# lzhangbj/deep_video_interpolation_extrapolation

Hardware: AMD Instinct MI355X
Metric: train frames/s (256x512 len-3 clips) (higher is better)
Workload: dtype bf16; 1 GPU; InterNet int_5_len_3 train step 256x512 bf16; per_gpu_batch=8, global_batch=8, parallelism=dp1, step=eager, executor side-stream lanes

## Files before the change

deep_video_interpolation_extrapolation_amd/_lib.py:

```python
import ctypes
import os
import threading

import torch

LIB_PATH = os.path.join(os.path.dirname(os.path.abspath(__file__)), "libdvie.so")

DVIE_OK = 0
DVIE_EINVAL = 1001
F32, BF16 = 0, 1
ACT_NONE, ACT_LRELU, ACT_ELU, ACT_RELU, ACT_TANH = 0, 1, 2, 3, 4
EW_FUSE, EW_UPT, EW_POOL, EW_POOLT, EW_COPY, EW_L1SIGN, EW_NCHW, EW_TONCHW, EW_MASK, EW_IM2COL, EW_LABELS = range(11)
LOSS_L1, LOSS_GDL, LOSS_SSIM, LOSS_MSE, LOSS_CE, LOSS_L1NHWC, LOSS_COSNHWC, LOSS_IOU, LOSS_ARGMAX_IOU = range(9)
OP_CONV, OP_WGRAD, OP_WREDUCE, OP_COLSUM, OP_EW, OP_LOSS, OP_PACK = 1, 2, 3, 4, 5, 6, 7
OP_BN_FWD, OP_BN_BWD, OP_HEAD_FWD, OP_HEAD_BWD, OP_ATTN, OP_HEAD3_BWD, OP_SEGENC_FWD = 8, 9, 10, 11, 12, 13, 14
OP_SEGENC_BWD = 15
OP_WREDUCE_MULTI = 16
(ATTN_L2NORM, ATTN_L2NORM_BWD, ATTN_CORR, ATTN_GATHER, ATTN_GATHER_T, ATTN_SOFTMAX, ATTN_SOFTMAX_BWD, ATTN_WNORM,
 ATTN_WNORM_BWD, ATTN_POOL, ATTN_POOL_T) = range(11)

vp = ctypes.c_void_p
i32 = ctypes.c_int
i64 = ctypes.c_longlong
f32 = ctypes.c_float


class ConvDesc(ctypes.Structure):
    _fields_ = [
        ("x", vp), ("w", vp), ("y", vp), ("bias", vp), ("res", vp), ("z", vp),
        ("x_ld", i64), ("y_ld", i64), ("res_ld", i64), ("z_ld", i64),
        ("n", i32), ("ih", i32), ("iw", i32), ("c", i32),
        ("kpad", i32), ("cout", i32),
        ("oh", i32), ("ow", i32), ("sy", i32), ("sx", i32),
        ("th", i32), ("tw", i32), ("dy0", i32), ("dx0", i32), ("ddy", i32), ("ddx", i32),
        ("yh", i32), ("yw", i32), ("osy", i32), ("osx", i32), ("ory", i32), ("orx", i32),
        ("act", i32), ("dact", i32), ("beta", i32), ("dtype", i32),
        ("out_f32", i32), ("alpha", f32), ("phc", i32), ("pad1", i32),
    ]


class WgradDesc(ctypes.Structure):
    _fields_ = [
        ("g", vp), ("x", vp), ("ws", vp),
        ("g_ld", i64), ("x_ld", i64),
        ("n", i32), ("oh", i32), ("ow", i32), ("cout", i32),
        ("ih", i32), ("iw", i32), ("c", i32), ("sy", i32),
        ("sx", i32), ("th", i32), ("tw", i32), ("dy0", i32),
        ("dx0", i32), ("ddy", i32), ("ddx", i32), ("splits", i32),
        ("dtype", i32), ("tmap", i32), ("bws", vp), ("ws_taps", i32), ("pad1", i32),
    ]


class WreduceDesc(ctypes.Structure):
    _fields_ = [
        ("ws", vp), ("dw", vp), ("cmap", vp),
        ("splits", i32), ("ws_rows", i32), ("ws_k", i32), ("co_off", i32),
        ("cout_p", i32), ("cin_p", i32), ("kh_n", i32), ("kw_n", i32),
        ("c", i32), ("beta", i32),
    ]


class ColsumDesc(ctypes.Structure):
    _fields_ = [
        ("g", vp), ("ws", vp), ("g_ld", i64), ("rows", i64),
        ("c", i32), ("splits", i32), ("dtype", i32), ("pad0", i32),
    ]


class PackDesc(ctypes.Structure):
    _fields_ = [
        ("src", vp), ("dst", vp), ("cmap", vp),
        ("rows", i32), ("kpad", i32), ("c", i32), ("mode", i32),
        ("th", i32), ("tw", i32), ("kh0", i32), ("kw0", i32),
        ("dkh", i32), ("dkw", i32), ("cout_s", i32), ("cin_s", i32),
        ("kh_s", i32), ("kw_s", i32), ("dtype", i32), ("blk0", i32),
    ]


class EwDesc(ctypes.Structure):
    _fields_ = [
        ("y", vp), ("src0", vp), ("src1", vp), ("src2", vp), ("res", vp), ("z", vp),
        ("ext", vp), ("mean", vp), ("std", vp),
        ("y_ld", i64), ("src_ld0", i64), ("src_ld1", i64), ("src_ld2", i64), ("res_ld", i64), ("z_ld", i64),
        ("sn", i64), ("sc", i64), ("sh", i64), ("sw", i64),
        ("op", i32), ("n", i32), ("h", i32), ("w", i32),
        ("c", i32), ("nsrc", i32), ("sh0", i32), ("sw0", i32),
        ("sh1", i32), ("sw1", i32), ("sh2", i32), ("sw2", i32),
        ("act", i32), ("dact", i32), ("beta", i32), ("dtype", i32),
        ("ext_c", i32), ("align", i32),
        ("alpha", f32), ("scale", f32),
    ]


class LossDesc(ctypes.Structure):
    _fields_ = [
        ("a", vp), ("b", vp), ("grad", vp), ("out", vp), ("partial", vp), ("ws", vp),
        ("a_sn", i64), ("a_sc", i64), ("a_sh", i64), ("a_sw", i64),
        ("b_sn", i64), ("b_sc", i64), ("b_sh", i64), ("b_sw", i64),
        ("kind", i32), ("bsz", i32), ("ch", i32), ("h", i32),
        ("w", i32), ("beta", i32), ("dtype", i32), ("out_acc", i32),
        ("weight", f32), ("out_scale", f32),
    ]


class WarpDesc(ctypes.Structure):
    _fields_ = [
        ("img", vp), ("flow", vp), ("out", vp), ("dout", vp), ("dimg", vp), ("dflow", vp), ("ws", vp),
        ("n", i32), ("c", i32), ("h", i32), ("w", i32),
        ("align_corners", i32), ("pad0", i32),
    ]


class ClipDesc(ctypes.Structure):
    _fields_ = [
        ("img", vp), ("seg", vp), ("idx", vp), ("params", vp), ("frames", vp), ("segs", vp), ("bad", vp),
        ("b", i32), ("t", i32), ("h0", i32), ("w0", i32), ("hc", i32), ("wc", i32),
        ("n_classes", i32), ("pad0", i32),
    ]


class SynthLoadDesc(ctypes.Structure):
    _fields_ = [("frames", vp), ("out", vp), ("npix", i64), ("out_ld", i32), ("pad0", i32)]


class SynthFinishDesc(ctypes.Structure):
    _fields_ = [
        ("rgb", vp), ("seg", vp), ("frame", vp), ("label", vp), ("npix", i64),
        ("rgb_ld", i32), ("seg_ld", i32), ("n_classes", i32), ("pad0", i32),
    ]


class SynthLoadPadDesc(ctypes.Structure):
    _fields_ = [
        ("frames", vp), ("labels", vp), ("out", vp), ("label_out", vp),
        ("n", i32), ("h", i32), ("w", i32), ("hp", i32), ("wp", i32), ("out_ld", i32),
    ]


class SynthFinishCropDesc(ctypes.Structure):
    _fields_ = [
        ("rgb", vp), ("seg", vp), ("frame", vp), ("label", vp), ("label_canvas", vp),
        ("n", i32), ("h", i32), ("w", i32), ("hp", i32), ("wp", i32),
        ("rgb_ld", i32), ("seg_ld", i32), ("n_classes", i32), ("pad0", i32),
    ]


class SynthBridgeDesc(ctypes.Structure):
    _fields_ = [
        ("rgb", vp), ("seg", vp), ("dst", vp), ("npix", i64),
        ("rgb_ld", i32), ("seg_ld", i32), ("dst_ld", i32), ("dtype", i32),
        ("n_rgb", i32), ("rgb_w", i32), ("seg_w", i32), ("pad0", i32),
    ]


class SynthScoreDesc(ctypes.Structure):
    _fields_ = [
        ("pred", vp), ("gt", vp), ("pred_label", vp), ("gt_label", vp),
        ("sse", vp), ("ssim", vp), ("agree", vp), ("valid", vp), ("inter", vp), ("uni", vp), ("ws", vp),
        ("pred_s0", i64), ("pred_s1", i64), ("gt_s0", i64), ("gt_s1", i64),
        ("pred_label_s0", i64), ("pred_label_s1", i64), ("gt_label_s0", i64), ("gt_label_s1", i64),
        ("n0", i32), ("n1", i32), ("h", i32), ("w", i32), ("n_classes", i32), ("pad0", i32),
    ]


class BnDesc(ctypes.Structure):
    _fields_ = [
        ("x", vp), ("y", vp), ("g", vp), ("dx", vp), ("gamma", vp), ("beta", vp), ("dgamma", vp), ("dbeta", vp),
        ("running_mean", vp), ("running_var", vp), ("partial", vp), ("stats", vp),
        ("x_ld", i64), ("y_ld", i64), ("g_ld", i64), ("dx_ld", i64), ("rows", i64),
        ("c", i32), ("splits", i32), ("act", i32), ("training", i32),
        ("dtype", i32), ("accumulate", i32), ("beta_dx", i32), ("x_f32", i32),
        ("alpha", f32), ("eps", f32), ("momentum", f32), ("pad1", f32),
    ]


class HeadDesc(ctypes.Structure):
    _fields_ = [
        ("x", vp), ("gx", vp), ("gout", vp), ("out", vp), ("pooled", vp),
        ("x_ld", i64), ("gx_ld", i64),
        ("n", i32), ("h", i32), ("w", i32), ("c", i32),
        ("pool", i32), ("dtype", i32), ("beta", i32), ("pad0", i32),
    ]


class SoftmaxDesc(ctypes.Structure):
    _fields_ = [
        ("x", vp), ("y", vp), ("gy", vp), ("gx", vp),
        ("sn", i64), ("sc", i64), ("sh", i64), ("sw", i64),
        ("n", i32), ("c", i32), ("h", i32), ("w", i32),
        ("beta", i32), ("pad0", i32),
    ]


class SnLayer(ctypes.Structure):
    _fields_ = [
        ("w_bar", vp), ("u", vp), ("v", vp), ("w_eff", vp), ("g_eff", vp), ("g_bar", vp), ("g_u", vp), ("g_v", vp),
        ("state_off", i64),
        ("h", i32), ("width", i32), ("power_iterations", i32), ("beta", i32),
    ]


class AttnDesc(ctypes.Structure):
    _fields_ = [
        ("a", vp), ("b0", vp), ("b1", vp), ("y", vp), ("res", vp), ("z", vp),
        ("a_ld", i64), ("b_ld", i64), ("y_ld", i64), ("res_ld", i64), ("z_ld", i64),
        ("op", i32), ("n", i32), ("h", i32), ("w", i32),
        ("c", i32), ("wh", i32), ("ww", i32), ("nhalf", i32),
        ("half0", i32), ("act", i32), ("dact", i32), ("beta", i32),
        ("dtype", i32), ("pad0", i32),
        ("alpha", f32), ("pad1", f32),
    ]


class PackList(ctypes.Structure):
    _fields_ = [("descs_dev", vp), ("n", i32), ("blocks", i32)]


class Head3BwdDesc(ctypes.Structure):
    _fields_ = [
        ("g", vp), ("h", vp), ("wd", vp), ("dh", vp), ("ws", vp),
        ("g_ld", i64), ("h_ld", i64), ("dh_ld", i64),
        ("n", i32), ("hgt", i32), ("wid", i32), ("c", i32),
        ("cout", i32), ("kpad", i32), ("dy0", i32), ("dx0", i32),
        ("splits", i32), ("dact", i32),
        ("alpha", f32), ("pad0", f32),
    ]


class SegencDesc(ctypes.Structure):
    _fields_ = [
        ("inp", vp), ("e1", vp), ("e2", vp), ("out", vp), ("w0", vp), ("w2", vp), ("w4", vp),
        ("b0", vp), ("b2", vp), ("b4", vp),
        ("in_ld", i64), ("e1_ld", i64), ("e2_ld", i64), ("out_ld", i64),
        ("n", i32), ("h", i32), ("w", i32), ("kpad0", i32), ("kpad2", i32), ("kpad4", i32),
    ]


class SegencBwdDesc(ctypes.Structure):
    _fields_ = [
        ("dout", vp), ("e2", vp), ("e1", vp), ("inp", vp), ("w4d", vp), ("w2d", vp),
        ("dw4", vp), ("dw2", vp), ("dw0", vp), ("db4", vp), ("db2", vp), ("db0", vp),
        ("dout_ld", i64), ("e2_ld", i64), ("e1_ld", i64), ("in_ld", i64),
        ("n", i32), ("h", i32), ("w", i32), ("kpad4", i32), ("kpad2", i32), ("slabs", i32),
    ]


class WreduceMultiDesc(ctypes.Structure):
    _fields_ = [("descs", vp), ("n", i32), ("pad", i32)]


class _OpUnion(ctypes.Union):
    _fields_ = [
        ("conv", ConvDesc), ("wgrad", WgradDesc), ("wreduce", WreduceDesc), ("colsum", ColsumDesc),
        ("ew", EwDesc), ("loss", LossDesc), ("pack", PackList), ("bn", BnDesc), ("head", HeadDesc),
        ("attn", AttnDesc), ("head3", Head3BwdDesc), ("segenc", SegencDesc), ("segenc_bwd", SegencBwdDesc),
        ("wreduce_multi", WreduceMultiDesc),
    ]


class Op(ctypes.Structure):
    _fields_ = [("kind", i32), ("lane", i32), ("u", _OpUnion)]


_ABI = {0: Op, OP_CONV: ConvDesc, OP_WGRAD: WgradDesc, OP_WREDUCE: WreduceDesc, OP_COLSUM: ColsumDesc,
        OP_EW: EwDesc, OP_LOSS: LossDesc, OP_PACK: PackDesc, OP_BN_FWD: BnDesc, OP_HEAD_FWD: HeadDesc,
        OP_ATTN: AttnDesc, OP_HEAD3_BWD: Head3BwdDesc, OP_SEGENC_FWD: SegencDesc, OP_SEGENC_BWD: SegencBwdDesc, OP_WREDUCE_MULTI: WreduceMultiDesc, 100: WarpDesc, 101: SoftmaxDesc, 102: SnLayer, 103: ClipDesc,
        104: SynthLoadDesc, 105: SynthFinishDesc, 106: SynthBridgeDesc, 107: SynthScoreDesc,
        108: SynthLoadPadDesc, 109: SynthFinishCropDesc}

EXPORTS = [
    "dvie_conv2d_fwd", "dvie_conv2d_wgrad", "dvie_wgrad_splits_hint", "dvie_wgrad_slabs", "dvie_wgrad_reduce", "dvie_wgrad_reduce_multi", "dvie_colsum", "dvie_pack_weights",
    "dvie_ew", "dvie_loss", "dvie_loss_partial_count", "dvie_loss_ws_floats", "dvie_warp_fwd",
    "dvie_warp_bwd", "dvie_adamax", "dvie_scale", "dvie_run_ops", "dvie_abi_sizeof", "dvie_version",
    "dvie_last_error", "dvie_bn_fwd", "dvie_bn_bwd", "dvie_bn_partial_splits", "dvie_head_fwd", "dvie_head_bwd",
    "dvie_softmax_fwd", "dvie_softmax_bwd", "dvie_adam", "dvie_sn_fwd", "dvie_sn_bwd", "dvie_reparam_fwd",
    "dvie_reparam_bwd", "dvie_warp_ws_floats", "dvie_clip_prep", "dvie_attn", "dvie_step_inc", "dvie_adamax_dev",
    "dvie_adam_dev", "dvie_mfma_probe", "dvie_launch_probe", "dvie_sum_f32", "dvie_wgrad_bias_slabs", "dvie_head3_bwd",
    "dvie_segenc_fwd", "dvie_segenc_bwd", "dvie_pack_blocks", "dvie_trace_kernels", "dvie_traced_kernels",
    "dvie_synth_load", "dvie_synth_finish", "dvie_synth_bridge", "dvie_synth_score", "dvie_synth_score_ws_bytes",
    "dvie_synth_load_pad", "dvie_synth_finish_crop",
]

_lib = None
_lock = threading.Lock()


class DvieError(RuntimeError):
    pass


def load():
    global _lib
    if _lib is not None:
        return _lib
    with _lock:
        if _lib is not None:
            return _lib
        if not os.path.exists(LIB_PATH):
            raise DvieError(
                f"{LIB_PATH} is missing: build it with `python -c 'import __graft_entry__ as g; g.build()'` "
                "(there is no non-HIP fallback)")
        lib = ctypes.CDLL(LIB_PATH)
        lib.dvie_abi_sizeof.restype = ctypes.c_size_t
        lib.dvie_abi_sizeof.argtypes = [i32]
        for which, st in _ABI.items():
            got = lib.dvie_abi_sizeof(which)
            if got != ctypes.sizeof(st):
                raise DvieError(f"ABI mismatch for {st.__name__}: C {got} vs ctypes {ctypes.sizeof(st)}")
        lib.dvie_version.restype = ctypes.c_char_p
        lib.dvie_last_error.restype = ctypes.c_char_p
        for name in ("dvie_conv2d_fwd", "dvie_conv2d_wgrad", "dvie_wgrad_reduce", "dvie_colsum", "dvie_ew",
                     "dvie_loss", "dvie_warp_fwd", "dvie_warp_bwd", "dvie_bn_fwd", "dvie_bn_bwd", "dvie_head_fwd",
                     "dvie_head_bwd", "dvie_softmax_fwd", "dvie_softmax_bwd", "dvie_clip_prep", "dvie_attn",
                     "dvie_head3_bwd", "dvie_segenc_fwd", "dvie_segenc_bwd", "dvie_synth_load", "dvie_synth_finish",
                     "dvie_synth_bridge", "dvie_synth_score", "dvie_synth_load_pad", "dvie_synth_finish_crop"):
            getattr(lib, name).argtypes = [vp, vp]
            getattr(lib, name).restype = i32
        lib.dvie_pack_weights.argtypes = [vp, i32, i32, vp]
        lib.dvie_wgrad_reduce_multi.argtypes = [vp, i32, vp]
        lib.dvie_wgrad_reduce_multi.restype = i32
        lib.dvie_trace_kernels.argtypes = [i32]
        lib.dvie_trace_kernels.restype = i32
        lib.dvie_traced_kernels.argtypes = []
        lib.dvie_traced_kernels.restype = ctypes.c_char_p
        for name in ("dvie_wgrad_splits_hint", "dvie_wgrad_slabs", "dvie_bn_partial_splits", "dvie_pack_blocks"):
            getattr(lib, name).argtypes = [vp]
            getattr(lib, name).restype = i32
        lib.dvie_run_ops.argtypes = [vp, i32, vp]
        lib.dvie_loss_partial_count.argtypes = [vp]
        lib.dvie_loss_partial_count.restype = ctypes.c_size_t
        lib.dvie_warp_ws_floats.argtypes = [vp]
        lib.dvie_warp_ws_floats.restype = ctypes.c_size_t
        lib.dvie_loss_ws_floats.argtypes = [vp]
        lib.dvie_loss_ws_floats.restype = ctypes.c_size_t
        lib.dvie_synth_score_ws_bytes.argtypes = [vp]
        lib.dvie_synth_score_ws_bytes.restype = ctypes.c_size_t
        lib.dvie_adamax.argtypes = [vp, vp, vp, vp, i64, f32, f32, f32, f32, f32, vp]
        lib.dvie_scale.argtypes = [vp, i64, f32, vp]
        lib.dvie_adam.argtypes = [vp, vp, vp, vp, i64, f32, f32, f32, f32, f32, vp]
        f64 = ctypes.c_double
        lib.dvie_adamax_dev.argtypes = [vp, vp, vp, vp, i64, f64, f64, f64, f64, f64, vp, vp]
        lib.dvie_adam_dev.argtypes = [vp, vp, vp, vp, i64, f64, f64, f64, f64, f64, vp, vp]
        lib.dvie_step_inc.argtypes = [vp, vp]
        lib.dvie_mfma_probe.argtypes = [vp, i32, i32, vp]
        lib.dvie_mfma_probe.restype = i32
        lib.dvie_launch_probe.argtypes = [i32, i32, vp]
        lib.dvie_launch_probe.restype = i32
        lib.dvie_sum_f32.argtypes = [vp, i32, vp, vp]
        lib.dvie_sum_f32.restype = i32
        lib.dvie_wgrad_bias_slabs.argtypes = [vp]
        lib.dvie_wgrad_bias_slabs.restype = i32
        for name in ("dvie_sn_fwd", "dvie_sn_bwd"):
            getattr(lib, name).argtypes = [vp, i32, vp, vp]
            getattr(lib, name).restype = i32
        lib.dvie_reparam_fwd.argtypes = [vp, vp, vp, vp, i64, vp]
        lib.dvie_reparam_bwd.argtypes = [vp, vp, vp, vp, vp, i64, i32, vp]
        lib.dvie_reparam_fwd.restype = lib.dvie_reparam_bwd.restype = i32
        _lib = lib
        return lib


def check(rc, what=""):
    if rc != DVIE_OK:
        msg = load().dvie_last_error().decode(errors="replace") if rc == DVIE_EINVAL else f"hipError {rc}"
        raise DvieError(f"{what}: {msg}")


def stream_ptr(device=None):
    return torch.cuda.current_stream(device).cuda_stream


def require_gpu(t):
    if not t.is_cuda:
        raise DvieError("dvie ops run on the MI355X only: tensor is on %s (no CPU fallback)" % t.device)
```

deep_video_interpolation_extrapolation_amd/csrc/conv1x1.hip:

```cpp
#include <stdlib.h>

#include "conv_epilogue.h"

namespace dvie {

typedef __attribute__((address_space(3))) void* lds_ptr_1x1;

#define DVIE_VMCNT1(N) __builtin_amdgcn_s_waitcnt(((N) & 15) | (((N) >> 4) << 14) | (7 << 4) | (15 << 8))

__device__ __forceinline__ void transpose8x8(i32x4 (&ob)[8], int lane) {
  const int b = lane & 7;
#pragma unroll
  for (int d = 4; d >= 1; d >>= 1) {
    const bool up = (b & d) != 0;
#pragma unroll
    for (int k = 0; k < 8; ++k) {
      if (k & d) continue;
      i32x4 t, r;
#pragma unroll
      for (int e = 0; e < 4; ++e) t[e] = up ? ob[k][e] : ob[k + d][e];
#pragma unroll
      for (int e = 0; e < 4; ++e) r[e] = __shfl_xor(t[e], d);
#pragma unroll
      for (int e = 0; e < 4; ++e) {
        ob[k][e] = up ? r[e] : ob[k][e];
        ob[k + d][e] = up ? ob[k + d][e] : r[e];
      }
    }
  }
}

template <int TMC, int NS, int KC, int NWP, int MI = 1, int NWC = 1>
struct G1Cfg {
  static constexpr int NW = NWP * NWC;
  static constexpr int BC = 32 * TMC * NWC;
  static constexpr int BP = 32 * MI * NWP;
  static constexpr int RB = KC * 2;
  static constexpr int NCH = RB / 16;
  static constexpr int RPP = 64 / NCH;
  static constexpr int NSL = KC / 16;
  static constexpr int XSZ = BP * RB;
  static constexpr int WSZ = BC * RB;
  static constexpr int STAGE = XSZ + WSZ;
  static constexpr int SMEM = NS * STAGE;
  static constexpr int XQ = BP / RPP / NW;
  static constexpr int WQ = (BC / RPP + NW - 1) / NW;
  static __device__ __forceinline__ int swz(int row) { return NCH == 8 ? (row >> 1) & 7 : (row >> 2) & 3; }
};

template <int TMC, int NS, int KC, int NWP, int MI, int NWC, bool OUTF32, int PRE = 0, bool CE = false>
__global__ __launch_bounds__(64 * NWP * NWC) void conv1x1_kernel(const dvie_conv_desc p, int n_ct, int n_tiles, int dbg) {
  dbg = DVIE_DBG(dbg);
  typedef G1Cfg<TMC, NS, KC, NWP, MI, NWC> C;
  constexpr int NW = C::NW;
  __shared__ __attribute__((aligned(1024))) char smem[C::SMEM];
  const int tid = threadIdx.x, lane = tid & 63;
  const int wave = __builtin_amdgcn_readfirstlane(tid >> 6);
  const int r32 = lane & 31, hh = lane >> 5;
  const unsigned OOB = 0xFFFFFFF0u;

  const int g = blockIdx.x & 7, i8 = blockIdx.x >> 3;
  const int q8 = n_tiles >> 3, r8 = n_tiles & 7;
  const int bid = (g < r8 ? g * (q8 + 1) : r8 * (q8 + 1) + (g - r8) * q8) + i8;
  const int c0 = (bid % n_ct) * C::BC;
  const int p0 = (bid / n_ct) * C::BP;
  const int npix = p.n * p.oh * p.ow;
  const int nk = (p.c + KC - 1) / KC;

  const int lrow = lane / C::NCH, lch = lane % C::NCH;
  unsigned xo[C::XQ];
#pragma unroll
  for (int q = 0; q < C::XQ; ++q) {
    const int row = (wave + NW * q) * C::RPP + lrow;
    const int cs = lch ^ C::swz(row);
    xo[q] = (p0 + row < npix) ? (unsigned)(p0 + row) * (unsigned)p.x_ld * 2u + cs * 16u : OOB;
    if (cs * 8 >= p.c) xo[q] = OOB;
  }
  unsigned wo[C::WQ];
#pragma unroll
  for (int q = 0; q < C::WQ; ++q) {
    const int row = (wave + NW * q) * C::RPP + lrow;
    const int cs = lch ^ C::swz(row);
    wo[q] = (row < C::BC && cs * 8 < p.c) ? (unsigned)row * (unsigned)p.kpad * 2u + cs * 16u : OOB;
  }
  const unsigned long long xbytes =
      ((unsigned long long)p.n * p.ih * p.iw - 1) * (unsigned long long)p.x_ld * 2ull + (unsigned long long)p.c * 2ull;
  const unsigned wbytes = (unsigned)p.cout * (unsigned)p.kpad * 2u;

  auto stage = [&](int k, int sb) {
    char* X = smem + sb * C::STAGE;
    char* W = X + C::XSZ;
    const int xr = (int)(xbytes - (unsigned long long)k * C::RB);
    const __amdgpu_buffer_rsrc_t rx =
        __builtin_amdgcn_make_buffer_rsrc((void*)((const char*)p.x + (size_t)k * C::RB), 0, xr, 0x00020000);
    const unsigned wb = (unsigned)(c0 * p.kpad + KC * k) * 2u;
    const __amdgpu_buffer_rsrc_t rw =
        __builtin_amdgcn_make_buffer_rsrc((void*)((const char*)p.w + wb), 0, (int)(wbytes - wb), 0x00020000);
    const int cvalid = p.c - KC * k;
#pragma unroll
    for (int q = 0; q < C::XQ; ++q) {
      const int row = (wave + NW * q) * C::RPP + lrow;
      const int cs = lch ^ C::swz(row);
      const unsigned o = cs * 8 < cvalid ? xo[q] : OOB;
      __builtin_amdgcn_raw_ptr_buffer_load_lds(rx, (lds_ptr_1x1)(X + (wave + NW * q) * 1024), 16, o, 0, 0, 0);
    }
#pragma unroll
    for (int q = 0; q < C::WQ; ++q) {
      if (wave + NW * q < C::BC / C::RPP) {
        const int row = (wave + NW * q) * C::RPP + lrow;
        const int cs = lch ^ C::swz(row);
        const unsigned o = cs * 8 < cvalid ? wo[q] : OOB;
        __builtin_amdgcn_raw_ptr_buffer_load_lds(rw, (lds_ptr_1x1)(W + (wave + NW * q) * 1024), 16, o, 0, 0, 0);
      }
    }
  };

  const int wp = wave % NWP, wc = wave / NWP;
  int xf[C::NSL], wf[C::NSL];
#pragma unroll
  for (int s = 0; s < C::NSL; ++s) {
    const int prow = wp * 32 * MI + r32;
    xf[s] = prow * C::RB + (((2 * s + hh) ^ C::swz(prow)) << 4);
    wf[s] = (wc * 32 * TMC + r32) * C::RB + (((2 * s + hh) ^ C::swz(r32)) << 4);
  }

  f32x16 acc[MI][TMC];
#pragma unroll
  for (int i = 0; i < MI; ++i)
#pragma unroll
    for (int j = 0; j < TMC; ++j)
#pragma unroll
      for (int e = 0; e < 16; ++e) acc[i][j][e] = 0.f;

#pragma unroll
  for (int k = 0; k < (NS > 1 ? NS - 1 : 1); ++k)
    if (k < nk) stage(k, k);

  static_assert(PRE == 0 || (NS == 1 && !OUTF32), "operand prefetch: single K-step, bf16 output");
  i32x4 pr_r[(PRE & 1) ? MI : 1][TMC][2], pr_b[(PRE & 2) ? MI : 1][TMC][2], pr_z[(PRE & 4) ? MI : 1][TMC][2];
  constexpr bool CEL = CE && (PRE & (PRE - 1)) != 0;
  if constexpr (CEL) {
    const int wp0 = wave % NWP, wc0 = wave / NWP;
    const int a8 = r32 >> 3, bl = lane & 7;
    const int co = c0 + wc0 * 32 * TMC + 16 * bl + 8 * hh;
#pragma unroll
    for (int k = 0; k < 8; ++k) {
      const int pix = p0 + wp0 * 32 + 8 * a8 + k;
      const bool ok = pix < npix;
      const long long q = ok ? pix : 0;
      if constexpr ((PRE & 1) != 0)
        pr_r[0][k >> 1][k & 1] = ok ? *(const i32x4*)((const bf16_t*)p.res + q * p.res_ld + co) : i32x4{0, 0, 0, 0};
      if constexpr ((PRE & 2) != 0)
        pr_b[0][k >> 1][k & 1] = ok ? *(const i32x4*)((const bf16_t*)p.y + q * p.y_ld + co) : i32x4{0, 0, 0, 0};
      if constexpr ((PRE & 4) != 0)
        pr_z[0][k >> 1][k & 1] = ok ? *(const i32x4*)((const bf16_t*)p.z + q * p.z_ld + co) : i32x4{0, 0, 0, 0};
    }
  } else if constexpr (PRE != 0) {
    const int wp0 = wave % NWP, wc0 = wave / NWP;
#pragma unroll
    for (int i = 0; i < MI; ++i)
#pragma unroll
      for (int j = 0; j < TMC; ++j)
#pragma unroll
        for (int P = 0; P < 2; ++P) {
          const int pix = p0 + wp0 * 32 * MI + 32 * i + r32;
          const int co = c0 + wc0 * 32 * TMC + 32 * j + 16 * P + 8 * hh;
          const bool ok = pix < npix && co < p.cout;
          const long long q = ok ? pix : 0;
          if constexpr ((PRE & 1) != 0)
            pr_r[i][j][P] = ok ? *(const i32x4*)((const bf16_t*)p.res + q * p.res_ld + co) : i32x4{0, 0, 0, 0};
          if constexpr ((PRE & 2) != 0)
            pr_b[i][j][P] = ok ? *(const i32x4*)((const bf16_t*)p.y + q * p.y_ld + co) : i32x4{0, 0, 0, 0};
          if constexpr ((PRE & 4) != 0)
            pr_z[i][j][P] = ok ? *(const i32x4*)((const bf16_t*)p.z + q * p.z_ld + co) : i32x4{0, 0, 0, 0};
        }
  }
  for (int k = 0; k < nk; ++k) {
    const int sb = k % NS;
    if constexpr (NS >= 3) {
      static_assert(NS <= 5, "wait table covers up to 3 stages in flight");
      constexpr int P_HI = C::XQ + C::WQ, P_LO = C::XQ + C::WQ - 1;
      static_assert(3 * P_HI < 64, "vmcnt is 6 bits");
      const bool hi = wave + NW * (C::WQ - 1) < C::BC / C::RPP;
      const int m = min(NS - 2, nk - 1 - k);
      if (m >= 3) {
        if (hi) DVIE_VMCNT1(3 * P_HI); else DVIE_VMCNT1(3 * P_LO);
      } else if (m == 2) {
        if (hi) DVIE_VMCNT1(2 * P_HI); else DVIE_VMCNT1(2 * P_LO);
      } else if (m == 1) {
        if (hi) DVIE_VMCNT1(P_HI); else DVIE_VMCNT1(P_LO);
      } else {
        __builtin_amdgcn_s_waitcnt(0);
      }
    } else {
      __builtin_amdgcn_s_waitcnt(0);
    }
    __builtin_amdgcn_s_barrier();
    if (NS > 1 && k + NS - 1 < nk) stage(k + NS - 1, (k + NS - 1) % NS);
    const char* X = smem + sb * C::STAGE;
    const char* W = X + C::XSZ;
    if (dbg & 2) continue;
#pragma unroll
    for (int s = 0; s < C::NSL; ++s) {
      i32x4 b[MI], a[TMC];
#pragma unroll
      for (int i = 0; i < MI; ++i) b[i] = *(const i32x4*)(X + xf[s] + i * 32 * C::RB);
#pragma unroll
      for (int j = 0; j < TMC; ++j) a[j] = *(const i32x4*)(W + wf[s] + j * 32 * C::RB);
#pragma unroll
      for (int i = 0; i < MI; ++i)
#pragma unroll
        for (int j = 0; j < TMC; ++j)
          acc[i][j] = __builtin_amdgcn_mfma_f32_32x32x16_bf16(__builtin_bit_cast(bf16x8, a[j]),
                                                              __builtin_bit_cast(bf16x8, b[i]), acc[i][j], 0, 0, 0);
    }
  }

  static_assert(!CE || (MI == 1 && 2 * TMC == 8 && !OUTF32), "coalesced epilogue: 8 chunks per lane");
  if constexpr (CEL) {
    auto tr = [&](i32x4 (&a)[TMC][2]) {
      i32x4 t8[8];
#pragma unroll
      for (int k = 0; k < 8; ++k) t8[k] = a[k >> 1][k & 1];
      transpose8x8(t8, lane);
#pragma unroll
      for (int k = 0; k < 8; ++k) a[k >> 1][k & 1] = t8[k];
    };
    if constexpr ((PRE & 1) != 0) tr(pr_r[0]);
    if constexpr ((PRE & 2) != 0) tr(pr_b[0]);
    if constexpr ((PRE & 4) != 0) tr(pr_z[0]);
  }
  i32x4 ob[CE ? 8 : 1];
#pragma unroll
  for (int i = 0; i < MI; ++i) {
  const int pix0 = p0 + wp * 32 * MI + 32 * i + r32;
  const int pix = CE ? min(pix0, npix - 1) : pix0;
  float v[TMC][2][8];
#pragma unroll
  for (int j = 0; j < TMC; ++j) acc_rows8(acc[i][j], v[j]);
  if (!CE && pix >= npix) continue;
  long long yp = pix;
  if (p.osy != 1 || p.osx != 1 || p.ory != 0 || p.orx != 0 || p.yh != p.oh || p.yw != p.ow) {
    const int hw = p.oh * p.ow;
    const int n = pix / hw, r = pix - n * hw;
    const int oy = r / p.ow, ox = r - oy * p.ow;
    yp = ((long long)n * p.yh + oy * p.osy + p.ory) * p.yw + ox * p.osx + p.orx;
  }
#pragma unroll
  for (int j = 0; j < TMC; ++j)
#pragma unroll
    for (int P = 0; P < 2; ++P) {
      const int co = c0 + wc * 32 * TMC + 32 * j + 16 * P + 8 * hh;
      if (!CE && co >= p.cout) continue;
      float* w = v[j][P];
      if constexpr (OUTF32) {
        epi8_mem<true>(w, p, yp, co);
      } else {
        if (p.bias) add_f32x8(w, p.bias + co);
        bf16_t* dst = (bf16_t*)p.y + yp * p.y_ld + co;
        if (p.res) {
          if constexpr ((PRE & 1) != 0)
            add_bf16x8(w, pr_r[i][j][P]);
          else
            add_bf16x8(w, *(const i32x4*)((const bf16_t*)p.res + yp * p.res_ld + co));
        }
        if (p.beta) {
          if constexpr ((PRE & 2) != 0)
            add_bf16x8(w, pr_b[i][j][P]);
          else
            add_bf16x8(w, *(const i32x4*)dst);
        }
        act8(w, p.act, p.alpha);
        if (p.dact) {
          if constexpr ((PRE & 4) != 0)
            dact_bf16x8(w, pr_z[i][j][P], p.dact, p.alpha);
          else
            dact_bf16x8(w, *(const i32x4*)((const bf16_t*)p.z + yp * p.z_ld + co), p.dact, p.alpha);
        }
        const i32x4 o = pack_bf16x8(w);
        if constexpr (CE)
          ob[2 * j + P] = o;
        else if (!(dbg & 1) || w[0] == 12345.678f)
          *(i32x4*)dst = o;
      }
    }
  }
  if constexpr (CE) {
    transpose8x8(ob, lane);
    const int b = lane & 7;
    const int a8 = r32 >> 3;
#pragma unroll
    for (int k = 0; k < 8; ++k) {
      const int px = p0 + wp * 32 + 8 * a8 + k;
      const int co = c0 + wc * 32 * TMC + 32 * (b >> 1) + 16 * (b & 1) + 8 * hh;
      if (px < npix) *(i32x4*)((bf16_t*)p.y + (long long)px * p.y_ld + co) = ob[k];
    }
  }
}

template <int TMC, int NS, int KC, int NWP, int MI, int NWC>
__global__ __launch_bounds__(64 * NWP * NWC) void conv1x1_persist_kernel(const dvie_conv_desc p, int n_ct, int n_tiles) {
  typedef G1Cfg<TMC, NS, KC, NWP, MI, NWC> C;
  constexpr int NW = C::NW;
  static_assert(NS >= 2, "stage ring");
  __shared__ __attribute__((aligned(1024))) char smem[C::SMEM];
  const int tid = threadIdx.x, lane = tid & 63;
  const int wave = __builtin_amdgcn_readfirstlane(tid >> 6);
  const int r32 = lane & 31, hh = lane >> 5;
  const unsigned OOB = 0xFFFFFFF0u;

  const int G = gridDim.x;
  const int g = blockIdx.x & 7, i8 = blockIdx.x >> 3;
  const int q8 = G >> 3, r8 = G & 7;
  const int b = (g < r8 ? g * (q8 + 1) : r8 * (q8 + 1) + (g - r8) * q8) + i8;
  const int npix = p.n * p.oh * p.ow;
  const int nk = (p.c + KC - 1) / KC;
  const int my_tiles = b < n_tiles ? (n_tiles - 1 - b) / G + 1 : 0;
  const int njobs = my_tiles * nk;
  if (njobs == 0) return;

  const int lrow = lane / C::NCH, lch = lane % C::NCH;
  const unsigned long long xbytes =
      ((unsigned long long)p.n * p.ih * p.iw - 1) * (unsigned long long)p.x_ld * 2ull + (unsigned long long)p.c * 2ull;
  const unsigned wbytes = (unsigned)p.cout * (unsigned)p.kpad * 2u;

  auto stage = [&](int jj, int sb) {
    const int i = jj / nk, k = jj - nk * (jj / nk);
    const int T = b + i * G;
    const int c0 = (T % n_ct) * C::BC, p0 = (T / n_ct) * C::BP;
    char* X = smem + sb * C::STAGE;
    char* W = X + C::XSZ;
    const int xr = (int)(xbytes - (unsigned long long)k * C::RB);
    const __amdgpu_buffer_rsrc_t rx =
        __builtin_amdgcn_make_buffer_rsrc((void*)((const char*)p.x + (size_t)k * C::RB), 0, xr, 0x00020000);
    const unsigned wb = (unsigned)(c0 * p.kpad + KC * k) * 2u;
    const __amdgpu_buffer_rsrc_t rw =
        __builtin_amdgcn_make_buffer_rsrc((void*)((const char*)p.w + wb), 0, (int)(wbytes - wb), 0x00020000);
    const int cvalid = p.c - KC * k;
#pragma unroll
    for (int q = 0; q < C::XQ; ++q) {
      const int row = (wave + NW * q) * C::RPP + lrow;
      const int cs = lch ^ C::swz(row);
      const unsigned o = (cs * 8 < cvalid && p0 + row < npix) ? (unsigned)(p0 + row) * (unsigned)p.x_ld * 2u + cs * 16u : OOB;
      __builtin_amdgcn_raw_ptr_buffer_load_lds(rx, (lds_ptr_1x1)(X + (wave + NW * q) * 1024), 16, o, 0, 0, 0);
    }
#pragma unroll
    for (int q = 0; q < C::WQ; ++q) {
      if (wave + NW * q < C::BC / C::RPP) {
        const int row = (wave + NW * q) * C::RPP + lrow;
        const int cs = lch ^ C::swz(row);
        const unsigned o = (row < C::BC && cs * 8 < cvalid) ? (unsigned)row * (unsigned)p.kpad * 2u + cs * 16u : OOB;
        __builtin_amdgcn_raw_ptr_buffer_load_lds(rw, (lds_ptr_1x1)(W + (wave + NW * q) * 1024), 16, o, 0, 0, 0);
      }
    }
  };

  const int wp = wave % NWP, wc = wave / NWP;
  int xf[C::NSL], wf[C::NSL];
#pragma unroll
  for (int sl = 0; sl < C::NSL; ++sl) {
    const int prow = wp * 32 * MI + r32;
    xf[sl] = prow * C::RB + (((2 * sl + hh) ^ C::swz(prow)) << 4);
    wf[sl] = (wc * 32 * TMC + r32) * C::RB + (((2 * sl + hh) ^ C::swz(r32)) << 4);
  }

  constexpr int P_HI = C::XQ + C::WQ, P_LO = C::XQ + C::WQ - 1;
  static_assert((NS - 2) * P_HI < 64, "vmcnt is 6 bits");
  const bool hi = wave + NW * (C::WQ - 1) < C::BC / C::RPP;
  auto wait_stages = [&](int j) {
    const int m = min(NS - 2, njobs - 1 - j);
    if (m >= 3) {
      if (hi) DVIE_VMCNT1(3 * P_HI); else DVIE_VMCNT1(3 * P_LO);
    } else if (m == 2) {
      if (hi) DVIE_VMCNT1(2 * P_HI); else DVIE_VMCNT1(2 * P_LO);
    } else if (m == 1) {
      if (hi) DVIE_VMCNT1(P_HI); else DVIE_VMCNT1(P_LO);
    } else {
      __builtin_amdgcn_s_waitcnt(0);
    }
  };

  f32x16 acc[MI][TMC];
#pragma unroll
  for (int k = 0; k < NS - 1; ++k)
    if (k < njobs) stage(k, k);
  for (int jj = 0; jj < njobs; ++jj) {
    const int k = jj - nk * (jj / nk);
    if (k == 0) {
#pragma unroll
      for (int i = 0; i < MI; ++i)
#pragma unroll
        for (int j = 0; j < TMC; ++j)
#pragma unroll
          for (int e = 0; e < 16; ++e) acc[i][j][e] = 0.f;
    }
    if (k != 0 || jj == 0) wait_stages(jj);
    __builtin_amdgcn_s_barrier();
    if (jj + NS - 1 < njobs) stage(jj + NS - 1, (jj + NS - 1) % NS);
    const char* X = smem + (jj % NS) * C::STAGE;
    const char* W = X + C::XSZ;
#pragma unroll
    for (int sl = 0; sl < C::NSL; ++sl) {
      i32x4 bq[MI], a[TMC];
#pragma unroll
      for (int i = 0; i < MI; ++i) bq[i] = *(const i32x4*)(X + xf[sl] + i * 32 * C::RB);
#pragma unroll
      for (int j = 0; j < TMC; ++j) a[j] = *(const i32x4*)(W + wf[sl] + j * 32 * C::RB);
#pragma unroll
      for (int i = 0; i < MI; ++i)
#pragma unroll
        for (int j = 0; j < TMC; ++j)
          acc[i][j] = __builtin_amdgcn_mfma_f32_32x32x16_bf16(__builtin_bit_cast(bf16x8, a[j]),
                                                              __builtin_bit_cast(bf16x8, bq[i]), acc[i][j], 0, 0, 0);
    }
    if (k + 1 < nk) continue;
    if (jj + 1 < njobs) wait_stages(jj + 1);

    const int T = b + (jj / nk) * G;
    const int c0 = (T % n_ct) * C::BC, p0 = (T / n_ct) * C::BP;
#pragma unroll
    for (int i = 0; i < MI; ++i) {
      const int pix = p0 + wp * 32 * MI + 32 * i + r32;
      float v[TMC][2][8];
#pragma unroll
      for (int j = 0; j < TMC; ++j) acc_rows8(acc[i][j], v[j]);
      if (pix >= npix) continue;
      long long yp = pix;
      if (p.osy != 1 || p.osx != 1 || p.ory != 0 || p.orx != 0 || p.yh != p.oh || p.yw != p.ow) {
        const int hw = p.oh * p.ow;
        const int n = pix / hw, r = pix - n * hw;
        const int oy = r / p.ow, ox = r - oy * p.ow;
        yp = ((long long)n * p.yh + oy * p.osy + p.ory) * p.yw + ox * p.osx + p.orx;
      }
#pragma unroll
      for (int j = 0; j < TMC; ++j)
#pragma unroll
        for (int P = 0; P < 2; ++P) {
          const int co = c0 + wc * 32 * TMC + 32 * j + 16 * P + 8 * hh;
          if (co >= p.cout) continue;
          epi8_mem<false>(v[j][P], p, yp, co);
        }
    }
  }
  __builtin_amdgcn_s_waitcnt(0);
}

template <int TMC, int NWP, int MI, int NWC, int ACT, int AB = 0>
__global__ __launch_bounds__(64 * NWP * NWC) void conv1x1_ring_kernel(const dvie_conv_desc p, int n_ct, int n_tiles) {
  constexpr int dbg = AB;
  typedef G1Cfg<TMC, 2, 64, NWP, MI, NWC> C;
  constexpr int NW = C::NW, SL = 32768, NSLOT = 5, PPH = 4;
  static_assert(C::XSZ == SL && C::WSZ == SL && C::XQ == PPH && C::WQ == PPH && C::BC / C::RPP == NW * PPH,
                "ring slot = one operand of one K-step, 4 pieces per wave");
  __shared__ __attribute__((aligned(1024))) char smem[NSLOT * SL];
  const int tid = threadIdx.x, lane = tid & 63;
  const int wave = __builtin_amdgcn_readfirstlane(tid >> 6);
  const int r32 = lane & 31, hh = lane >> 5;
  const unsigned OOB = 0xFFFFFFF0u;

  const int G = gridDim.x;
  const int g = blockIdx.x & 7, i8 = blockIdx.x >> 3;
  const int q8 = G >> 3, r8 = G & 7;
  const int b = (g < r8 ? g * (q8 + 1) : r8 * (q8 + 1) + (g - r8) * q8) + i8;
  const int npix = p.n * p.oh * p.ow;
  const int nk = (p.c + 63) / 64;
  const int my_tiles = b < n_tiles ? (n_tiles - 1 - b) / G + 1 : 0;
  const int njobs = my_tiles * nk;
  if (njobs == 0) return;

  const int lrow = lane / C::NCH, lch = lane % C::NCH;
  const unsigned long long xbytes =
      ((unsigned long long)p.n * p.ih * p.iw - 1) * (unsigned long long)p.x_ld * 2ull + (unsigned long long)p.c * 2ull;
  const unsigned wbytes = (unsigned)p.cout * (unsigned)p.kpad * 2u;
  const __amdgpu_buffer_rsrc_t rx = __builtin_amdgcn_make_buffer_rsrc((void*)p.x, 0, (int)xbytes, 0x00020000);
  const __amdgpu_buffer_rsrc_t rw = __builtin_amdgcn_make_buffer_rsrc((void*)p.w, 0, (int)wbytes, 0x00020000);
  const unsigned long long ybytes =
      ((unsigned long long)p.n * p.yh * p.yw - 1) * (unsigned long long)p.y_ld * 2ull + (unsigned long long)p.cout * 2ull;
  const __amdgpu_buffer_rsrc_t ry = __builtin_amdgcn_make_buffer_rsrc(p.y, 0, (int)ybytes, 0x00020000);
  const __amdgpu_buffer_rsrc_t rb = __builtin_amdgcn_make_buffer_rsrc((void*)p.bias, 0, p.bias ? p.cout * 4 : 0, 0x00020000);

  int prow[PPH];
  unsigned xoff[PPH], woff[PPH], chk[PPH];
#pragma unroll
  for (int q = 0; q < PPH; ++q) {
    const int row = (wave + NW * q) * C::RPP + lrow;
    const int cs = lch ^ C::swz(row);
    prow[q] = row;
    chk[q] = (unsigned)cs * 8u;
    xoff[q] = (unsigned)row * (unsigned)p.x_ld * 2u + (unsigned)cs * 16u;
    woff[q] = (unsigned)row * (unsigned)p.kpad * 2u + (unsigned)cs * 16u;
  }
  struct Cur {
    int i, k, c0, p0;
  };
  auto cur_at = [&](int jj) {
    Cur c;
    c.i = jj / nk;
    c.k = jj - c.i * nk;
    const int T = b + c.i * G;
    c.c0 = (T % n_ct) * C::BC;
    c.p0 = (T / n_ct) * C::BP;
    return c;
  };
  auto cur_next = [&](Cur c) {
    if (++c.k == nk) {
      c.k = 0;
      ++c.i;
      const int T = b + c.i * G;
      c.c0 = (T % n_ct) * C::BC;
      c.p0 = (T / n_ct) * C::BP;
    }
    return c;
  };
  auto issue = [&](const Cur& c, bool live, int wop, int sl) {
    char* dst = smem + sl * SL + wave * 1024;
    const int cvalid = live ? p.c - 64 * c.k : 0;
    const int lim = live ? (wop ? p.cout - c.c0 : npix - c.p0) : 0;
    const unsigned base = wop ? (unsigned)c.c0 * (unsigned)p.kpad * 2u + 128u * (unsigned)c.k
                              : (unsigned)c.p0 * (unsigned)p.x_ld * 2u + 128u * (unsigned)c.k;
#pragma unroll
    for (int q = 0; q < PPH; ++q) {
      const bool ok = prow[q] < lim && (cvalid >= 64 || (int)chk[q] < cvalid);
      const unsigned o = ok ? base + (wop ? woff[q] : xoff[q]) : OOB;
      __builtin_amdgcn_raw_ptr_buffer_load_lds(wop ? rw : rx, (lds_ptr_1x1)(dst + q * NW * 1024), 16, o, 0, 0, 0);
    }
  };

  const int wp = wave % NWP, wc = wave / NWP;
  int xf[C::NSL], wf[C::NSL];
#pragma unroll
  for (int sl = 0; sl < C::NSL; ++sl) {
    const int pr = wp * 32 * MI + r32;
    xf[sl] = pr * C::RB + (((2 * sl + hh) ^ C::swz(pr)) << 4);
    wf[sl] = (wc * 32 * TMC + r32) * C::RB + (((2 * sl + hh) ^ C::swz(r32)) << 4);
  }
  const int bco = wc * 32 * TMC + 4 * hh;

  f32x16 acc[MI][TMC];
  Cur cj = cur_at(0);
  Cur cw = cur_next(cj);
  Cur cx = cur_next(cw);
  issue(cj, true, 0, 0);
  issue(cj, true, 1, 1);
  issue(cw, 1 < njobs, 0, 2);
  int s0 = 0;
  int jj = 0;
  auto job = [&](bool first, bool after_epi) {
    if (after_epi)
      DVIE_VMCNT1(PPH + 2 * MI * TMC);
    else
      DVIE_VMCNT1(PPH);
    __builtin_amdgcn_s_waitcnt(0xC07F);
    __builtin_amdgcn_s_barrier();
    f32x4 bi[TMC][4];
    if (first) {
#pragma unroll
      for (int j = 0; j < TMC; ++j)
#pragma unroll
        for (int u = 0; u < 4; ++u) {
          const int co = cj.c0 + bco + 32 * j + 8 * u;
          bi[j][u] = __builtin_bit_cast(f32x4, __builtin_amdgcn_raw_buffer_load_b128(rb, co < p.cout ? (unsigned)co * 4u : OOB, 0, 0));
        }
    }
    if (!(dbg & 4)) {
      const int sw = s0 + 3 >= NSLOT ? s0 + 3 - NSLOT : s0 + 3, sx = s0 + 4 >= NSLOT ? s0 + 4 - NSLOT : s0 + 4;
      issue(cw, jj + 1 < njobs, 1, sw);
      issue(cx, jj + 2 < njobs, 0, sx);
    }
    if (first) {
#pragma unroll
      for (int ii = 0; ii < MI; ++ii)
#pragma unroll
        for (int j = 0; j < TMC; ++j)
#pragma unroll
          for (int e = 0; e < 16; ++e) acc[ii][j][e] = bi[j][e >> 2][e & 3];
    }
    const char* X = smem + s0 * SL;
    const char* W = smem + (s0 + 1 >= NSLOT ? s0 + 1 - NSLOT : s0 + 1) * SL;
#pragma unroll
    for (int sl = 0; sl < C::NSL; ++sl) {
      if (dbg & 2) break;
      i32x4 bq[MI], a[TMC];
#pragma unroll
      for (int ii = 0; ii < MI; ++ii) bq[ii] = *(const i32x4*)(X + xf[sl] + ii * 32 * C::RB);
#pragma unroll
      for (int j = 0; j < TMC; ++j) a[j] = *(const i32x4*)(W + wf[sl] + j * 32 * C::RB);
#pragma unroll
      for (int ii = 0; ii < MI; ++ii)
#pragma unroll
        for (int j = 0; j < TMC; ++j)
          acc[ii][j] = __builtin_amdgcn_mfma_f32_32x32x16_bf16(__builtin_bit_cast(bf16x8, a[j]),
                                                               __builtin_bit_cast(bf16x8, bq[ii]), acc[ii][j], 0, 0, 0);
    }
    s0 = s0 + 2 >= NSLOT ? s0 + 2 - NSLOT : s0 + 2;
    cj = cw;
    cw = cx;
    cx = cur_next(cx);
    ++jj;
  };
  for (int it = 0; it < my_tiles; ++it) {
    const int c0 = cj.c0, p0 = cj.p0;
    job(true, it > 0);
    for (int k = 1; k < nk; ++k) job(false, false);

#pragma unroll
    for (int ii = 0; ii < MI; ++ii) {
      const int pix0 = p0 + wp * 32 * MI + 32 * ii + r32;
      const bool pix_ok = pix0 < npix;
      const int pix = pix_ok ? pix0 : npix - 1;
      long long yp = pix;
      if (p.osy != 1 || p.osx != 1 || p.ory != 0 || p.orx != 0 || p.yh != p.oh || p.yw != p.ow) {
        const int hw = p.oh * p.ow;
        const int n = pix / hw, r = pix - n * hw;
        const int oy = r / p.ow, ox = r - oy * p.ow;
        yp = ((long long)n * p.yh + oy * p.osy + p.ory) * p.yw + ox * p.osx + p.orx;
      }
#pragma unroll
      for (int j = 0; j < TMC; ++j)
#pragma unroll
        for (int P = 0; P < 2; ++P) {
          float w[8];
#pragma unroll
          for (int e = 0; e < 4; ++e) {
            const auto sw = __builtin_amdgcn_permlane32_swap(__float_as_uint(acc[ii][j][8 * P + e]),
                                                             __float_as_uint(acc[ii][j][8 * P + 4 + e]), false, false);
            w[e] = __uint_as_float(sw[0]);
            w[4 + e] = __uint_as_float(sw[1]);
          }
          if (ACT == DVIE_ACT_LRELU) {
#pragma unroll
            for (int e = 0; e < 8; ++e) w[e] = fmaxf(w[e], w[e] * p.alpha);
          }
          const i32x4 o = pack_bf16x8(w);
          const int co = c0 + wc * 32 * TMC + 32 * j + 16 * P + 8 * hh;
          const unsigned yo = (pix_ok && co < p.cout && !(dbg & 1)) ? (unsigned)((yp * p.y_ld + co) * 2) : OOB;
          __builtin_amdgcn_raw_buffer_store_b128(__builtin_bit_cast(i32x4, o), ry, yo, 0, 0);
        }
    }
  }
  __builtin_amdgcn_s_waitcnt(0);
}

template <int V, int NS, int MT>
struct PreOk {
  static constexpr int v = NS != 1 || MT > 4 ? 0 : V;
};

static int dbg_env() {
#ifdef DVIE_TIMING_DBG
  const char* e = getenv("DVIE_1X1_DBG");
  return e && *e ? atoi(e) : 0;
#else
  return 0;
#endif
}

static bool ce_env_on() {
  const char* e = getenv("DVIE_1X1_CE");
  return !(e && *e == '0');
}

template <int TMC, int NS, int KC = 64, int NWP = 8, int MI = 1, int NWC = 1>
static void launch_1x1(const dvie_conv_desc& p, hipStream_t s) {
  typedef G1Cfg<TMC, NS, KC, NWP, MI, NWC> C;
  constexpr int NW = C::NW;
  const int npix = p.n * p.oh * p.ow;
  const int n_ct = (p.cout + C::BC - 1) / C::BC;
  const int n_tiles = n_ct * ((npix + C::BP - 1) / C::BP);
  if (p.out_f32) {
    DVIE_LAUNCH((conv1x1_kernel<TMC, NS, KC, NWP, MI, NWC, true>), dim3(n_tiles), dim3(64 * NW), 0, s, p, n_ct, n_tiles, dbg_env());
    return;
  }
  if constexpr (NS == 2 && KC == 64 && TMC == 4 && NWP == 4 && MI == 2 && NWC == 2) {
    const unsigned long long span = ((unsigned long long)p.n * p.yh * p.yw - 1) * (unsigned long long)p.y_ld * 2ull +
                                    (unsigned long long)p.cout * 2ull;
    const unsigned long long xspan = ((unsigned long long)npix - 1) * (unsigned long long)p.x_ld * 2ull + (unsigned long long)p.c * 2ull;
    if (p.c > KC && n_tiles > 256 && !p.res && !p.beta && !p.dact && span < 0xFFFFFF00ull &&
        xspan < 0xFFFFFF00ull && p.ih == p.oh && p.iw == p.ow &&
        (p.act == DVIE_ACT_NONE || (p.act == DVIE_ACT_LRELU && p.alpha >= 0.f && p.alpha <= 1.f))) {
#ifdef DVIE_TIMING_DBG
      if (p.act == DVIE_ACT_LRELU) switch (dbg_env() & 7) {
#define DVIE_RING_AB(V)                                                                                                \
  case V:                                                                                                              \
    DVIE_LAUNCH((conv1x1_ring_kernel<TMC, NWP, MI, NWC, DVIE_ACT_LRELU, V>), dim3(256), dim3(64 * NW), 0, s, p, n_ct, \
                n_tiles);                                                                                              \
    return;
          DVIE_RING_AB(1) DVIE_RING_AB(2) DVIE_RING_AB(3) DVIE_RING_AB(4) DVIE_RING_AB(5) DVIE_RING_AB(6) DVIE_RING_AB(7)
#undef DVIE_RING_AB
          default: break;
        }
#endif
      if (p.act == DVIE_ACT_LRELU)
        DVIE_LAUNCH((conv1x1_ring_kernel<TMC, NWP, MI, NWC, DVIE_ACT_LRELU>), dim3(256), dim3(64 * NW), 0, s, p, n_ct, n_tiles);
      else
        DVIE_LAUNCH((conv1x1_ring_kernel<TMC, NWP, MI, NWC, DVIE_ACT_NONE>), dim3(256), dim3(64 * NW), 0, s, p, n_ct, n_tiles);
      return;
    }
  }
  if constexpr (NS >= 2 && NS <= 5 && MI * TMC <= 4) {
    const int per_cu = 163840 / C::SMEM;
    const int G = 256 * (per_cu > 2 ? 2 : per_cu);
    if (p.c > KC && n_tiles > G) {
      DVIE_LAUNCH((conv1x1_persist_kernel<TMC, NS, KC, NWP, MI, NWC>), dim3(G), dim3(64 * NW), 0, s, p, n_ct,
                         n_tiles);
      return;
    }
  }
  const bool ident = p.osy == 1 && p.osx == 1 && p.ory == 0 && p.orx == 0 && p.yh == p.oh && p.yw == p.ow;
  int pre = 0;
  if constexpr (NS == 1) {
    if (ident && p.c <= KC) {
      pre = MI * TMC > 4 ? 0 : (p.res ? 1 : 0) | (p.beta ? 2 : 0) | (p.dact ? 4 : 0);
    }
  }
  if constexpr (NS == 1 && MI == 1 && 2 * TMC == 8) {
    if (ident && ce_env_on() && p.cout % C::BC == 0) {
      switch (pre) {
#define DVIE_CE_CASE(V)                                                                                              \
  case V:                                                                                                            \
    DVIE_LAUNCH((conv1x1_kernel<TMC, NS, KC, NWP, MI, NWC, false, PreOk<V, NS, MI * TMC>::v, true>), dim3(n_tiles), \
                       dim3(64 * NW), 0, s, p, n_ct, n_tiles, 0);                                                     \
    return;
        DVIE_CE_CASE(0) DVIE_CE_CASE(1) DVIE_CE_CASE(2) DVIE_CE_CASE(3) DVIE_CE_CASE(4)
        DVIE_CE_CASE(5) DVIE_CE_CASE(6) DVIE_CE_CASE(7)
#undef DVIE_CE_CASE
      }
    }
  }
  switch (pre) {
#define DVIE_PRE_CASE(V)                                                                                          \
  case V:                                                                                                        \
    DVIE_LAUNCH((conv1x1_kernel<TMC, NS, KC, NWP, MI, NWC, false, PreOk<V, NS, MI * TMC>::v>), dim3(n_tiles), \
                       dim3(64 * NW), 0, s, p, n_ct, n_tiles, dbg_env());                                                   \
    break;
    DVIE_PRE_CASE(1) DVIE_PRE_CASE(2) DVIE_PRE_CASE(3) DVIE_PRE_CASE(4) DVIE_PRE_CASE(5)
    DVIE_PRE_CASE(6) DVIE_PRE_CASE(7)
#undef DVIE_PRE_CASE
    default:
      DVIE_LAUNCH((conv1x1_kernel<TMC, NS, KC, NWP, MI, NWC, false>), dim3(n_tiles), dim3(64 * NW), 0, s, p, n_ct, n_tiles, dbg_env());
  }
}

bool conv1x1_launch(const dvie_conv_desc& p, hipStream_t s) {
  if (p.dtype != DVIE_BF16 || p.th != 1 || p.tw != 1) return false;
  if (p.sy != 1 || p.sx != 1 || p.dy0 != 0 || p.dx0 != 0 || p.ih != p.oh || p.iw != p.ow) return false;
  if (p.osy < 1 || p.osx < 1 || p.ory < 0 || p.orx < 0) return false;
  if (p.c % 64 != 0 && p.c > 64) return false;
  if ((long long)p.n * p.oh * p.ow >= (1LL << 31)) return false;
  const int cout = p.cout;
  const bool one = p.c <= 64;
  if (cout <= 64 || (cout <= 128 && one))
    one ? launch_1x1<2, 1>(p, s) : launch_1x1<2, 3>(p, s);
  else if (cout <= 128)
    launch_1x1<4, 3>(p, s);
  else if (one)
    launch_1x1<4, 1>(p, s);
  else
    launch_1x1<4, 2, 64, 4, 2, 2>(p, s);
  return true;
}

}
```

deep_video_interpolation_extrapolation_amd/csrc/conv_epilogue.h:

```cpp
#pragma once
#include "common.h"

namespace dvie {

template <bool F32OUT = false>
__device__ __forceinline__ void act8(float* v, int act, float alpha) {
  if (act == DVIE_ACT_LRELU) {
    for (int k = 0; k < 8; ++k) v[k] = v[k] > 0.f ? v[k] : v[k] * alpha;
  } else if (act == DVIE_ACT_RELU) {
    for (int k = 0; k < 8; ++k) v[k] = v[k] > 0.f ? v[k] : 0.f;
  } else if (act == DVIE_ACT_ELU) {
    for (int k = 0; k < 8; ++k) v[k] = F32OUT ? (v[k] > 0.f ? v[k] : expm1f(v[k])) : elu_bf(v[k]);
  } else if (act == DVIE_ACT_TANH) {
    for (int k = 0; k < 8; ++k) v[k] = F32OUT ? tanhf(v[k]) : tanh_bf(v[k]);
  }
}

__device__ __forceinline__ void dact8(float* v, const float* z, int dact, float alpha) {
  if (dact == DVIE_ACT_LRELU) {
    for (int k = 0; k < 8; ++k) v[k] *= z[k] > 0.f ? 1.f : alpha;
  } else if (dact == DVIE_ACT_RELU) {
    for (int k = 0; k < 8; ++k) v[k] = z[k] > 0.f ? v[k] : 0.f;
  } else if (dact == DVIE_ACT_ELU) {
    for (int k = 0; k < 8; ++k) v[k] *= z[k] > 0.f ? 1.f : z[k] + 1.f;
  } else if (dact == DVIE_ACT_TANH) {
    for (int k = 0; k < 8; ++k) v[k] *= 1.f - z[k] * z[k];
  }
}

__device__ __forceinline__ void unpack_bf16x8(const i32x4 t, float* v) {
#pragma unroll
  for (int e = 0; e < 4; ++e) {
    v[2 * e] = __uint_as_float(((uint32_t)t[e]) << 16);
    v[2 * e + 1] = __uint_as_float(((uint32_t)t[e]) & 0xffff0000u);
  }
}

__device__ __forceinline__ void add_bf16x8(float* w, const i32x4 t) {
  float v[8];
  unpack_bf16x8(t, v);
#pragma unroll
  for (int e = 0; e < 8; ++e) w[e] += v[e];
}

__device__ __forceinline__ void add_f32x8(float* w, const float* s) {
  const f32x4 r0 = *(const f32x4*)s, r1 = *(const f32x4*)(s + 4);
#pragma unroll
  for (int e = 0; e < 4; ++e) {
    w[e] += r0[e];
    w[4 + e] += r1[e];
  }
}

__device__ __forceinline__ i32x4 pack_bf16x8(const float* w) {
  i32x4 o;
#pragma unroll
  for (int e = 0; e < 4; ++e) o[e] = (int)pack_bf16x2(w[2 * e], w[2 * e + 1]);
  return o;
}

__device__ __forceinline__ void dact_bf16x8(float* w, const i32x4 tz, int dact, float alpha) {
  float z[8];
  unpack_bf16x8(tz, z);
  dact8(w, z, dact, alpha);
}

template <bool R, bool B, bool Z>
__device__ __forceinline__ i32x4 epi8_regs(float* w, const dvie_conv_desc& p, const i32x4* r, const i32x4* b,
                                           const i32x4* z) {
  if constexpr (R) add_bf16x8(w, *r);
  if constexpr (B) add_bf16x8(w, *b);
  act8(w, p.act, p.alpha);
  if constexpr (Z) dact_bf16x8(w, *z, p.dact, p.alpha);
  return pack_bf16x8(w);
}

template <bool OUTF32>
__device__ __forceinline__ void epi8_mem(float* w, const dvie_conv_desc& p, long long pix, int co) {
  if (p.bias) add_f32x8(w, p.bias + co);
  if constexpr (OUTF32) {
    float* dst = (float*)p.y + pix * p.y_ld + co;
    if (p.res) add_f32x8(w, (const float*)p.res + pix * p.res_ld + co);
    if (p.beta) add_f32x8(w, dst);
    act8<true>(w, p.act, p.alpha);
    if (p.dact) dact_bf16x8(w, *(const i32x4*)((const bf16_t*)p.z + pix * p.z_ld + co), p.dact, p.alpha);
    *(f32x4*)dst = f32x4{w[0], w[1], w[2], w[3]};
    *(f32x4*)(dst + 4) = f32x4{w[4], w[5], w[6], w[7]};
  } else {
    bf16_t* dst = (bf16_t*)p.y + pix * p.y_ld + co;
    if (p.res) add_bf16x8(w, *(const i32x4*)((const bf16_t*)p.res + pix * p.res_ld + co));
    if (p.beta) add_bf16x8(w, *(const i32x4*)dst);
    act8(w, p.act, p.alpha);
    if (p.dact) dact_bf16x8(w, *(const i32x4*)((const bf16_t*)p.z + pix * p.z_ld + co), p.dact, p.alpha);
    *(i32x4*)dst = pack_bf16x8(w);
  }
}

}
```

deep_video_interpolation_extrapolation_amd/csrc/conv_fwd.hip:

```cpp
#include "common.h"

namespace dvie {

template <typename T>
__device__ __forceinline__ void mfma_chunk(f32x4& acc, const i32x4& a, const i32x4& b);

template <>
__device__ __forceinline__ void mfma_chunk<float>(f32x4& acc, const i32x4& a, const i32x4& b) {
  acc = __builtin_amdgcn_mfma_f32_16x16x4f32(__int_as_float(a[0]), __int_as_float(b[0]), acc, 0, 0, 0);
  acc = __builtin_amdgcn_mfma_f32_16x16x4f32(__int_as_float(a[1]), __int_as_float(b[1]), acc, 0, 0, 0);
  acc = __builtin_amdgcn_mfma_f32_16x16x4f32(__int_as_float(a[2]), __int_as_float(b[2]), acc, 0, 0, 0);
  acc = __builtin_amdgcn_mfma_f32_16x16x4f32(__int_as_float(a[3]), __int_as_float(b[3]), acc, 0, 0, 0);
}

template <>
__device__ __forceinline__ void mfma_chunk<bf16_t>(f32x4& acc, const i32x4& a, const i32x4& b) {
  acc = __builtin_amdgcn_mfma_f32_16x16x32_bf16(__builtin_bit_cast(bf16x8, a), __builtin_bit_cast(bf16x8, b),
                                                acc, 0, 0, 0);
}

__device__ __forceinline__ int swz128(int row, int ch) { return row * 128 + ((ch ^ ((row >> 1) & 7)) << 4); }

typedef __attribute__((address_space(3))) void* lds_ptr_t;

// ... 154 lines not shown
      } else {
        const int kv = kv0 + b_ch[i];
        tap = kv / CV;
        cv = kv - tap * CV;
        const int ti = tap / p.tw;
        dy = p.dy0 + ti * p.ddy;
        dx = p.dx0 + (tap - ti * p.tw) * p.ddx;
      }
      const int iy = by[i] + dy, ix = bx[i] + dx;
      unsigned off = OOB;
      if (tap < ntap && (unsigned)iy < (unsigned)p.ih && (unsigned)ix < (unsigned)p.iw)
        off = (unsigned)(((((unsigned long long)bn[i] * p.ih + iy) * p.iw + ix) * p.x_ld + (unsigned)cv * VEC) * ES);
      __builtin_amdgcn_raw_ptr_buffer_load_lds(rx, (lds_ptr_t)(Bs + (wave + 4 * i) * 1024), 16, off, 0, 0, 0);
    }
  };

  f32x4 acc[TM][TN];
#pragma unroll
  for (int i = 0; i < TM; ++i)
#pragma unroll
    for (int j = 0; j < TN; ++j) acc[i][j] = f32x4{0.f, 0.f, 0.f, 0.f};

  stage(0, 0);
  __builtin_amdgcn_s_waitcnt(0);
  __syncthreads();

  const int r16 = lane & 15;
  for (int kt = 0; kt < nk; ++kt) {
    const int cur = kt & 1;
    if (kt + 1 < nk) stage(kt + 1, cur ^ 1);
    const char* As = smem + cur * STAGE;
    const char* Bs = As + BC * 128;
#pragma unroll
    for (int s = 0; s < 2; ++s) {
      const int ch = 4 * s + (lane >> 4);
      i32x4 af[TM], bfr[TN];
#pragma unroll
      for (int i = 0; i < TM; ++i) af[i] = *(const i32x4*)(As + swz128(wc * (BC / WC) + 16 * i + r16, ch));
#pragma unroll
      for (int j = 0; j < TN; ++j) bfr[j] = *(const i32x4*)(Bs + swz128(wp * (BP / WP) + 16 * j + r16, ch));
#pragma unroll
      for (int i = 0; i < TM; ++i)
#pragma unroll
        for (int j = 0; j < TN; ++j) mfma_chunk<T>(acc[i][j], af[i], bfr[j]);
    }
    __builtin_amdgcn_s_waitcnt(0);
    __syncthreads();
  }

  float* E = (float*)smem;
#pragma unroll
  for (int i = 0; i < TM; ++i)
#pragma unroll
    for (int j = 0; j < TN; ++j) {
      const int co_l = wc * (BC / WC) + 16 * i + 4 * (lane >> 4);
      const int px_l = wp * (BP / WP) + 16 * j + r16;
      *(f32x4*)((char*)E + px_l * EROW + co_l * 4) = acc[i][j];
    }
  __syncthreads();
  constexpr int OV = Out16<OutT>::N;
  constexpr int CPR = BC / OV;
  OutT* __restrict__ yg = (OutT*)p.y;
  const OutT* __restrict__ rg = (const OutT*)p.res;
  const T* __restrict__ zg = (const T*)p.z;
  for (int idx = tid; idx < BP * CPR; idx += 256) {
    const int px_l = idx / CPR;
    const int ck = idx - px_l * CPR;
    const int co = c0 + ck * OV;
    const long long pix = p0 + px_l;
    if (pix >= npix || co >= p.cout) continue;
    float v[OV];
    const char* er = (const char*)E + px_l * EROW + ck * OV * 4;
#pragma unroll
    for (int k = 0; k < OV; k += 4) {
      const f32x4 t = *(const f32x4*)(er + k * 4);
      v[k] = t[0];
      v[k + 1] = t[1];
      v[k + 2] = t[2];
      v[k + 3] = t[3];
    }
    const int n = (int)(pix / hw);
    const int r = (int)(pix - (long long)n * hw);
    const int oy = r / p.ow;
    const int ox = r - oy * p.ow;
    const long long yrow = ((long long)n * p.yh + oy * p.osy + p.ory) * p.yw + ox * p.osx + p.orx;
    if (p.bias) {
#pragma unroll
      for (int k = 0; k < OV; k += 4) {
        const f32x4 b = *(const f32x4*)(p.bias + co + k);
        v[k] += b[0];
        v[k + 1] += b[1];
        v[k + 2] += b[2];
        v[k + 3] += b[3];
      }
    }
    if (rg) {
      float t[OV];
      Out16<OutT>::load(rg + yrow * p.res_ld + co, t);
#pragma unroll
      for (int k = 0; k < OV; ++k) v[k] += t[k];
    }
    if (p.beta) {
      float t[OV];
      Out16<OutT>::load(yg + yrow * p.y_ld + co, t);
#pragma unroll
      for (int k = 0; k < OV; ++k) v[k] += t[k];
    }
    if (p.act) {
#pragma unroll
      for (int k = 0; k < OV; ++k) v[k] = act_fwd(v[k], p.act, p.alpha);
    }
    if (p.dact) {
      float z[OV];
      load_n<T, OV>(zg + yrow * p.z_ld + co, z);
#pragma unroll
      for (int k = 0; k < OV; ++k) v[k] *= act_dz(z[k], p.dact, p.alpha);
    }
    Out16<OutT>::store(yg + yrow * p.y_ld + co, v);
  }
}

template <typename T, int BC, int BP, int WC, int WP>
static void launch_conv(const dvie_conv_desc& p, hipStream_t s) {
  const long long npix = (long long)p.n * p.oh * p.ow;
  const int n_ct = (p.cout + BC - 1) / BC;
  const int n_tiles = (int)((npix + BP - 1) / BP) * n_ct;
  if (p.out_f32)
    DVIE_LAUNCH((conv_igemm_kernel<T, BC, BP, WC, WP, true>), dim3(n_tiles), dim3(256), 0, s, p, n_ct, n_tiles);
  else
    DVIE_LAUNCH((conv_igemm_kernel<T, BC, BP, WC, WP, false>), dim3(n_tiles), dim3(256), 0, s, p, n_ct,
                       n_tiles);
}

template <typename T>
static void dispatch_conv(const dvie_conv_desc& p, hipStream_t s) {
  const long long npix = (long long)p.n * p.oh * p.ow;
  const bool small = npix < 64LL * 512;
  if (p.cout <= 32) {
    if (small) launch_conv<T, 32, 64, 2, 2>(p, s);
    else launch_conv<T, 32, 128, 2, 2>(p, s);
  } else if (p.cout <= 64) {
    if (small) launch_conv<T, 64, 64, 2, 2>(p, s);
    else launch_conv<T, 64, 128, 2, 2>(p, s);
  } else {
    if (small) launch_conv<T, 128, 64, 2, 2>(p, s);
    else launch_conv<T, 128, 128, 2, 2>(p, s);
  }
}

bool conv_halo_launch(const dvie_conv_desc& p, hipStream_t s);
bool conv_halo_ph4_launch(const dvie_conv_desc& p, hipStream_t s);
bool conv1x1_launch(const dvie_conv_desc& p, hipStream_t s);
bool conv_s2_launch(const dvie_conv_desc& p, hipStream_t s);

}

using namespace dvie;

extern "C" int dvie_conv2d_fwd(const dvie_conv_desc* d, void* stream) {
  DVIE_CHECK_ARG(d && d->x && d->w && d->y, "conv: null pointer");
  const int vec = d->dtype == DVIE_BF16 ? 8 : 4;
  const int es = d->dtype == DVIE_BF16 ? 2 : 4;
  const int ovec = (d->out_f32 || d->dtype == DVIE_F32) ? 4 : 8;
  DVIE_CHECK_ARG(d->c > 0 && d->c % vec == 0, "conv: c=%d must be a multiple of %d", d->c, vec);
  DVIE_CHECK_ARG(d->cout > 0 && d->cout % ovec == 0, "conv: cout=%d must be a multiple of %d", d->cout, ovec);
  DVIE_CHECK_ARG(d->kpad % 64 == 0 && d->kpad >= d->th * d->tw * d->c, "conv: kpad=%d", d->kpad);
  DVIE_CHECK_ARG(d->x_ld % vec == 0 && d->y_ld % ovec == 0 && (!d->res || d->res_ld % ovec == 0) &&
                     (!d->z || d->z_ld % ovec == 0),
                 "conv: ld alignment x_ld=%lld y_ld=%lld", d->x_ld, d->y_ld);
  DVIE_CHECK_ARG(d->th >= 1 && d->tw >= 1 && d->th * d->tw <= 64, "conv: taps");
  DVIE_CHECK_ARG(d->n > 0 && d->oh > 0 && d->ow > 0 && d->ih > 0 && d->iw > 0, "conv: empty shape");
  DVIE_CHECK_ARG(((uintptr_t)d->x & 15) == 0 && ((uintptr_t)d->w & 15) == 0 && ((uintptr_t)d->y & 15) == 0,
                 "conv: x/w/y not 16B aligned");
  DVIE_CHECK_ARG(!d->bias || ((uintptr_t)d->bias & 15) == 0, "conv: bias not 16B aligned");
  DVIE_CHECK_ARG(d->dtype == DVIE_BF16 || d->out_f32 || d->dtype == DVIE_F32, "conv: dtype");
  const unsigned long long img_x = (unsigned long long)d->ih * d->iw * d->x_ld * es;
  const unsigned long long wb = (unsigned long long)d->cout * d->kpad * es;
  DVIE_CHECK_ARG(wb < 0xFFFFFF00ull, "conv: weights exceed the 4 GiB buffer range");
  DVIE_CHECK_ARG(img_x < 0xFFFFFF00ull, "conv: one input image exceeds the 4 GiB buffer range");
  hipStream_t s = (hipStream_t)stream;
  const long long chunk = (long long)(0xFFFFFF00ull / img_x) < d->n ? (long long)(0xFFFFFF00ull / img_x) : d->n;
  const int oes = (d->out_f32 || d->dtype == DVIE_F32) ? 4 : 2;
  const unsigned long long img_y = (unsigned long long)d->yh * d->yw;
  for (long long n0 = 0; n0 < d->n; n0 += chunk) {
    dvie_conv_desc c = *d;
    c.n = (int)(d->n - n0 < chunk ? d->n - n0 : chunk);
    c.x = (const char*)d->x + n0 * img_x;
    c.y = (char*)d->y + n0 * img_y * d->y_ld * oes;
    if (d->res) c.res = (const char*)d->res + n0 * img_y * d->res_ld * oes;
    if (d->z) c.z = (const char*)d->z + n0 * img_y * d->z_ld * es;
    if (c.phc) {
      DVIE_CHECK_ARG(conv_halo_ph4_launch(c, s), "conv: phase-split output (phc=%d) needs bf16, 2x2 taps at "
                     "(0,0), osy=osx=2, cout=4*phc, phc %% 32 == 0, no bias", c.phc);
      continue;
    }
    if (conv1x1_launch(c, s)) continue;
    if (conv_halo_launch(c, s)) continue;
    if (conv_s2_launch(c, s)) continue;
    if (c.dtype == DVIE_BF16)
      dispatch_conv<bf16_t>(c, s);
    else
      dispatch_conv<float>(c, s);
  }
  DVIE_RETURN_LAUNCH();
}
```

deep_video_interpolation_extrapolation_amd/csrc/conv_halo.hip:

```cpp
#include <stdlib.h>
#include <string.h>

#include "conv_epilogue.h"

namespace dvie {

typedef __attribute__((address_space(3))) void* lds_ptr_t;

__device__ __forceinline__ int xcd_remap3(int b, int nb) {
  const int g = b & 7, i = b >> 3;
  const int q = nb >> 3, r = nb & 7;
  const int start = g < r ? g * (q + 1) : r * (q + 1) + (g - r) * q;
  return start + i;
}

template <int TM, int WC, int WP, int TH, int TW>
struct HaloCfg {
  static constexpr int NW = WC * WP;
  static constexpr int NTH = NW * 64;
  static constexpr int BC = 32 * TM * WC;
  static constexpr int PR = WP;
  static constexpr int NT = TH * TW;
  static constexpr int HR = PR + TH - 1;
  static constexpr int HWD = 64 + TW - 1;
// ... 661 lines not shown
  auto group_issue = [&](int g) {
    const __amdgpu_buffer_rsrc_t r = g < niter ? rx : rnone;
#pragma unroll
    for (int q = 0; q < C::NPL; ++q) {
      const int pc = wave + NW * q;
      const int j = pc / C::RP, pr = pc - C::RP * (pc / C::RP);
      const int R = g * WR + 2 + j;
      char* dst = smem + (R % C::RR) * C::RB + pr * 1024;
      const unsigned o = lane_off(pr, yb + R);
      __builtin_amdgcn_raw_ptr_buffer_load_lds(r, (lds_ptr_t)dst, 16, o, 0, 0, 0);
    }
  };
  {
#pragma unroll
    for (int q = 0; q < C::NP0; ++q) {
      const int pc = wave + NW * q;
      const int j = pc / C::RP, pr = pc - C::RP * (pc / C::RP);
      char* dst = pc < 2 * C::RP ? smem + j * C::RB + pr * 1024 : smem + C::RR * C::RB + (pc - 2 * C::RP) * 1024;
      const unsigned o = pc < 2 * C::RP ? lane_off(pr, yb + j) : OOB;
      __builtin_amdgcn_raw_ptr_buffer_load_lds(rx, (lds_ptr_t)dst, 16, o, 0, 0, 0);
    }
#pragma unroll
    for (int g = 0; g < D; ++g) group_issue(g);
  }

  constexpr int NE = OUTF32 ? 0 : 4 * (((EPI & 1) ? 1 : 0) + ((EPI & 2) ? 1 : 0) + ((EPI & 4) ? 1 : 0));
  i32x4 er[2][2], eb[2][2], ez[2][2];
  auto epi_issue = [&](int i) {
    const int oy = ys + i * WR + wr;
#pragma unroll
    for (int b = 0; b < 2; ++b)
#pragma unroll
      for (int P = 0; P < 2; ++P) {
        const int ox = x0 + 32 * b + r32, co = 32 * wc + 8 * hh + 16 * P;
        const bool ok = oy < p.oh && ox < p.ow && co < p.cout;
        const long long pix = ((long long)n * p.yh + (long long)oy * p.osy + p.ory) * p.yw + (long long)ox * p.osx + p.orx;
        if constexpr ((EPI & 1) != 0) {
          const __amdgpu_buffer_rsrc_t r = __builtin_amdgcn_make_buffer_rsrc((void*)p.res, 0, 0x7FFFFFF0, 0x00020000);
          er[b][P] = __builtin_amdgcn_raw_buffer_load_b128(r, ok ? (unsigned)((pix * p.res_ld + co) * 2) : OOB, 0, 0);
        }
        if constexpr ((EPI & 2) != 0) {
          const __amdgpu_buffer_rsrc_t r = __builtin_amdgcn_make_buffer_rsrc((void*)p.y, 0, 0x7FFFFFF0, 0x00020000);
          eb[b][P] = __builtin_amdgcn_raw_buffer_load_b128(r, ok ? (unsigned)((pix * p.y_ld + co) * 2) : OOB, 0, 0);
        }
        if constexpr ((EPI & 4) != 0) {
          const __amdgpu_buffer_rsrc_t r = __builtin_amdgcn_make_buffer_rsrc((void*)p.z, 0, 0x7FFFFFF0, 0x00020000);
          ez[b][P] = __builtin_amdgcn_raw_buffer_load_b128(r, ok ? (unsigned)((pix * p.z_ld + co) * 2) : OOB, 0, 0);
        }
      }
  };

  constexpr int NST = OUTF32 ? 8 : 4;
  const int b_lane = r32 * C::PITCH + hh * 16;
  for (int i = 0; i < niter; ++i) {
    wait_vmcnt((D - 1) * C::NPL + min(i, D) * NST + min(i, D - 1) * NE);
    __builtin_amdgcn_s_barrier();
    if constexpr (NE > 0) epi_issue(i);
    group_issue(i + D);

    f32x16 acc[2];
#pragma unroll
    for (int b = 0; b < 2; ++b)
#pragma unroll
      for (int e = 0; e < 16; ++e) acc[b][e] = 0.f;
#pragma unroll
    for (int ti = 0; ti < 3; ++ti) {
      const char* H = smem + ((i * WR + wr + ti) % C::RR) * C::RB + b_lane;
#pragma unroll
      for (int tj = 0; tj < 3; ++tj)
#pragma unroll
        for (int sl = 0; sl < KS; ++sl) {
          i32x4 bf[2];
#pragma unroll
          for (int b = 0; b < 2; ++b) bf[b] = *(const i32x4*)(H + (32 * b + tj) * C::PITCH + sl * 32);
#pragma unroll
          for (int b = 0; b < 2; ++b)
            acc[b] = __builtin_amdgcn_mfma_f32_32x32x16_bf16(__builtin_bit_cast(bf16x8, wa[3 * ti + tj][sl]),
                                                             __builtin_bit_cast(bf16x8, bf[b]), acc[b], 0, 0, 0);
        }
    }
#pragma unroll
    for (int b = 0; b < 2; ++b) {
      if constexpr (OUTF32)
        ws_epilogue<true>(p, acc[b], n, ys + i * WR + wr, x0 + 32 * b + r32, 32 * wc + 8 * hh);
      else
        strip_epilogue<(EPI < 0 ? 0 : EPI)>(p, acc[b], n, ys + i * WR + wr, x0 + 32 * b + r32, 32 * wc + 8 * hh, er[b], eb[b],
                                          ez[b]);
    }
  }
  __builtin_amdgcn_s_waitcnt(0);
}

template <int KS, int WR, int D, int EPI>
static void launch_strip_k(const dvie_conv_desc& p, hipStream_t s) {
  const int tiles_x = (p.ow + 63) / 64;
  const int cap = 256 * (4 / WR);
  const int cols = p.n * tiles_x;
  int nseg = cap / cols;
  if (nseg < 1) nseg = 1;
  if (nseg > (p.oh + WR - 1) / WR) nseg = (p.oh + WR - 1) / WR;
  int seg = (p.oh + nseg - 1) / nseg;
  seg = (seg + WR - 1) / WR * WR;
  nseg = (p.oh + seg - 1) / seg;
  const int n_wg = cols * nseg;
  DVIE_LAUNCH((conv_strip_kernel<KS, EPI, WR, D>), dim3(n_wg), dim3(2 * WR * 64), 0, s, p, tiles_x, nseg, seg,
                     n_wg);
}

template <int KS, int WR, int D>
static bool launch_strip_cfg(const dvie_conv_desc& p, hipStream_t s) {
  if (p.out_f32) {
    launch_strip_k<KS, WR, D, -1>(p, s);
    return true;
  }
  switch ((p.res ? 1 : 0) | (p.beta ? 2 : 0) | (p.dact ? 4 : 0)) {
    case 0: launch_strip_k<KS, WR, D, 0>(p, s); return true;
    case 1: launch_strip_k<KS, WR, D, 1>(p, s); return true;
    case 2: launch_strip_k<KS, WR, D, 2>(p, s); return true;
    case 3: launch_strip_k<KS, WR, D, 3>(p, s); return true;
    case 4: launch_strip_k<KS, WR, D, 4>(p, s); return true;
    case 5: launch_strip_k<KS, WR, D, 5>(p, s); return true;
    case 6: launch_strip_k<KS, WR, D, 6>(p, s); return true;
  }
  return false;
}

static int strip_mode() {
  const char* e = getenv("DVIE_CONV_STRIP");
  return e && *e ? atoi(e) : 2;
}

template <int KS>
static bool launch_strip(const dvie_conv_desc& p, hipStream_t s) {
  switch (strip_mode()) {
    case 1: return launch_strip_cfg<KS, 4, 2>(p, s);
    case 2: return launch_strip_cfg<KS, 2, 2>(p, s);
    case 3: return launch_strip_cfg<KS, 2, 1>(p, s);
  }
  return false;
}

template <int CP8>
struct NkCfg {
  static constexpr int WP = 4, NW = 8;
  static constexpr int HR = WP + 2, HWD = 66;
  static constexpr int PS = CP8 == 1 ? 1 : 3;
  static constexpr int SLOTS = HR * HWD * PS;
  static constexpr int NPC = ((SLOTS + 63) / 64 + NW - 1) / NW;
  static constexpr int HSZ = NPC * NW * 1024;
  static constexpr int NG = 9 * CP8;
  static constexpr int NS = (NG + 1) / 2;
};

template <int CP8, bool OUTF32, bool PRE = false>
__global__ __launch_bounds__(512, 2) void conv_nk_kernel(const dvie_conv_desc p, int n_cb, int n_tiles, int tiles_x,
                                                        int tiles_y) {
  typedef NkCfg<CP8> C;
  __shared__ __attribute__((aligned(1024))) char smem[2 * C::HSZ];
  const int tid = threadIdx.x, lane = tid & 63;
  const int wave = __builtin_amdgcn_readfirstlane(tid >> 6);
  const int wc = wave / C::WP, wp = wave % C::WP;
  const int r32 = lane & 31, hh = lane >> 5;
  const unsigned OOB = 0xFFFFFFF0u;

  const int lid = xcd_remap3(blockIdx.x, gridDim.x);
  const int cb = lid % n_cb;
  const int per_cb = gridDim.x / n_cb;
  const int tile0 = lid / n_cb;
  if (tile0 >= n_tiles) return;

  i32x4 wa[C::NS];
  {
    const int co = cb * 64 + 32 * wc + r32;
#pragma unroll
    for (int sl = 0; sl < C::NS; ++sl) {
      const int k = 16 * sl + 8 * hh;
      i32x4 v = {0, 0, 0, 0};
      if (co < p.cout && k < 9 * p.c) v = *(const i32x4*)((const bf16_t*)p.w + (long long)co * p.kpad + k);
      wa[sl] = v;
    }
  }
  int boff[C::NS];
#pragma unroll
  for (int sl = 0; sl < C::NS; ++sl) {
    const int g = 2 * sl + hh;
    const int t = g < C::NG ? g / CP8 : 0, j = g < C::NG ? g % CP8 : 0;
    boff[sl] = (((t / 3) * C::HWD + (t % 3)) * C::PS + j) * 16;
  }
  int hgeo[C::NPC];
#pragma unroll
  for (int q = 0; q < C::NPC; ++q) {
    const int slot = (wave + C::NW * q) * 64 + lane;
    const int px = slot / C::PS, cs = slot - C::PS * (slot / C::PS);
    const int hy = px / C::HWD, hx = px - (px / C::HWD) * C::HWD;
    hgeo[q] = (cs < CP8 && cs * 8 < p.c && px < C::HR * C::HWD) ? (hy << 16) | (hx << 4) | cs : -1;
  }
  const unsigned xrow = (unsigned)p.x_ld * 2u;
  const unsigned long long xbytes =
      ((unsigned long long)p.n * p.ih * p.iw - 1) * (unsigned long long)p.x_ld * 2ull + (unsigned long long)p.c * 2ull;
  const __amdgpu_buffer_rsrc_t rx = __builtin_amdgcn_make_buffer_rsrc((void*)p.x, 0, (int)xbytes, 0x00020000);
  struct TP {
    int n, y0, x0;
  };
  auto decode = [&](int t) {
    TP q;
    q.x0 = (t % tiles_x) * 64;
    const int r = t / tiles_x;
    q.y0 = (r % tiles_y) * C::WP;
    q.n = r / tiles_y;
    return q;
  };
  auto halo_issue = [&](const TP& T, int hb) {
    char* dst = smem + hb * C::HSZ + wave * 1024;
    const int ybase = T.y0 + p.dy0, xbase = T.x0 + p.dx0;
#pragma unroll
    for (int q = 0; q < C::NPC; ++q) {
      const int gq = hgeo[q];
      const int iy = ybase + (gq >> 16), ix = xbase + ((gq >> 4) & 0xFFF);
      const bool ok = gq >= 0 && (unsigned)iy < (unsigned)p.ih && (unsigned)ix < (unsigned)p.iw;
      const unsigned o = ok ? (unsigned)((T.n * p.ih + iy) * p.iw + ix) * xrow + (unsigned)(gq & 15) * 16u : OOB;
      __builtin_amdgcn_raw_ptr_buffer_load_lds(rx, (lds_ptr_t)(dst + q * C::NW * 1024), 16, o, 0, 0, 0);
    }
  };

  const int b_base = ((wp * C::HWD + r32) * C::PS) * 16;
  TP cur = decode(tile0);
  halo_issue(cur, 0);
  if constexpr (PRE) {
    const int co0 = cb * 64 + 32 * wc + 8 * hh;
    const unsigned long long yspan =
        ((unsigned long long)p.n * p.yh * p.yw - 1) * (unsigned long long)p.y_ld * 2ull + (unsigned long long)p.cout * 2ull;
    const __amdgpu_buffer_rsrc_t ry = __builtin_amdgcn_make_buffer_rsrc(p.y, 0, (int)yspan, 0x00020000);
    const __amdgpu_buffer_rsrc_t rr = __builtin_amdgcn_make_buffer_rsrc(
        (void*)p.res, 0,
        p.res ? (int)(((unsigned long long)p.n * p.yh * p.yw - 1) * (unsigned long long)p.res_ld * 2ull + p.cout * 2ull) : 0,
        0x00020000);
    const __amdgpu_buffer_rsrc_t rz = __builtin_amdgcn_make_buffer_rsrc(
        (void*)p.z, 0,
        p.dact ? (int)(((unsigned long long)p.n * p.yh * p.yw - 1) * (unsigned long long)p.z_ld * 2ull + p.cout * 2ull) : 0,
        0x00020000);
    const int nops = (p.res ? 1 : 0) + (p.beta ? 1 : 0) + (p.dact ? 1 : 0);
    auto offs = [&](const TP& T, int b, int P, unsigned& oy_, unsigned& or_, unsigned& oz_) {
      const int oy = T.y0 + wp, ox = T.x0 + 32 * b + r32, co = co0 + 16 * P;
      const bool ok = oy < p.oh && ox < p.ow && co < p.cout;
      const long long pix = ((long long)T.n * p.yh + oy * p.osy + p.ory) * p.yw + ox * p.osx + p.orx;
      oy_ = ok ? (unsigned)((pix * p.y_ld + co) * 2) : OOB;
      or_ = ok ? (unsigned)((pix * p.res_ld + co) * 2) : OOB;
      oz_ = ok ? (unsigned)((pix * p.z_ld + co) * 2) : OOB;
    };
    i32x4 er[2][2], eb[2][2], ez[2][2];
    auto prefetch = [&](const TP& T) {
#pragma unroll
      for (int b = 0; b < 2; ++b)
#pragma unroll
        for (int P = 0; P < 2; ++P) {
          unsigned o_y, o_r, o_z;
          offs(T, b, P, o_y, o_r, o_z);
          if (p.res) er[b][P] = __builtin_bit_cast(i32x4, __builtin_amdgcn_raw_buffer_load_b128(rr, o_r, 0, 0));
          if (p.beta) eb[b][P] = __builtin_bit_cast(i32x4, __builtin_amdgcn_raw_buffer_load_b128(ry, o_y, 0, 0));
          if (p.dact) ez[b][P] = __builtin_bit_cast(i32x4, __builtin_amdgcn_raw_buffer_load_b128(rz, o_z, 0, 0));
        }
    };
    f32x4 bia[2][2];
#pragma unroll
    for (int P = 0; P < 2; ++P) {
      const int co = co0 + 16 * P;
      bia[P][0] = p.bias && co < p.cout ? *(const f32x4*)(p.bias + co) : f32x4{0.f, 0.f, 0.f, 0.f};
      bia[P][1] = p.bias && co < p.cout ? *(const f32x4*)(p.bias + co + 4) : f32x4{0.f, 0.f, 0.f, 0.f};
    }
    prefetch(cur);
    __builtin_amdgcn_s_waitcnt(0);
    __syncthreads();
    int hb = 0;
    for (int tile = tile0; tile < n_tiles; tile += per_cb, hb ^= 1) {
      const bool has_next = tile + per_cb < n_tiles;
      const TP nxt = decode(has_next ? tile + per_cb : tile);
      halo_issue(nxt, hb ^ 1);
      f32x16 acc[2];
#pragma unroll
      for (int b = 0; b < 2; ++b)
#pragma unroll
        for (int e = 0; e < 16; ++e) acc[b][e] = 0.f;
      const char* H = smem + hb * C::HSZ + b_base;
#pragma unroll
      for (int sl = 0; sl < C::NS; ++sl) {
        i32x4 bf[2];
#pragma unroll
        for (int b = 0; b < 2; ++b) bf[b] = *(const i32x4*)(H + boff[sl] + 32 * b * C::PS * 16);
#pragma unroll
        for (int b = 0; b < 2; ++b)
          acc[b] = __builtin_amdgcn_mfma_f32_32x32x16_bf16(__builtin_bit_cast(bf16x8, wa[sl]), __builtin_bit_cast(bf16x8, bf[b]),
                                                           acc[b], 0, 0, 0);
      }
#pragma unroll
      for (int b = 0; b < 2; ++b) {
        float v[2][8];
#pragma unroll
        for (int P = 0; P < 2; ++P)
#pragma unroll
          for (int e = 0; e < 4; ++e) {
            const auto sw = __builtin_amdgcn_permlane32_swap(__float_as_uint(acc[b][8 * P + e]),
                                                             __float_as_uint(acc[b][8 * P + 4 + e]), false, false);
            v[P][e] = __uint_as_float(sw[0]) + bia[P][0][e];
            v[P][4 + e] = __uint_as_float(sw[1]) + bia[P][1][e];
          }
#pragma unroll
        for (int P = 0; P < 2; ++P) {
          float* w = v[P];
          if (p.res) add_bf16x8(w, er[b][P]);
          if (p.beta) add_bf16x8(w, eb[b][P]);
          act8(w, p.act, p.alpha);
          if (p.dact) dact_bf16x8(w, ez[b][P], p.dact, p.alpha);
          const i32x4 o = pack_bf16x8(w);
          unsigned o_y, o_r, o_z;
          offs(cur, b, P, o_y, o_r, o_z);
          __builtin_amdgcn_raw_buffer_store_b128(__builtin_bit_cast(i32x4, o), ry, o_y, 0, 0);
        }
      }
      prefetch(nxt);
      wait_vmcnt(4 + 4 * nops);
      __builtin_amdgcn_s_barrier();
      cur = nxt;
    }
    __builtin_amdgcn_s_waitcnt(0);
    return;
  }
  __builtin_amdgcn_s_waitcnt(0);
  __syncthreads();
  int hb = 0;
  for (int tile = tile0; tile < n_tiles; tile += per_cb, hb ^= 1) {
    const bool has_next = tile + per_cb < n_tiles;
    const TP nxt = decode(has_next ? tile + per_cb : tile);
    if (has_next) halo_issue(nxt, hb ^ 1);
    f32x16 acc[2];
#pragma unroll
    for (int b = 0; b < 2; ++b)
#pragma unroll
      for (int e = 0; e < 16; ++e) acc[b][e] = 0.f;
    const char* H = smem + hb * C::HSZ + b_base;
#pragma unroll
    for (int sl = 0; sl < C::NS; ++sl) {
      i32x4 bf[2];
#pragma unroll
      for (int b = 0; b < 2; ++b) bf[b] = *(const i32x4*)(H + boff[sl] + 32 * b * C::PS * 16);
#pragma unroll
      for (int b = 0; b < 2; ++b)
        acc[b] = __builtin_amdgcn_mfma_f32_32x32x16_bf16(__builtin_bit_cast(bf16x8, wa[sl]), __builtin_bit_cast(bf16x8, bf[b]),
                                                         acc[b], 0, 0, 0);
    }
    __builtin_amdgcn_s_waitcnt(0);
    __builtin_amdgcn_s_barrier();
#pragma unroll
    for (int b = 0; b < 2; ++b)
      ws_epilogue<OUTF32>(p, acc[b], cur.n, cur.y0 + wp, cur.x0 + 32 * b + r32, cb * 64 + 32 * wc + 8 * hh);
    cur = nxt;
  }
}

static bool nk_pre_on() {
  const char* e = getenv("DVIE_NK_PRE");
  return !(e && *e == '0');
}

template <int CP8>
static void launch_nk(const dvie_conv_desc& p, hipStream_t s) {
  typedef NkCfg<CP8> C;
  const int tiles_x = (p.ow + 63) / 64, tiles_y = (p.oh + C::WP - 1) / C::WP;
  const int n_tiles = tiles_x * tiles_y * p.n;
  const int n_cb = (p.cout + 63) / 64;
  int per_cb = 512 / n_cb;
  if (per_cb < 1) per_cb = 1;
  if (per_cb > n_tiles) per_cb = n_tiles;
  const int grid = per_cb * n_cb;
  const unsigned long long opix = (unsigned long long)p.n * p.yh * p.yw - 1;
  const bool spans_ok = (opix * p.y_ld + p.cout) * 2ull < 0xFFFFFF00ull &&
                        (!p.res || (opix * p.res_ld + p.cout) * 2ull < 0xFFFFFF00ull) &&
                        (!p.dact || (opix * p.z_ld + p.cout) * 2ull < 0xFFFFFF00ull);
  if (p.out_f32)
    DVIE_LAUNCH((conv_nk_kernel<CP8, true>), dim3(grid), dim3(512), 0, s, p, n_cb, n_tiles, tiles_x, tiles_y);
  else if (nk_pre_on() && spans_ok && (p.res || p.beta || p.dact))
    DVIE_LAUNCH((conv_nk_kernel<CP8, false, true>), dim3(grid), dim3(512), 0, s, p, n_cb, n_tiles, tiles_x, tiles_y);
  else
    DVIE_LAUNCH((conv_nk_kernel<CP8, false>), dim3(grid), dim3(512), 0, s, p, n_cb, n_tiles, tiles_x, tiles_y);
}

struct H8 {
  static constexpr int NW = 8, NTH = 512;
  static constexpr int BC = 128, PR = 8, KC = 32;
  static constexpr int HR = PR + 2, HWD = 66, PITCH = 80;
  static constexpr int HSLOTS = HR * HWD * 5;
  static constexpr int NHI = ((HSLOTS + 63) / 64 + NW - 1) / NW * NW;
  static constexpr int NHQ = NHI / NW;
  static constexpr int HSZ = NHI * 1024;
  static constexpr int ASZ = BC * KC * 2;
  static constexpr int WSZ = 3 * ASZ;
  static constexpr int SMEM = 2 * HSZ + 2 * WSZ;
  static constexpr int H0 = 4;
};
static_assert(H8::SMEM <= 163840, "conv_h8 LDS budget");
static_assert(H8::NHQ == 7 && H8::H0 < H8::NHQ, "halo shares");

template <int EPI>
__global__ __launch_bounds__(512) void conv_h8_kernel(const dvie_conv_desc p, int n_ct, int n_tiles, int tiles_x,
                                                      int tiles_y) {
  typedef H8 C;
  __shared__ __attribute__((aligned(1024))) char smem[C::SMEM];
  const int tid = threadIdx.x, lane = tid & 63;
  const int wave = __builtin_amdgcn_readfirstlane(tid >> 6);
  const int wc = wave >> 2, wp = wave & 3;
  const int r32 = lane & 31, hh = lane >> 5;
  const int nchunks = p.c >> 5;
  const unsigned OOB = 0xFFFFFFF0u;

  const int G = gridDim.x, g = blockIdx.x & 7, jb = blockIdx.x >> 3;
  const int nbg = G / 8 + (g < G % 8 ? 1 : 0);
  const int q8 = n_tiles / 8, r8 = n_tiles % 8;
  const int ts = g < r8 ? g * (q8 + 1) : r8 * (q8 + 1) + (g - r8) * q8;
  const int tile0 = ts + jb, tile_end = ts + q8 + (g < r8 ? 1 : 0);
  if (tile0 >= tile_end) return;

  auto tile_job = [&](int t) {
    JobInfo J;
    J.t = t;
    J.k = 0;
    J.valid = t < tile_end;
    J.c0 = (t % n_ct) * C::BC;
    int pt = t / n_ct;
    J.x0 = (pt % tiles_x) * 64;
    pt /= tiles_x;
    J.y0 = (pt % tiles_y) * C::PR;
    J.n = pt / tiles_y;
    return J;
  };
  auto next_job = [&](const JobInfo& J) {
    if (J.k + 1 < nchunks) {
      JobInfo N = J;
      N.k = J.k + 1;
      return N;
    }
    return tile_job(J.t + nbg);
  };

  int hgeo[C::NHQ];
#pragma unroll
  for (int q = 0; q < C::NHQ; ++q) {
    const int slot = (wave + C::NW * q) * 64 + lane;
    const int hr = slot / 5, cs = slot - 5 * (slot / 5);
    const int hy = hr / C::HWD, hx = hr - (hr / C::HWD) * C::HWD;
    hgeo[q] = (cs < 4 && hr < C::HR * C::HWD) ? (hy << 16) | (hx << 4) | cs : -1;
  }
  const int arow = wave * 16 + (lane >> 2);
  const unsigned aoff = (unsigned)arow * (unsigned)p.kpad * 2u + (unsigned)((((lane & 3) ^ ((arow >> 2) & 3))) * 16);
  const unsigned xrow = (unsigned)p.x_ld * 2u;
  const unsigned long long xbytes =
      ((unsigned long long)p.n * p.ih * p.iw - 1) * (unsigned long long)p.x_ld * 2ull + (unsigned long long)p.c * 2ull;
  const unsigned wbytes = (unsigned)p.cout * (unsigned)p.kpad * 2u;

  char* const Hs = smem;
  char* const As = smem + 2 * C::HSZ;

  auto halo_issue = [&](const JobInfo& J, int hb, int qa, int qb) {
    const int nrec = J.valid ? (int)(xbytes - (unsigned long long)J.k * 64) : 0;
    const __amdgpu_buffer_rsrc_t r =
        __builtin_amdgcn_make_buffer_rsrc((void*)((const char*)p.x + (size_t)J.k * 64), 0, nrec, 0x00020000);
    char* dst = Hs + hb * C::HSZ + wave * 1024;
    const int ybase = J.y0 + p.dy0, xbase = J.x0 + p.dx0;
#pragma unroll
    for (int q = qa; q < qb; ++q) {
      const int gq = hgeo[q];
      const int iy = ybase + (gq >> 16), ix = xbase + ((gq >> 4) & 0xFFF);
      const bool ok = gq >= 0 && (unsigned)iy < (unsigned)p.ih && (unsigned)ix < (unsigned)p.iw;
      const unsigned o = ok ? (unsigned)((J.n * p.ih + iy) * p.iw + ix) * xrow + (unsigned)(gq & 15) * 16u : OOB;
      __builtin_amdgcn_raw_ptr_buffer_load_lds(r, (lds_ptr_t)(dst + q * C::NW * 1024), 16, o, 0, 0, 0);
    }
  };
  auto a_issue = [&](const JobInfo& J, int v, int ab, int ti) {
    const __amdgpu_buffer_rsrc_t r = __builtin_amdgcn_make_buffer_rsrc((void*)p.w, 0, J.valid ? (int)wbytes : 0, 0x00020000);
    const unsigned so = (unsigned)(J.c0 * p.kpad + (ti * 3 + v) * p.c + 32 * J.k) * 2u;
    __builtin_amdgcn_raw_ptr_buffer_load_lds(r, (lds_ptr_t)(As + ab * C::WSZ + ti * C::ASZ + wave * 1024), 16, aoff, so, 0,
                                             0);
  };

  const int arw = wc * 64 + r32;
  const int a_s0 = arw * 64 + (((0 + hh) ^ ((arw >> 2) & 3)) << 4);
  const int a_s1 = arw * 64 + (((2 + hh) ^ ((arw >> 2) & 3)) << 4);
  const int b_base = (2 * wp * C::HWD + r32) * C::PITCH + hh * 16;

  f32x16 acc[2][2][2];

  {
    const JobInfo J0 = tile_job(tile0);
    halo_issue(J0, 0, 0, C::NHQ);
#pragma unroll
    for (int ti = 0; ti < 3; ++ti) a_issue(J0, 0, 0, ti);
    __builtin_amdgcn_s_waitcnt(0);
    __syncthreads();
  }

  int hb = 0, ab = 0;
  JobInfo J = tile_job(tile0);
  JobInfo J1 = next_job(J);
  i32x4 pa[2], pb[2][2];
  auto load_p0 = [&](const char* A0, const char* H0, int v0) {
#pragma unroll
    for (int i = 0; i < 2; ++i) pa[i] = *(const i32x4*)(A0 + a_s0 + i * 2048);
#pragma unroll
    for (int r = 0; r < 2; ++r)
#pragma unroll
      for (int b = 0; b < 2; ++b) pb[r][b] = *(const i32x4*)(H0 + (r * C::HWD + 32 * b + v0) * C::PITCH);
  };
  load_p0(As, Hs + b_base, 0);
  while (J.valid) {
    if (J.k == 0) {
#pragma unroll
      for (int i = 0; i < 2; ++i)
#pragma unroll
        for (int r = 0; r < 2; ++r)
#pragma unroll
          for (int b = 0; b < 2; ++b)
#pragma unroll
            for (int e = 0; e < 16; ++e) acc[i][r][b][e] = 0.f;
    }
    const char* H = Hs + hb * C::HSZ + b_base;
    const bool tile_end_job = J.k + 1 == nchunks;
#pragma unroll
    for (int v = 0; v < 3; ++v) {
      const char* A = As + ab * C::WSZ;
      const JobInfo& JW = v < 2 ? J : J1;
      const int vw = v < 2 ? v + 1 : 0;
      i32x4 af[2][3][2], bf[2][4][2];
      auto load_a = [&](int s, int ti) {
#pragma unroll
        for (int i = 0; i < 2; ++i) af[s][ti][i] = *(const i32x4*)(A + (s ? a_s1 : a_s0) + ti * C::ASZ + i * 2048);
      };
      auto load_b = [&](int s, int row) {
#pragma unroll
        for (int b = 0; b < 2; ++b) bf[s][row][b] = *(const i32x4*)(H + (row * C::HWD + 32 * b + v) * C::PITCH + s * 32);
      };
#pragma unroll
      for (int i = 0; i < 2; ++i) af[0][0][i] = pa[i];
#pragma unroll
      for (int r = 0; r < 2; ++r)
#pragma unroll
        for (int b = 0; b < 2; ++b) bf[0][r][b] = pb[r][b];
#pragma unroll
      for (int ph = 0; ph < 6; ++ph) {
        const int s = ph / 3, ti = ph % 3;
        if (ph < 5) {
          const int s2 = (ph + 1) / 3, t2 = (ph + 1) % 3;
          load_a(s2, t2);
          if (t2 == 0) {
            load_b(s2, 0);
            load_b(s2, 1);
          } else {
            load_b(s2, t2 + 1);
          }
        }
        if (ph < 3) a_issue(JW, vw, ab ^ 1, ph);
        if (v == 0 && ph == 3) halo_issue(J1, hb ^ 1, 0, 2);
        if (v == 0 && ph == 4) halo_issue(J1, hb ^ 1, 2, 3);
        if (v == 0 && ph == 5) halo_issue(J1, hb ^ 1, 3, C::H0);
        if (v == 1 && ph == 3) halo_issue(J1, hb ^ 1, C::H0, C::H0 + 1);
        if (v == 1 && ph == 4) halo_issue(J1, hb ^ 1, C::H0 + 1, C::H0 + 2);
        if (v == 1 && ph == 5) halo_issue(J1, hb ^ 1, C::H0 + 2, C::NHQ);
        if (ph == 5) {
          if (v == 0)
            DVIE_VMCNT_LGKM0(C::H0);
          else if (v == 1)
            DVIE_VMCNT_LGKM0(C::NHQ - C::H0);
          else
            DVIE_VMCNT_LGKM0(0);
          __builtin_amdgcn_s_barrier();
          if (v < 2)
            load_p0(As + (ab ^ 1) * C::WSZ, H, v + 1);
          else if (!tile_end_job)
            load_p0(As + (ab ^ 1) * C::WSZ, Hs + (hb ^ 1) * C::HSZ + b_base, 0);
        }
        __builtin_amdgcn_sched_barrier(0);
#pragma unroll
        for (int i = 0; i < 2; ++i)
#pragma unroll
          for (int r = 0; r < 2; ++r)
#pragma unroll
            for (int b = 0; b < 2; ++b)
              acc[i][r][b] = __builtin_amdgcn_mfma_f32_32x32x16_bf16(__builtin_bit_cast(bf16x8, af[s][ti][i]),
                                                                     __builtin_bit_cast(bf16x8, bf[s][ti + r][b]),
                                                                     acc[i][r][b], 0, 0, 0);
        __builtin_amdgcn_sched_barrier(0);
      }
      ab ^= 1;
    }
    hb ^= 1;

    if (J.k + 1 == nchunks) {
      const long long pix0 = ((long long)J.n * p.yh + (long long)J.y0 * p.osy + p.ory) * p.yw + (long long)J.x0 * p.osx + p.orx;
      const __amdgpu_buffer_rsrc_t rr = __builtin_amdgcn_make_buffer_rsrc(
          (void*)((const bf16_t*)p.res + ((EPI & 1) ? pix0 * p.res_ld : 0)), 0, 0x7FFFFFF0, 0x00020000);
      const __amdgpu_buffer_rsrc_t rb =
          __builtin_amdgcn_make_buffer_rsrc((void*)((const bf16_t*)p.y + pix0 * p.y_ld), 0, 0x7FFFFFF0, 0x00020000);
      const __amdgpu_buffer_rsrc_t rz = __builtin_amdgcn_make_buffer_rsrc(
          (void*)((const bf16_t*)p.z + ((EPI & 4) ? pix0 * p.z_ld : 0)), 0, 0x7FFFFFF0, 0x00020000);
      i32x4 o_r[2][2], o_b[2][2], o_z[2][2];
      auto epi_load = [&](int gi) {
        const int i = gi & 1, r = gi >> 2, b = (gi >> 1) & 1, u = gi & 1;
#pragma unroll
          for (int P = 0; P < 2; ++P) {
            const int oy = J.y0 + 2 * wp + r, ox = J.x0 + 32 * b + r32;
            const int co = J.c0 + wc * 64 + 32 * i + 16 * P + 8 * hh;
            const bool ok = oy < p.oh && ox < p.ow;
            const long long dp = (long long)(2 * wp + r) * p.osy * p.yw + (long long)(32 * b + r32) * p.osx;
            if (EPI & 1) o_r[u][P] = __builtin_amdgcn_raw_buffer_load_b128(rr, ok ? (unsigned)((dp * p.res_ld + co) * 2) : OOB, 0, 0);
            if (EPI & 2) o_b[u][P] = __builtin_amdgcn_raw_buffer_load_b128(rb, ok ? (unsigned)((dp * p.y_ld + co) * 2) : OOB, 0, 0);
            if (EPI & 4) o_z[u][P] = __builtin_amdgcn_raw_buffer_load_b128(rz, ok ? (unsigned)((dp * p.z_ld + co) * 2) : OOB, 0, 0);
          }
      };
      if (EPI) epi_load(0);
#pragma unroll
      for (int gi = 0; gi < 8; ++gi) {
        const int i = gi & 1, r = gi >> 2, b = (gi >> 1) & 1, u = gi & 1;
        if (EPI && gi < 7) epi_load(gi + 1);
        __builtin_amdgcn_sched_barrier(0);
        {
          float v8[2][8];
#pragma unroll
          for (int P = 0; P < 2; ++P)
#pragma unroll
            for (int e = 0; e < 4; ++e) {
              const auto sw = __builtin_amdgcn_permlane32_swap(__float_as_uint(acc[i][r][b][8 * P + e]),
                                                               __float_as_uint(acc[i][r][b][8 * P + 4 + e]), false, false);
              v8[P][e] = __uint_as_float(sw[0]);
              v8[P][4 + e] = __uint_as_float(sw[1]);
            }
          const int oy = J.y0 + 2 * wp + r, ox = J.x0 + 32 * b + r32;
          const bool ok = oy < p.oh && ox < p.ow;
          const long long dp = (long long)(2 * wp + r) * p.osy * p.yw + (long long)(32 * b + r32) * p.osx;
#pragma unroll
          for (int P = 0; P < 2; ++P) {
            const int co = J.c0 + wc * 64 + 32 * i + 16 * P + 8 * hh;
            float* w = v8[P];
            if (p.bias) add_f32x8(w, p.bias + co);
            const i32x4 o = epi8_regs<(EPI & 1) != 0, (EPI & 2) != 0, (EPI & 4) != 0>(w, p, &o_r[u][P], &o_b[u][P], &o_z[u][P]);
            if (ok) __builtin_amdgcn_raw_buffer_store_b128(o, rb, (unsigned)((dp * p.y_ld + co) * 2), 0, 0);
          }
        }
        __builtin_amdgcn_sched_barrier(0);
      }
      load_p0(As + ab * C::WSZ, Hs + hb * C::HSZ + b_base, 0);
    }
    J = J1;
    J1 = next_job(J1);
  }
}

static bool h8_on() {
  const char* e = getenv("DVIE_CONV_H8");
  return !(e && *e == '0');
}

template <int EPI>
static void launch_h8(const dvie_conv_desc& p, hipStream_t s, int n_ct, int n_tiles, int tiles_x, int tiles_y) {
  const int grid = n_tiles > 256 ? 256 : n_tiles;
  DVIE_LAUNCH((conv_h8_kernel<EPI>), dim3(grid), dim3(H8::NTH), 0, s, p, n_ct, n_tiles, tiles_x, tiles_y);
}

static bool conv_h8_launch(const dvie_conv_desc& p, hipStream_t s) {
  if (!h8_on() || p.out_f32 || p.c % 32 != 0 || p.c < 64 || p.cout % 128 != 0) return false;
  const int n_ct = p.cout / H8::BC, tiles_x = (p.ow + 63) / 64, tiles_y = (p.oh + H8::PR - 1) / H8::PR;
  const long long nt = (long long)n_ct * tiles_x * tiles_y * p.n;
  if (nt < 224 || nt >= (1LL << 30)) return false;
  const int n_tiles = (int)nt;
  switch ((p.res ? 1 : 0) | (p.beta ? 2 : 0) | (p.dact ? 4 : 0)) {
#define DVIE_H8(EPI) \
  case EPI: launch_h8<EPI>(p, s, n_ct, n_tiles, tiles_x, tiles_y); break;
    DVIE_H8(0) DVIE_H8(1) DVIE_H8(2) DVIE_H8(3) DVIE_H8(4) DVIE_H8(5) DVIE_H8(6) DVIE_H8(7)
#undef DVIE_H8
  }
  return true;
}

bool conv_narrow_launch(const dvie_conv_desc& p, hipStream_t s);

bool conv_halo_ph4_launch(const dvie_conv_desc& p, hipStream_t s) {
  if (p.dtype != DVIE_BF16 || p.out_f32 || p.bias || p.phc <= 0 || p.phc % 32 != 0 || p.cout != 4 * p.phc) return false;
  if (p.th != 2 || p.tw != 2 || p.dy0 != 0 || p.dx0 != 0 || p.ddy != 1 || p.ddx != 1 || p.sy != 1 || p.sx != 1)
    return false;
  if (p.osy != 2 || p.osx != 2 || p.ory != 0 || p.orx != 0) return false;
  if (p.c % 64 != 0 && p.c > 64) return false;
  const unsigned long long pix = (unsigned long long)p.n * p.ih * p.iw;
  if (pix >= (1ull << 31) || ((pix - 1) * (unsigned long long)p.x_ld + (unsigned long long)p.c) * 2ull >= 0xFFFFFF00ull)
    return false;
  return p.cout % 128 != 0 ? try_halo<1, 2, 4, 2, 2, true>(p, s) : try_halo<2, 2, 4, 2, 2, true>(p, s);
}

bool conv_halo_launch(const dvie_conv_desc& p, hipStream_t s) {
  if (p.dtype != DVIE_BF16) return false;
  if (p.sy != 1 || p.sx != 1 || p.ddy != 1 || p.ddx != 1) return false;
  if (p.osy < 1 || p.osx < 1 || p.ory < 0 || p.orx < 0) return false;
  if (p.c % 64 != 0 && p.c > 64) return false;
  const bool t1 = p.th == 1 && p.tw == 1, t3 = p.th == 3 && p.tw == 3;
  const bool t22 = p.th == 2 && p.tw == 2, t12 = p.th == 1 && p.tw == 2, t21 = p.th == 2 && p.tw == 1;
  if (!t1 && !t3 && !t22 && !t12 && !t21) return false;
  const unsigned long long pix = (unsigned long long)p.n * p.ih * p.iw;
  if (pix >= (1ull << 31)) return false;
  if (((pix - 1) * (unsigned long long)p.x_ld + (unsigned long long)p.c) * 2ull >= 0xFFFFFF00ull) return false;
  if (t3 && p.c % 8 == 0 && p.c <= 24 && p.kpad >= 9 * p.c) {
    switch (p.c / 8) {
      case 1: launch_nk<1>(p, s); break;
      case 2: launch_nk<2>(p, s); break;
      default: launch_nk<3>(p, s); break;
    }
    return true;
  }
  if (t3 && p.c <= 64 && p.cout <= 64 && (long long)p.n * p.oh * p.ow >= 65536) {
    switch ((p.c + 15) / 16) {
      case 1: if (!launch_strip<1>(p, s)) launch_ws<1>(p, s); break;
      case 2: if (!launch_strip<2>(p, s)) launch_ws<2>(p, s); break;
      case 3: if (!launch_strip<3>(p, s)) launch_ws<3>(p, s); break;
      default: if (!launch_strip<4>(p, s)) launch_ws<4>(p, s); break;
    }
    return true;
  }
  if (t3 && conv_narrow_launch(p, s)) return true;
  if (t3 && conv_h8_launch(p, s)) return true;
  int cfg;
  if (p.cout <= 32)
    cfg = 2;
  else if (t1)
    cfg = p.cout <= 64 ? 3 : (p.c <= 64 ? 5 : 4);
  else
    cfg = (p.cout <= 64 || p.cout % 128 != 0) ? 3 : 4;
  if (t3 && cfg == 4 && (long long)(p.cout / 128) * ((p.ow + 63) / 64) * ((p.oh + 3) / 4) * p.n < 256) cfg = 5;
  if (t3) return launch_cfg<3, 3>(cfg, p, s);
  if (t1) return launch_cfg<1, 1>(cfg, p, s);
  const int c2 = p.cout <= 64 || p.cout % 128 != 0 ? 3 : 4;
  if (t22) return launch_cfg2<2, 2>(c2, p, s);
  if (t12) return launch_cfg2<1, 2>(c2, p, s);
  return launch_cfg2<2, 1>(c2, p, s);
}

}
```

deep_video_interpolation_extrapolation_amd/engine.py:

```python
import ctypes
import os
from typing import NamedTuple, Optional

import torch

from . import _lib as L

PADC = 8
PROFILE = None
DEBUG_NAN = bool(os.environ.get("DVIE_DEBUG_NAN"))
def _wgrad_lane():
    return os.environ.get("DVIE_WGRAD_LANE", "1") != "0"


OP_HOOK = None


def pack_blocks(d):
    n = L.load().dvie_pack_blocks(ctypes.byref(d))
    assert n > 0, "dvie_pack_blocks: empty pack descriptor"
    return n


def _reduce_meta(name, r):
# ... 468 lines not shown
        self.n_l1 += 1
        self._add(op)
        return op.idx

    def output(self, key, region, channels):
        self.outputs[key] = (region, channels)

    def segenc_chain(self, ops):
        self.segenc.append(tuple(ops))

    def _add(self, op):
        self.ops.append(op)
        if op.out is not None:
            op.out.buf.producers.append(op)
        for r in op.inputs():
            r.buf.consumers.append((op, r))

    def compile(self, n_fwd, device, n_bwd=None, backward=True, alias=False):
        return Plan(self, n_fwd, n_fwd if n_bwd is None else n_bwd, device, backward, alias)


ARENA_ALIGN = 512


def segenc_fusable(dtype, nf, ops):
    if dtype != torch.bfloat16 or os.environ.get("DVIE_SEGENC_FUSED", "1") == "0":
        return False
    o0, o1, o2 = ops
    acts = (L.ACT_ELU, L.ACT_ELU, L.ACT_NONE)
    chans = ((24, 32), (32, 32), (32, 8))
    for op, act, (ci, co) in zip(ops, acts, chans):
        lay = op.layer
        if not (isinstance(op, ConvOp) and op.act == act and op.res is None and lay.kh == 3 and lay.kw == 3
                and lay.stride == 1 and lay.pad == 1 and lay.dil == 1 and lay.has_bias and op.x.c == ci
                and op.out.c == co and lay.cout_p == co):
            return False
    if not (o1.x.buf is o0.out.buf and o2.x.buf is o1.out.buf and o0.out.c0 == 0 and o1.out.c0 == 0):
        return False
    if o0.out.buf.C != 32 or o1.out.buf.C != 32 or o2.out.buf.external:
        return False
    x = o0.x
    return nf * x.H * x.W * x.buf.C * 2 < 0xFFFFFF00


def forward_launches(g, nf):
    fused_first, skip = {}, set()
    if os.environ.get("DVIE_SEGENC_FWD", "1") == "1":
        for chain in g.segenc:
            if segenc_fusable(g.dtype, nf, chain):
                fused_first[id(chain[0])] = chain
                skip.update(id(op) for op in chain[1:])
    return [list(fused_first.get(id(op), (op,))) for op in g.ops if id(op) not in skip]


def _op_regions(op):
    rs = list(op.inputs())
    for r in (op.out, getattr(op, "region", None)):
        if r is not None:
            rs.append(r)
    return rs


def forward_lifetimes(g, nf):
    life = {}
    for i, ops in enumerate(forward_launches(g, nf)):
        for op in ops:
            for r in _op_regions(op):
                a, b = life.get(id(r.buf), (i, i))
                life[id(r.buf)] = (min(a, i), max(b, i))
    for r in g.caller_written.values():
        life[id(r.buf)] = (0, life.get(id(r.buf), (0, 0))[1])
    return life


def assign_offsets(items):
    size = [rup(max(int(b), 1), ARENA_ALIGN) for b, _, _ in items]
    order = sorted(range(len(items)), key=lambda i: (-size[i], items[i][1], i))
    offsets = [0] * len(items)
    placed = []
    arena = 0
    for i in order:
        _, f, l = items[i]
        busy = sorted((offsets[j], offsets[j] + size[j]) for j in placed if items[j][1] <= l and f <= items[j][2])
        off = 0
        for lo, hi in busy:
            if off + size[i] <= lo:
                break
            off = max(off, hi)
        offsets[i] = off
        placed.append(i)
        arena = max(arena, off + size[i])
    if arena > sum(size):
        offsets, arena = [], 0
        for sz in size:
            offsets.append(arena)
            arena += sz
    return offsets, arena


def arena_layout(g, nf):
    life = forward_lifetimes(g, nf)
    n_sites = max([b for _, b in life.values()] + [0])
    bufs = [b for b in g.buffers if not b.external]
    items = []
    for b in bufs:
        nbytes = nf * b.H * b.W * b.C * elem_size(b.dtype or g.dtype)
        items.append((nbytes,) + life.get(id(b), (0, n_sites)))
    offsets, arena = assign_offsets(items)
    return {id(b): o for b, o in zip(bufs, offsets)}, arena, sum(it[0] for it in items)


class Plan:

    def __init__(self, g, nf, nb, device, backward, alias=False):
        assert not (alias and backward), "alias=True is for forward-only plans (a backward reads every activation)"
        self.g, self.nf, self.nb, self.device, self.alias = g, nf, nb, device, alias
        self.dtype = g.dtype
        self.dt = dv_dtype(g.dtype)
        self.es = elem_size(g.dtype)
        self.vec = 16 // self.es
        self.backward_enabled = backward
        self.keep = []
        self.busy = False
        self.generation = 0
        self.static_weights = False
        self._pack_srcs, self._pack_sig, self._pack_descs = [], None, []
        self.arena, self.arena_bytes, self.unaliased_bytes = None, None, 0
        self.l1_out = self.bn_partial = None
        self.bn_splits = 1
        self._seg_bwd, self._seg_inner = {}, set()
        self.fwd = []
        self.bwd = []
        self.fwd_arr = self.bwd_arr = None
        self.fwd_off = self.n_bwd = 0
        self._l1_fwd = []
        self._l1_bwd = []
        self.ext_in = {}
        self.ext_out = {}
        self.ext_mask = {}
        self.ext_nchw_out = {}
        self.ext_head = {}
        self.ext_head_grad = {}
        self.keep_grad = None
        self.ext_grad = {}
        self._grad_slots = []
        self.ext_ograd = {}
        self.wg_first = {}
        self._uses_left = {}
        self.completions = []
        self._multi = []
        self._i2c = None
        self.ws = None
        self.ws_floats = 1
        self._alloc()
        self._build_pack()
        self._build_forward()
        if backward:
            self._build_backward()
        assert all(o.lane == 0 for o in self.fwd), "forward ops run on the caller's stream"
        self._finalize()

    def _alloc(self):
        g = self.g
        offsets, self.arena_bytes, self.unaliased_bytes = arena_layout(g, self.nf) if self.alias else ({}, None, 0)
        if self.alias:
            self.arena = torch.empty(max(self.arena_bytes, ARENA_ALIGN), dtype=torch.uint8, device=self.device)
            self.keep.append(self.arena)
        for b in g.buffers:
            dt = b.dtype or self.dtype
            b.dt = dt
            if b.external:
                b.t = None
            elif self.alias:
                nbytes = self.nf * b.H * b.W * b.C * elem_size(dt)
                o = offsets[id(b)]
                b.t = self.arena[o:o + nbytes].view(dt).view(self.nf, b.H, b.W, b.C)
            else:
                b.t = torch.empty((self.nf, b.H, b.W, b.C), dtype=dt, device=self.device)
                self.unaliased_bytes += b.t.numel() * b.t.element_size()
        if self.backward_enabled:
            for op in g.ops:
                if op.out is None:
                    continue
                need = False
                if isinstance(op, InputOp):
                    need = op.requires_grad
                elif isinstance(op, (ConvOp, ConvTOp)):
                    need = op.layer.trainable or any(r.buf.needs_grad for r in op.inputs())
                elif isinstance(op, BNOp):
                    need = op.trainable or op.x.buf.needs_grad
                elif isinstance(op, FuseOp) and op.detach:
                    need = False
                else:
                    need = any(r.buf.needs_grad for r in op.inputs())
                op.out.buf.needs_grad = op.out.buf.needs_grad or need
            self._seg_bwd = self._segenc_bwd_chains()
            self._seg_inner = {id(op.out.buf) for ch in self._seg_bwd.values() for op in ch[:2]}
            for b in g.buffers:
                if b.needs_grad and id(b) not in self._seg_inner:
                    b.g = torch.zeros((self.nb, b.H, b.W, b.C), dtype=self.dtype, device=self.device)
            for b in g.buffers:
                b.expected, b.pending = {}, {}
                b.n_flushed = 0
                b.done = b.dact_done = False
            for op in g.ops:
                if isinstance(op, FuseOp) and op.detach:
                    continue
                for r in op.inputs():
                    if r.buf.needs_grad:
                        r.buf.expected[r.key()] = r.buf.expected.get(r.key(), 0) + 1
            for b in g.buffers:
                keys = sorted(b.expected)
                for (a0, ac), (b0, _) in zip(keys, keys[1:]):
                    assert a0 + ac <= b0, f"{b}: consumers read overlapping regions {keys}"
        self.l1_out = torch.zeros(max(1, g.n_l1), dtype=torch.float32, device=self.device)
        self.keep.append(self.l1_out)
        for op in g.ops:
            if isinstance(op, BNOp):
                d = L.BnDesc()
                d.rows = self.nf * op.x.H * op.x.W
                self.bn_splits = max(self.bn_splits, L.load().dvie_bn_partial_splits(ctypes.byref(d)))
                d.rows = self.nb * op.x.H * op.x.W
                self.bn_splits = max(self.bn_splits, L.load().dvie_bn_partial_splits(ctypes.byref(d)))
                op.stats = torch.zeros((8, op.x.c), dtype=torch.float32, device=self.device)
                self.keep.append(op.stats)
        maxc = max([op.x.c for op in g.ops if isinstance(op, BNOp)] + [4])
        self.bn_partial = torch.zeros(self.bn_splits * 2 * maxc, dtype=torch.float64, device=self.device)
        self.keep.append(self.bn_partial)

    def ptr(self, region, n0=0, grad=False):
        b = region.buf
        t = b.g if grad else b.t
        es = elem_size(t.dtype)
        return t.data_ptr() + (n0 * b.H * b.W * b.C + region.c0) * es

    def _build_pack(self):
        descs = []
        self._pack_srcs = [t for lay in self.g.layers if lay.cin_p is not None
                           for t in (lay.m.weight, lay.m.bias if lay.has_bias else None) if t is not None]
        self._pack_sig = None
        for lay in self.g.layers:
            if lay.cin_p is None:
                continue
            K = lay.kh * lay.kw * lay.cin_p
            kpad = rup(K, 64)
            lay.kpad = kpad
            lay.wf = torch.zeros((lay.cout_p, kpad), dtype=self.dtype, device=self.device)
            cmap_t = torch.tensor(lay.cmap, dtype=torch.int32, device=self.device)
            lay.cmap_t = cmap_t
            self.keep += [lay.wf, cmap_t]
            ft = lay.fwd_taps()
            descs.append(self._pack_desc(lay, lay.wf, lay.cout_p, kpad, lay.cin_p, 0, ft, cmap_t))
            if lay.has_bias:
                nbias, rows = (lay.cin, lay.cin_p) if lay.transposed else (lay.cout, lay.cout_p)
                lay.bias_p = torch.zeros(rows, dtype=torch.float32, device=self.device)
                self.keep.append(lay.bias_p)
                d = L.PackDesc()
                d.src, d.dst, d.cmap = lay.m.bias.data_ptr(), lay.bias_p.data_ptr(), None
                d.rows, d.kpad, d.c, d.mode = rows, 1, 1, 0
                d.th, d.tw, d.kh0, d.kw0, d.dkh, d.dkw = 1, 1, 0, 0, 1, 1
                d.cout_s, d.cin_s, d.kh_s, d.kw_s, d.dtype = nbias, 1, 1, 1, L.F32
                descs.append(d)
            lay.wd = []
            lay.wd4 = None
        self._pack_descs = descs

    def _pack_desc(self, lay, dst, rows, kpad, c, mode, taps, cmap_t):
        if isinstance(lay.m, StackedConv):
            assert lay.m.contiguous(), f"{lay.name}: stacked parts are not consecutive in memory"
        d = L.PackDesc()
        d.src, d.dst, d.cmap = lay.m.weight.data_ptr(), dst.data_ptr(), cmap_t.data_ptr()
        d.rows, d.kpad, d.c, d.mode = rows, kpad, c, mode
        d.th, d.tw, d.kh0, d.kw0, d.dkh, d.dkw = taps["th"], taps["tw"], taps["kh0"], taps["kw0"], taps["dkh"], taps["dkw"]
        d.cout_s, d.cin_s, d.kh_s, d.kw_s, d.dtype = lay.cout, lay.cin, lay.kh, lay.kw, self.dt
        return d

    def _dgrad_weights(self, lay, H, W):
        key = (H, W)
        for k, v in lay.wd:
            if k == key:
                return v
        out = []
        for ph in lay.dgrad_phases(H, W):
            kpad = rup(ph["th"] * ph["tw"] * lay.cout_p, 64)
            t = torch.zeros((lay.cin_p, kpad), dtype=self.dtype, device=self.device)
            self.keep.append(t)
            self._pack_descs.append(self._pack_desc(lay, t, lay.cin_p, kpad, lay.cout_p, 1, ph, lay.cmap_t))
            out.append((ph, t, kpad))
        lay.wd.append((key, out))
        return out

    PH4_ORDER = ((0, 0), (1, 1), (0, 1), (1, 0))

    def _ph4_eligible(self, lay, x):
        return (self.dtype == torch.bfloat16 and os.environ.get("DVIE_PH4", "1") != "0" and lay.stride == 2
                and lay.kh == 3 and lay.kw == 3 and lay.pad == 1 and lay.dil == 1 and not lay.transposed
                and x.c == lay.cin_p and lay.cin_p % 32 == 0 and lay.cin_p <= 128
                and (lay.cout_p % 64 == 0 or lay.cout_p < 64))

    def _dgrad_weights_ph4(self, lay):
        if lay.wd4 is not None:
            return lay.wd4
        kpad = rup(4 * lay.cout_p, 64)
        t = torch.zeros((4 * lay.cin_p, kpad), dtype=self.dtype, device=self.device)
        self.keep.append(t)
        for q, (a, b) in enumerate(self.PH4_ORDER):
            taps = dict(th=2, tw=2, kh0=a + 1, kw0=b + 1, dkh=-2, dkw=-2)
            self._pack_descs.append(self._pack_desc(lay, t[q * lay.cin_p:(q + 1) * lay.cin_p], lay.cin_p, kpad,
                                                    lay.cout_p, 1, taps, lay.cmap_t))
        lay.wd4 = (t, kpad)
        return lay.wd4

    def _op(self, kind):
        o = L.Op()
        o.kind = kind
        o.ws_base, o.ws_off, o.bws_off, o.ws_ptr = 0, 0, None, None
        o.l1_seed = None
        return o

    def conv_desc(self, x_ptr, x_ld, n, ih, iw, c, w_ptr, kpad, cout, oh, ow, sy, sx, taps, y_ptr, y_ld, yh, yw,
                  osy=1, osx=1, ory=0, orx=0, bias=None, res=None, res_ld=0, z=None, z_ld=0, act=0, dact=0, beta=0,
                  out_f32=False):
        o = self._op(L.OP_CONV)
        d = o.u.conv
        d.x, d.w, d.y, d.bias, d.res, d.z = x_ptr, w_ptr, y_ptr, bias, res, z
        d.x_ld, d.y_ld, d.res_ld, d.z_ld = x_ld, y_ld, res_ld, z_ld
        d.n, d.ih, d.iw, d.c, d.kpad, d.cout = n, ih, iw, c, kpad, cout
        d.oh, d.ow, d.sy, d.sx = oh, ow, sy, sx
        d.th, d.tw, d.dy0, d.dx0, d.ddy, d.ddx = taps["th"], taps["tw"], taps["dy0"], taps["dx0"], taps["ddy"], taps["ddx"]
        d.yh, d.yw, d.osy, d.osx, d.ory, d.orx = yh, yw, osy, osx, ory, orx
        d.act, d.dact, d.beta, d.dtype, d.out_f32 = act, dact, beta, self.dt, int(out_f32)
        d.alpha = 0.2
        return o

    def ew_desc(self, op, n, h, w, c, y_ptr, y_ld, srcs=(), res=None, res_ld=0, z=None, z_ld=0, act=0, dact=0,
                beta=0, scale=1.0):
        o = self._op(L.OP_EW)
        d = o.u.ew
        d.op, d.n, d.h, d.w, d.c = op, n, h, w, c
        d.y, d.y_ld = y_ptr, y_ld
        d.nsrc = len(srcs)
        for i, (p, ld, sh, sw) in enumerate(srcs):
            setattr(d, f"src{i}", p)
            setattr(d, f"src_ld{i}", ld)
            setattr(d, f"sh{i}", sh)
            setattr(d, f"sw{i}", sw)
        d.res, d.res_ld, d.z, d.z_ld = res, res_ld, z, z_ld
        d.act, d.dact, d.beta, d.dtype = act, dact, beta, self.dt
        d.alpha, d.scale = 0.2, scale
        npx = n * h * w
        nbytes = self.es * c * (npx * (1 + int(bool(beta)) + int(res is not None) + int(z is not None))
                                + sum(n * sh * sw for (_, _, sh, sw) in srcs))
        o.meta = dict(cls="pointwise", name=f"ew{op} {n}x{h}x{w}x{c} src{len(srcs)}"
                      + ("+res" if res is not None else "") + ("+acc" if beta else "") + ("+z" if z is not None else ""),
                      flops=0.0, bytes=float(nbytes))
        return o

    def _part(self, part):
        if part is None:
            return 0, self.nf
        return (0 if part == 0 else self.nf // 2), self.nf // 2

    def _segenc_fwd(self, ops):
        o0, o1, o2 = ops
        x, nf = o0.x, self.nf
        o = self._op(L.OP_SEGENC_FWD)
        d = o.u.segenc
        d.inp, d.e1, d.e2, d.out = self.ptr(x), self.ptr(o0.out), self.ptr(o1.out), self.ptr(o2.out)
        d.in_ld, d.e1_ld, d.e2_ld, d.out_ld = x.buf.C, o0.out.buf.C, o1.out.buf.C, o2.out.buf.C
        d.w0, d.w2, d.w4 = o0.layer.wf.data_ptr(), o1.layer.wf.data_ptr(), o2.layer.wf.data_ptr()
        d.b0, d.b2, d.b4 = o0.layer.bias_p.data_ptr(), o1.layer.bias_p.data_ptr(), o2.layer.bias_p.data_ptr()
        d.n, d.h, d.w = nf, x.H, x.W
        d.kpad0, d.kpad2, d.kpad4 = o0.layer.kpad, o1.layer.kpad, o2.layer.kpad
        npx = nf * x.H * x.W
        o.meta = dict(cls="conv_fwd", name="seg_encoder (fused)",
                      flops=2.0 * npx * 9 * sum(op.layer.cout * op.layer.cin for op in ops),
                      bytes=float(self.es * npx * (x.c + 32 + 32 + 8)))
        return o

    def _build_forward(self):
        for site in forward_launches(self.g, self.nf):
            if len(site) > 1:
                self.fwd.append(self._segenc_fwd(tuple(site)))
                continue
            lower = self._FWD.get(type(site[0]))
            if lower is None:
                raise TypeError(site[0])
            lower(self, site[0])

    def _label_input_fwd(self, op):
        o = self.ew_desc(L.EW_LABELS, self.nf, op.out.H, op.out.W, op.out.c, self.ptr(op.out), op.out.buf.C)
        o.u.ew.ext_c = op.ext_c
        self.ext_in.setdefault(op.key, []).append((len(self.fwd), op))
        self.fwd.append(o)

    def _input_fwd(self, op):
        n0, cnt = self._part(op.part)
        o = self.ew_desc(L.EW_NCHW, cnt, op.out.H, op.out.W, op.out.c, self.ptr(op.out, n0), op.out.buf.C)
        o.u.ew.ext_c = op.ext_c
        if op.normalize:
            m = torch.tensor(_IMAGENET_MEAN + [0.0] * 5, dtype=torch.float32, device=self.device)
            s = torch.tensor(_IMAGENET_STD + [1.0] * 5, dtype=torch.float32, device=self.device)
            self.keep += [m, s]
            o.u.ew.mean, o.u.ew.std = m.data_ptr(), s.data_ptr()
            op.std_t = s
        self.ext_in.setdefault(op.key, []).append((len(self.fwd), op))
        self.fwd.append(o)

    def _conv_fwd(self, op):
        lay, x, out, nf = op.layer, op.x, op.out, self.nf
        ext = out.buf.external
        o = self.conv_desc(
            self.ptr(x), x.buf.C, nf, x.H, x.W, x.c, lay.wf.data_ptr(), lay.kpad, lay.cout_p, out.H, out.W,
            lay.stride, lay.stride, lay.fwd_taps(), 0 if ext else self.ptr(out), out.buf.C, out.H, out.W,
            bias=lay.bias_p.data_ptr() if lay.has_bias else None,
            res=self.ptr(op.res) if op.res is not None else None,
            res_ld=op.res.buf.C if op.res is not None else 0, act=op.act,
            out_f32=(out.buf.dt == torch.float32 and self.dtype != torch.float32))
        npx = nf * out.H * out.W
        o.meta = dict(cls="conv_fwd", name=lay.name,
                      flops=2.0 * npx * lay.cout * lay.cin * lay.kh * lay.kw,
                      bytes=float(self.es * (nf * x.H * x.W * lay.cin + npx * lay.cout * (2 if op.res is not None else 1)
                                             + lay.cout * lay.cin * lay.kh * lay.kw)))
        if ext:
            self.ext_out.setdefault(out.buf.name, []).append((len(self.fwd), out))
        self.fwd.append(o)

    def _convT_fwd(self, op):
        lay, x, out, nf = op.layer, op.x, op.out, self.nf
        assert not out.buf.external
        for ph, wt, kpad in self._dgrad_weights(lay, out.H, out.W):
            o = self.conv_desc(
                self.ptr(x), x.buf.C, nf, x.H, x.W, lay.cout_p, wt.data_ptr(), kpad, out.c, ph["oh"], ph["ow"],
                1, 1, ph, self.ptr(out), out.buf.C, out.H, out.W, osy=lay.stride, osx=lay.stride,
                ory=ph["ry"], orx=ph["rx"], bias=lay.bias_p.data_ptr() if lay.has_bias else None, act=op.act,
                out_f32=(out.buf.dt == torch.float32 and self.dtype != torch.float32))
            npx = nf * ph["oh"] * ph["ow"]
            o.meta = dict(cls="conv_fwd", name=lay.name, flops=2.0 * npx * lay.cout * lay.cin * ph["th"] * ph["tw"],
                          bytes=float(self.es * (nf * x.H * x.W * lay.cout + npx * lay.cin)))
            self.fwd.append(o)

    def _fuse_fwd(self, op):
        out = op.out
        srcs = [(self.ptr(s), s.buf.C, s.H, s.W) for s in op.srcs]
        o = self.ew_desc(L.EW_FUSE, self.nf, out.H, out.W, out.c, self.ptr(out), out.buf.C, srcs, act=op.act)
        o.u.ew.align = int(op.align)
        self.fwd.append(o)

    def _mask_fwd(self, op):
        out, src = op.out, op.src
        o = self.ew_desc(L.EW_MASK, self.nf, out.H, out.W, out.c, self.ptr(out), out.buf.C,
                         [(self.ptr(src), src.buf.C, src.H, src.W)])
        o.u.ew.ext_c = int(op.inverse)
        self.ext_mask.setdefault(op.key, []).append(("fwd", len(self.fwd), op))
        self.fwd.append(o)

    def _out_nchw_fwd(self, op):
        r = op.region
        o = self.ew_desc(L.EW_TONCHW, self.nf, r.H, r.W, r.c, 0, 0, [(self.ptr(r), r.buf.C, r.H, r.W)])
        o.u.ew.ext_c = op.channels
        if op.clamp:
            o.u.ew.align, o.u.ew.scale = 1, float(op.clamp)
        self.ext_nchw_out[op.key] = len(self.fwd)
        self.fwd.append(o)

    def _pool_fwd(self, op):
        x, out = op.x, op.out
        self.fwd.append(self.ew_desc(L.EW_POOL, self.nf, out.H, out.W, out.c, self.ptr(out), out.buf.C,
                                     [(self.ptr(x), x.buf.C, x.H, x.W)]))

    def _bn_fwd(self, op):
        o = self._op(L.OP_BN_FWD)
        self._bn_common(o.u.bn, op, self.nf)
        o.u.bn.y, o.u.bn.y_ld = self.ptr(op.out), op.out.buf.C
        self.fwd.append(o)

    def _head_fwd(self, op):
        x = op.x
        o = self._op(L.OP_HEAD_FWD)
        d = o.u.head
        d.x, d.x_ld = self.ptr(x), x.buf.C
        d.n, d.h, d.w, d.c, d.pool, d.dtype = self.nf, x.H, x.W, x.c, op.pool, self.dt
        rows = self.nf * (x.H // op.pool) * (x.W // op.pool)
        op.pooled = torch.zeros(rows * x.c, dtype=torch.float32, device=self.device)
        self.keep.append(op.pooled)
        d.pooled = op.pooled.data_ptr()
        self.ext_head[op.key] = (len(self.fwd), rows)
        self.fwd.append(o)

    def _l1feat_fwd(self, op):
        a = op.a
        half = self.nf // 2
        o = self._op(L.OP_LOSS)
        d = o.u.loss
        d.a, d.b = self.ptr(a, 0), self.ptr(a, half)
        sn, sh, sw = a.H * a.W * a.buf.C, a.W * a.buf.C, a.buf.C
        d.a_sn, d.a_sc, d.a_sh, d.a_sw = sn, 1, sh, sw
        d.b_sn, d.b_sc, d.b_sh, d.b_sw = sn, 1, sh, sw
        d.kind, d.bsz, d.ch, d.h, d.w, d.dtype = L.LOSS_L1NHWC, half, a.c, a.H, a.W, self.dt
        d.weight, d.out_scale = 1.0, 1.0
        npart = L.load().dvie_loss_partial_count(ctypes.byref(d))
        part = torch.zeros(max(1, npart), dtype=torch.float64, device=self.device)
        self.keep.append(part)
        d.partial = part.data_ptr()
        d.out = self.l1_out.data_ptr() + 4 * op.idx
        self._l1_fwd.append((len(self.fwd), op.idx))
        self.fwd.append(o)

    _ATTN_FWD = {"l2norm": L.ATTN_L2NORM, "corr": L.ATTN_CORR, "softmax": L.ATTN_SOFTMAX, "wnorm": L.ATTN_WNORM,
                 "gather": L.ATTN_GATHER, "pool": L.ATTN_POOL}

    def attn_desc(self, kind, n, region_hw, c, a, a_ld, y, y_ld, b0=None, b1=None, b_ld=0, wh=1, ww=1, nhalf=1,
                  half0=0, res=None, res_ld=0, z=None, z_ld=0, dact=0, beta=0):
        o = self._op(L.OP_ATTN)
        d = o.u.attn
        d.op, d.n, d.h, d.w, d.c = kind, n, region_hw[0], region_hw[1], c
        d.a, d.a_ld, d.y, d.y_ld, d.b0, d.b1, d.b_ld = a, a_ld, y, y_ld, b0, b1, b_ld
        d.wh, d.ww, d.nhalf, d.half0 = wh, ww, nhalf, half0
        d.res, d.res_ld, d.z, d.z_ld, d.dact, d.beta = res, res_ld, z, z_ld, dact, beta
        d.dtype, d.alpha = self.dt, 0.2
        return o

    def _attn_fwd(self, op):
        a, out = op.a, op.out
        bs = [self.ptr(b) for b in op.bs] + [None, None]
        b_ld = op.bs[0].buf.C if op.bs else 0
        if len(op.bs) == 2:
            assert op.bs[1].buf.C == b_ld, "attn: target maps need one pixel stride"
        o = self.attn_desc(self._ATTN_FWD[op.kind], self.nf, (out.H, out.W), op.c, self.ptr(a), a.buf.C,
                           self.ptr(out), out.buf.C, bs[0], bs[1], b_ld, op.wh, op.ww, op.nhalf, op.half0)
        npx = self.nf * out.H * out.W
        o.meta = dict(cls="attn", name=f"{op.kind}:{out.buf.name}", flops=0.0,
                      bytes=float(self.es * npx * (a.c + sum(b.c for b in op.bs) + out.c)))
        self.fwd.append(o)

    def _attn_backward(self, op, gout, gld):
        nb = self.nb
        a, out = op.a, op.out
        hw = (out.H, out.W)
        K = op.wh * op.ww
        ld_a = a.buf.C

        npx = nb * out.H * out.W
        J = op.nhalf * K
        cb = sum(b.c for b in op.bs)
        moved = {"l2norm": 4 * op.c, "softmax": 3 * J, "wnorm": 4 * J, "pool": 2 * op.c,
                 "corr": op.c + J + cb, "gather": out.c + J + cb}[op.kind]

        def contrib(region, build):
            if region.buf.needs_grad:
                def emit(epi):
                    o = build(epi._asdict())
                    o.meta = dict(cls="attn_bwd", name=f"{op.kind}:{region.buf.name}", flops=0.0,
                                  bytes=float(self.es * npx * moved))
                    return [o]
                self._contrib(region, emit)

        if op.kind == "l2norm":
            contrib(a, lambda e: self.attn_desc(L.ATTN_L2NORM_BWD, nb, hw, op.c, gout, gld, self.ptr(a, grad=True),
                                                ld_a, self.ptr(out), self.ptr(a), self._same_ld(out, a), **e))
        elif op.kind == "softmax":
            contrib(a, lambda e: self.attn_desc(L.ATTN_SOFTMAX_BWD, nb, hw, op.c, gout, gld, self.ptr(a, grad=True),
                                                ld_a, self.ptr(out), None, out.buf.C, op.wh, op.ww, op.nhalf, **e))
        elif op.kind == "wnorm":
            contrib(a, lambda e: self.attn_desc(L.ATTN_WNORM_BWD, nb, hw, op.c, gout, gld, self.ptr(a, grad=True),
                                                ld_a, self.ptr(out), self.ptr(a), self._same_ld(out, a), op.wh,
                                                op.ww, op.nhalf, **e))
        elif op.kind == "pool":
            contrib(a, lambda e: self.attn_desc(L.ATTN_POOL_T, nb, hw, op.c, gout, gld, self.ptr(a, grad=True), ld_a,
                                                wh=op.wh, ww=op.ww, **e))
        elif op.kind == "corr":
            bs = op.bs
            bp = [self.ptr(b) for b in bs] + [None]
            contrib(a, lambda e: self.attn_desc(L.ATTN_GATHER, nb, hw, op.c, gout, gld, self.ptr(a, grad=True), ld_a,
                                                bp[0], bp[1], bs[0].buf.C, op.wh, op.ww, op.nhalf, 0, **e))
            for m, b in enumerate(bs):
                contrib(b, lambda e, m=m, b=b: self.attn_desc(
                    L.ATTN_GATHER_T, nb, hw, op.c, gout, gld, self.ptr(b, grad=True), b.buf.C, self.ptr(a), None,
                    ld_a, op.wh, op.ww, op.nhalf, m, **e))
        elif op.kind == "gather":
            fs = op.bs
            maps = [None] * op.nhalf
            for m, f in enumerate(fs):
                maps[op.half0 + m] = self.ptr(f)
            assert op.nhalf <= 2
            maps += [None]
            contrib(a, lambda e: self.attn_desc(L.ATTN_CORR, nb, hw, out.c, gout, gld, self.ptr(a, grad=True), ld_a,
                                                maps[0], maps[1], fs[0].buf.C, op.wh, op.ww, op.nhalf, **e))
            for m, f in enumerate(fs):
                contrib(f, lambda e, m=m, f=f: self.attn_desc(
                    L.ATTN_GATHER_T, nb, hw, out.c, self.ptr(a), ld_a, self.ptr(f, grad=True), f.buf.C, gout, None,
                    gld, op.wh, op.ww, op.nhalf, op.half0 + m, **e))
        else:
            raise TypeError(op.kind)

    @staticmethod
    def _same_ld(r0, r1):
        assert r0.buf.C == r1.buf.C, f"attn backward: {r0.buf} and {r1.buf} need one pixel stride"
        return r0.buf.C

    def _bn_common(self, d, op, n):
        x, m = op.x, op.m
        d.x, d.x_ld = self.ptr(x), x.buf.C
        d.rows, d.c = n * x.H * x.W, x.c
        d.splits = L.load().dvie_bn_partial_splits(ctypes.byref(d))
        d.partial, d.stats = self.bn_partial.data_ptr(), op.stats.data_ptr()
        d.gamma = m.weight.data_ptr() if m.weight is not None else None
        d.beta = m.bias.data_ptr() if m.bias is not None else None
        d.running_mean = m.running_mean.data_ptr() if m.running_mean is not None else None
        d.running_var = m.running_var.data_ptr() if m.running_var is not None else None
        assert m.num_features == x.c or rup(m.num_features, PADC) == x.c
        assert m.num_features == x.c, "BatchNorm channel count must be a multiple of 8"
        d.training = int(self.g.bn_training)
        d.act, d.alpha, d.eps = op.act, 0.2, m.eps
        d.x_f32 = int(x.buf.dt == torch.float32 and self.dtype != torch.float32)
        d.momentum = m.momentum if m.momentum is not None else 0.0
        d.dtype = self.dt

    def _contrib(self, region, emitter, ident=None):
        b = region.buf
        key = region.key()
        assert key in b.expected, (b, key)
        pend = b.pending.setdefault(key, [])
        pend.append((emitter, ident))
        if len(pend) == b.expected[key]:
            self._flush(b, key)

    def _flush(self, b, key):
        c0, c = key
        region = Region(b, c0, c)
        pending = b.pending.pop(key)
        kernels = [e for e, i in pending if e is not None]
        idents = [i for e, i in pending if e is None]
        prod = b.producers
        fuse_dact = False
        if len(prod) == 1 and prod[0].act != L.ACT_NONE and prod[0].out.buf is b:
            o0, oc = prod[0].out.c0, prod[0].out.c
            fuse_dact = (all(o0 <= k0 and k0 + kc <= o0 + oc for k0, kc in b.expected) and
                         sum(kc for _, kc in b.expected) == oc)
        b.dact_done = fuse_dact
        dact = prod[0].act if fuse_dact else 0
        z = self.ptr(region) if fuse_dact else None
        if fuse_dact:
            assert b.dt == self.dtype
        seq = []
        k = 0
        for em in kernels:
            r = idents[k] if k < len(idents) else None
            k += 1 if r is not None else 0
            seq.append((em, r))
        rest = idents[k:]
        gptr, gld = self.ptr(region, grad=True), b.C

        def copy_em(a):
            return lambda epi: [self.ew_desc(L.EW_COPY, self.nb, b.H, b.W, c, gptr, gld, [(a[0], a[1], b.H, b.W)],
                                             **epi._asdict())]

        while rest:
            a = rest.pop(0)
            seq.append((copy_em(a), rest.pop(0) if rest else None))
        for i, (em, r) in enumerate(seq):
            epi = Epilogue(beta=0 if i == 0 else 1, res=r[0] if r else None, res_ld=r[1] if r else 0)
            if i == len(seq) - 1:
                epi = epi._replace(dact=dact, z=z, z_ld=b.C)
            self.bwd.extend(em(epi))
        b.n_flushed += 1
        b.done = b.n_flushed == len(b.expected)

    def _ensure_dact(self, op):
        b = op.out.buf
        if op.act == L.ACT_NONE or b.dact_done:
            return
        out = op.out
        gp = self.ptr(out, grad=True)
        self.bwd.append(self.ew_desc(L.EW_COPY, self.nb, out.H, out.W, out.c, gp, b.C, [(gp, b.C, out.H, out.W)],
                                     z=self.ptr(out), z_ld=b.C, dact=op.act))

    def _segenc_bwd_chains(self):
        out = {}
        if os.environ.get("DVIE_SEGENC_FUSED", "1") == "0":
            return out
        for chain in self.g.segenc:
            o0, o1, o2 = chain
            if not segenc_fusable(self.dtype, self.nf, chain) or o0.x.buf.needs_grad:
                continue
            if not all(op.layer.trainable for op in chain):
                continue
            if len(o0.out.buf.consumers) != 1 or len(o1.out.buf.consumers) != 1:
                continue
            if self.nb * o0.x.H * o0.x.W * max(o2.out.buf.C, 32) * 2 >= 0xFFFFFF00:
                continue
            out[id(o2)] = chain
        return out

    def _segenc_backward(self, chain, gout, gld):
        o0, o1, o2 = chain
        x, nb = o0.x, self.nb
        slabs = 256
        bufs = {k: torch.empty(slabs * n, dtype=torch.float32, device=self.device) for k, n in
                (("dw4", 8 * 288), ("dw2", 32 * 288), ("dw0", 32 * 216), ("db4", 8), ("db2", 32), ("db0", 32))}
        self.keep += list(bufs.values())
        (_, w4d, kpad4), = self._dgrad_weights(o2.layer, x.H, x.W)
        (_, w2d, kpad2), = self._dgrad_weights(o1.layer, x.H, x.W)
        o = self._op(L.OP_SEGENC_BWD)
        d = o.u.segenc_bwd
        d.dout, d.e2, d.e1, d.inp = gout, self.ptr(o1.out), self.ptr(o0.out), self.ptr(x)
        d.dout_ld, d.e2_ld, d.e1_ld, d.in_ld = gld, o1.out.buf.C, o0.out.buf.C, x.buf.C
        d.w4d, d.w2d, d.kpad4, d.kpad2 = w4d.data_ptr(), w2d.data_ptr(), kpad4, kpad2
        for k in ("dw4", "dw2", "dw0", "db4", "db2", "db0"):
            setattr(d, k, bufs[k].data_ptr())
        d.n, d.h, d.w, d.slabs = nb, x.H, x.W, slabs
        npx = nb * x.H * x.W
        o.meta = dict(cls="conv_wgrad", name="seg_encoder (fused backward)",
                      flops=2.0 * npx * 9 * (2 * o2.layer.cout * o2.layer.cin + 2 * o1.layer.cout * o1.layer.cin
                                             + o0.layer.cout * o0.layer.cin),
                      bytes=float(self.es * npx * (8 + 32 + 32 + x.c)))
        self.bwd.append(o)
        for op, wk, bk in ((o2, "dw4", "db4"), (o1, "dw2", "db2"), (o0, "dw0", "db0")):
            self._reduce_op(op.layer, "weight", slabs, 9 * op.x.c, op.x.c, own=bufs[wk])
            self._reduce_op(op.layer, "bias", slabs, own=bufs[bk])
            self._close_layer(op.layer)
        for op in (o0, o1):
            op.out.buf.done = True
            op.out.buf.dact_done = True
            op.out.buf.pending = {}

    def _build_backward(self):
        g = self.g
        seg_bwd = self._seg_bwd
        seg_skip = {id(op) for ch in seg_bwd.values() for op in ch[:2]}
        for op in g.ops:
            if isinstance(op, (ConvOp, ConvTOp)) and op.layer.trainable:
                self._uses_left[op.layer] = self._uses_left.get(op.layer, 0) + 1
        for key, (region, ch) in g.outputs.items():
            b = region.buf
            assert b.needs_grad and not b.expected
            assert b.t is not None or all(p.act == L.ACT_NONE for p in b.producers), "external output with activation"
            o = self.ew_desc(L.EW_NCHW, self.nb, region.H, region.W, region.c, self.ptr(region, grad=True), b.C)
            o.u.ew.ext_c = ch
            self.ext_ograd[key] = len(self.bwd)
            self.bwd.append(o)
            b.done = True
            b.dact_done = all(p.act == L.ACT_NONE for p in b.producers)
        for op in reversed(g.ops):
            lower = self._BWD.get(type(op))
            if lower is None:
                raise TypeError(op)
            out = op.out
            if out is None:
                lower(self, op, None, 0)
                continue
            b = out.buf
            if not b.needs_grad or not b.done:
                continue
            if id(op) in seg_skip:
                continue
            self._ensure_dact(op)
            gout, gld = self.ptr(out, grad=True), b.C
            if id(op) in seg_bwd:
                self._segenc_backward(seg_bwd[id(op)], gout, gld)
            else:
                lower(self, op, gout, gld)
        for bf in g.buffers:
            if bf.needs_grad and bf.expected and not bf.done:
                raise RuntimeError(f"incomplete gradient for {bf}: pending {({k: len(v) for k, v in bf.pending.items()})}"
                                   f" of {bf.expected}")

    def _out_nchw_backward(self, op, gout, gld):
        pass

    def _head_backward(self, op, gout, gld):
        x = op.x
        if not x.buf.needs_grad:
            return
        xg = self.ptr(x, grad=True)

        def em(epi):
            assert epi.res is None and epi.dact == 0, "head backward has no fused epilogue"
            o = self._op(L.OP_HEAD_BWD)
            d = o.u.head
            d.gx, d.gx_ld = xg, x.buf.C
            d.n, d.h, d.w, d.c, d.pool, d.dtype, d.beta = self.nb, x.H, x.W, x.c, op.pool, self.dt, epi.beta
            self.ext_head_grad[op.key] = len(self.bwd)
            return [o]

        self._contrib(x, em)

    def _l1feat_backward(self, op, gout, gld):
        a = op.a
        if not a.buf.needs_grad:
            return
        numel = (self.nf // 2) * a.H * a.W * a.c
        ap, bp, ld = self.ptr(a, 0), self.ptr(a, self.nf // 2), a.buf.C
        gp = self.ptr(a, grad=True)
        scale = op.weight / numel

        def em(epi):
            o = self.ew_desc(L.EW_L1SIGN, self.nb, a.H, a.W, a.c, gp, ld, [(ap, ld, a.H, a.W), (bp, ld, a.H, a.W)],
                             scale=scale, **epi._asdict())
            o.l1_seed = scale
            return [o]

        self._contrib(a, em)

    def _input_backward(self, op, gout, gld):
        if not op.requires_grad:
            return
        out = op.out
        o = self.ew_desc(L.EW_TONCHW, self.nb, out.H, out.W, out.c, 0, 0, [(gout, gld, out.H, out.W)])
        o.u.ew.ext_c = op.ext_c
        if op.normalize:
            o.u.ew.std = op.std_t.data_ptr()
        self.ext_grad.setdefault(op.key, []).append((len(self.bwd), op))
        self.bwd.append(o)

    def _bn_backward(self, op, gout, gld):
        x = op.x
        assert len(x.buf.consumers) == 1, "BatchNorm input must have no other reader"
        if not x.buf.needs_grad:
            return
        xg = self.ptr(x, grad=True)

        def em(epi):
            assert epi.res is None and epi.dact == 0, "BatchNorm backward has no fused epilogue"
            o = self._op(L.OP_BN_BWD)
            d = o.u.bn
            self._bn_common(d, op, self.nb)
            d.g, d.g_ld = gout, gld
            d.dx, d.dx_ld, d.beta_dx = xg, x.buf.C, epi.beta
            if op.trainable:
                self._grad_slots.append((len(self.bwd), op.m, "bn", op.m not in self.wg_first))
                self.wg_first[op.m] = True
            return [o]

        self._contrib(x, em)

    def _fuse_backward(self, op, gout, gld):
        if op.detach:
            return
        out = op.out

        def resize_t(s):
            sp = self.ptr(s, grad=True)

            def em(epi):
                o = self.ew_desc(L.EW_UPT, self.nb, s.H, s.W, s.c, sp, s.buf.C, [(gout, gld, out.H, out.W)],
                                 **epi._asdict())
                o.u.ew.align = int(op.align)
                return [o]
            return em

        for s in op.srcs:
            if not s.buf.needs_grad:
                continue
            if (s.H, s.W) == (out.H, out.W):
                self._contrib(s, None, ident=(gout, gld))
            else:
                self._contrib(s, resize_t(s))

    def _mask_backward(self, op, gout, gld):
        src, out = op.src, op.out
        if not src.buf.needs_grad:
            return
        sp = self.ptr(src, grad=True)

        def em(epi):
            o = self.ew_desc(L.EW_MASK, self.nb, src.H, src.W, src.c, sp, src.buf.C, [(gout, gld, out.H, out.W)],
                             **epi._asdict())
            o.u.ew.ext_c = int(op.inverse)
            self.ext_mask.setdefault(op.key, []).append(("bwd", len(self.bwd), op))
            return [o]

        self._contrib(src, em)

    def _pool_backward(self, op, gout, gld):
        x, out = op.x, op.out
        if not x.buf.needs_grad:
            return
        xp = self.ptr(x, grad=True)
        self._contrib(x, lambda epi: [self.ew_desc(L.EW_POOLT, self.nb, x.H, x.W, x.c, xp, x.buf.C,
                                                   [(gout, gld, out.H, out.W)], **epi._asdict())])

    def _head3_fusable(self, op, gld):
        lay, x, out = op.layer, op.x, op.out
        mode = os.environ.get("DVIE_HEAD3_FUSED", "1")
        if self.dtype != torch.bfloat16 or mode == "0" or (mode == "1" and lay.cout_p != 8):
            return False
        if os.environ.get("DVIE_IM2COL_DGRAD", "0") == "1":
            return False
        if not (lay.trainable and x.buf.needs_grad and op.res is None and lay.kh == 3 and lay.kw == 3
                and lay.stride == 1 and lay.pad == 1 and lay.dil == 1 and lay.cout_p in (8, 24)
                and x.c % 64 == 0 and (out.H, out.W) == (x.H, x.W)):
            return False
        if x.buf.expected.get(x.key(), 0) != 1 or lay.cmap_t is not None and lay.cin != x.c:
            return False
        npx = self.nb * x.H * x.W
        return npx * max(x.buf.C, gld) * 2 < 0xFFFFFF00

    def _emit_head3(self, op, gout, gld, phase, xg, dact):
        lay, x = op.layer, op.x
        ph, wt, kpad = phase
        splits = max(1, 256 // (x.c // 64))
        slabs = torch.empty(splits * lay.cout_p * 9 * x.c, dtype=torch.float32, device=self.device)
        self.keep.append(slabs)
        o = self._op(L.OP_HEAD3_BWD)
        d = o.u.head3
        d.g, d.h, d.wd, d.dh, d.ws = gout, self.ptr(x), wt.data_ptr(), xg, slabs.data_ptr()
        d.g_ld, d.h_ld, d.dh_ld = gld, x.buf.C, x.buf.C
        d.n, d.hgt, d.wid, d.c = self.nb, x.H, x.W, x.c
        d.cout, d.kpad, d.dy0, d.dx0 = lay.cout_p, kpad, ph["dy0"], ph["dx0"]
        d.splits, d.dact, d.alpha = splits, dact, 0.2
        npix = self.nb * x.H * x.W
        o.meta = dict(cls="conv_dgrad", name=lay.name + "+wgrad",
                      flops=2.0 * npix * lay.cout * lay.cin * 9 * 2,
                      bytes=float(self.es * (2 * npix * x.c + npix * lay.cout) + 4 * slabs.numel()))
        self.bwd.append(o)
        csplits = self._colsum_op(gout, gld, npix, lay.cout_p) if lay.has_bias else 0
        self._reduce_op(lay, "weight", splits, 9 * x.c, x.c, own=slabs)
        if lay.has_bias:
# ... 596 lines not shown
```

include/dvie.h:

```cpp
#ifndef DVIE_H
#define DVIE_H

#include <stddef.h>
#include <stdint.h>

#ifdef __cplusplus
extern "C" {
#endif

#define DVIE_OK 0
#define DVIE_EINVAL 1001

#define DVIE_F32 0
#define DVIE_BF16 1

#define DVIE_ACT_NONE 0
#define DVIE_ACT_LRELU 1
#define DVIE_ACT_ELU 2
#define DVIE_ACT_RELU 3
#define DVIE_ACT_TANH 4

typedef struct dvie_conv_desc {
  const void* x;
  const void* w;
  void* y;
  const float* bias;
  const void* res;
  const void* z;
  long long x_ld, y_ld, res_ld, z_ld;
  int n, ih, iw, c;
  int kpad, cout;
  int oh, ow, sy, sx;
  int th, tw, dy0, dx0, ddy, ddx;
  int yh, yw, osy, osx, ory, orx;
  int act, dact, beta, dtype;
  int out_f32;
  float alpha;
  int phc;
  int pad1;
} dvie_conv_desc;

int dvie_conv2d_fwd(const dvie_conv_desc* d, void* stream);

typedef struct dvie_wgrad_desc {
  const void* g;
  const void* x;
  float* ws;
  long long g_ld, x_ld;
  int n, oh, ow, cout;
  int ih, iw, c, sy;
  int sx, th, tw, dy0;
  int dx0, ddy, ddx, splits;
  int dtype;
  int tmap;
  float* bws;
  int ws_taps;
  int pad1;
} dvie_wgrad_desc;

int dvie_conv2d_wgrad(const dvie_wgrad_desc* d, void* stream);

int dvie_wgrad_bias_slabs(const dvie_wgrad_desc* d);

int dvie_wgrad_splits_hint(const dvie_wgrad_desc* d);

int dvie_wgrad_slabs(const dvie_wgrad_desc* d);

typedef struct dvie_wreduce_desc {
  const float* ws;
  float* dw;
  const int* cmap;
  int splits, ws_rows, ws_k, co_off;
  int cout_p, cin_p, kh_n, kw_n;
  int c, beta;
} dvie_wreduce_desc;

int dvie_wgrad_reduce(const dvie_wreduce_desc* d, void* stream);

int dvie_wgrad_reduce_multi(const dvie_wreduce_desc* descs, int n, void* stream);
typedef struct dvie_wreduce_multi_desc {
  const dvie_wreduce_desc* descs;
  int n, pad;
} dvie_wreduce_multi_desc;

typedef struct dvie_colsum_desc {
  const void* g;
  float* ws;
  long long g_ld;
  long long rows;
  int c, splits, dtype, pad0;
} dvie_colsum_desc;

int dvie_colsum(const dvie_colsum_desc* d, void* stream);

typedef struct dvie_pack_desc {
  const float* src;
  void* dst;
  const int* cmap;
  int rows, kpad, c, mode;
  int th, tw, kh0, kw0;
  int dkh, dkw, cout_s, cin_s;
  int kh_s, kw_s, dtype, blk0;
} dvie_pack_desc;

int dvie_pack_weights(const dvie_pack_desc* descs_dev, int n, int blocks, void* stream);

int dvie_pack_blocks(const dvie_pack_desc* d);

#define DVIE_EW_FUSE 0
#define DVIE_EW_UPT 1
#define DVIE_EW_POOL 2
#define DVIE_EW_POOLT 3
#define DVIE_EW_COPY 4
#define DVIE_EW_L1SIGN 5
#define DVIE_EW_NCHW 6
#define DVIE_EW_TONCHW 7
#define DVIE_EW_MASK 8
#define DVIE_EW_IM2COL 9
#define DVIE_EW_LABELS 10

typedef struct dvie_ew_desc {
  void* y;
  const void* src0;
  const void* src1;
  const void* src2;
  const void* res;
  const void* z;
  float* ext;
  const float* mean;
  const float* std;
  long long y_ld, src_ld0, src_ld1, src_ld2, res_ld, z_ld;
  long long sn, sc, sh, sw;
  int op, n, h, w;
  int c, nsrc, sh0, sw0;
  int sh1, sw1, sh2, sw2;
  int act, dact, beta, dtype;
  int ext_c, align;
  float alpha, scale;
} dvie_ew_desc;

int dvie_ew(const dvie_ew_desc* d, void* stream);

#define DVIE_LOSS_L1 0
#define DVIE_LOSS_GDL 1
#define DVIE_LOSS_SSIM 2
#define DVIE_LOSS_MSE 3
#define DVIE_LOSS_CE 4
#define DVIE_LOSS_L1NHWC 5
#define DVIE_LOSS_COSNHWC 6
#define DVIE_LOSS_IOU 7
#define DVIE_LOSS_ARGMAX_IOU 8

typedef struct dvie_loss_desc {
  const void* a;
  const void* b;
  float* grad;
  float* out;
  double* partial;
  float* ws;
  long long a_sn, a_sc, a_sh, a_sw;
  long long b_sn, b_sc, b_sh, b_sw;
  int kind, bsz, ch, h;
  int w, beta, dtype, out_acc;
  float weight, out_scale;
} dvie_loss_desc;

int dvie_loss(const dvie_loss_desc* d, void* stream);

int dvie_sum_f32(const float* x, int n, float* out, void* stream);
size_t dvie_loss_partial_count(const dvie_loss_desc* d);
size_t dvie_loss_ws_floats(const dvie_loss_desc* d);

typedef struct dvie_warp_desc {
  const float* img;
  const float* flow;
  float* out;
  const float* dout;
  float* dimg;
  float* dflow;
  float* ws;
  int n, c, h, w;
  int align_corners, pad0;
} dvie_warp_desc;

int dvie_warp_fwd(const dvie_warp_desc* d, void* stream);
int dvie_warp_bwd(const dvie_warp_desc* d, void* stream);
size_t dvie_warp_ws_floats(const dvie_warp_desc* d);

int dvie_adamax(float* p, const float* g, float* m, float* u, long long n, float clr,
                float b1, float b2, float eps, float wd, void* stream);

int dvie_step_inc(float* step, void* stream);
int dvie_adamax_dev(float* p, const float* g, float* m, float* u, long long n, double lr, double b1, double b2,
                    double eps, double wd, const float* step, void* stream);

// ... 307 lines not shown
```

Baseline: 256.5 frames/s.

## Store activation sign bitmaps in forward convs for backward dact epilogues

```diff
diff --git a/deep_video_interpolation_extrapolation_amd/_lib.py b/deep_video_interpolation_extrapolation_amd/_lib.py
--- a/deep_video_interpolation_extrapolation_amd/_lib.py
+++ b/deep_video_interpolation_extrapolation_amd/_lib.py
@@ -36,6 +36,7 @@
         ("yh", i32), ("yw", i32), ("osy", i32), ("osx", i32), ("ory", i32), ("orx", i32),
         ("act", i32), ("dact", i32), ("beta", i32), ("dtype", i32),
         ("out_f32", i32), ("alpha", f32), ("phc", i32), ("pad1", i32),
+        ("zbits", vp), ("zbits_ld", i64),
     ]
 
 
@@ -278,7 +279,7 @@
     "dvie_adam_dev", "dvie_mfma_probe", "dvie_launch_probe", "dvie_sum_f32", "dvie_wgrad_bias_slabs", "dvie_head3_bwd",
     "dvie_segenc_fwd", "dvie_segenc_bwd", "dvie_pack_blocks", "dvie_trace_kernels", "dvie_traced_kernels",
     "dvie_synth_load", "dvie_synth_finish", "dvie_synth_bridge", "dvie_synth_score", "dvie_synth_score_ws_bytes",
-    "dvie_synth_load_pad", "dvie_synth_finish_crop",
+    "dvie_synth_load_pad", "dvie_synth_finish_crop", "dvie_conv_zbits",
 ]
 
 _lib = None
@@ -323,7 +324,8 @@
         lib.dvie_trace_kernels.restype = i32
         lib.dvie_traced_kernels.argtypes = []
         lib.dvie_traced_kernels.restype = ctypes.c_char_p
-        for name in ("dvie_wgrad_splits_hint", "dvie_wgrad_slabs", "dvie_bn_partial_splits", "dvie_pack_blocks"):
+        for name in ("dvie_wgrad_splits_hint", "dvie_wgrad_slabs", "dvie_bn_partial_splits", "dvie_pack_blocks",
+                     "dvie_conv_zbits"):
             getattr(lib, name).argtypes = [vp]
             getattr(lib, name).restype = i32
         lib.dvie_run_ops.argtypes = [vp, i32, vp]
diff --git a/deep_video_interpolation_extrapolation_amd/csrc/conv1x1.hip b/deep_video_interpolation_extrapolation_amd/csrc/conv1x1.hip
--- a/deep_video_interpolation_extrapolation_amd/csrc/conv1x1.hip
+++ b/deep_video_interpolation_extrapolation_amd/csrc/conv1x1.hip
@@ -137,8 +137,22 @@
     if (k < nk) stage(k, k);
 
   static_assert(PRE == 0 || (NS == 1 && !OUTF32), "operand prefetch: single K-step, bf16 output");
-  i32x4 pr_r[(PRE & 1) ? MI : 1][TMC][2], pr_b[(PRE & 2) ? MI : 1][TMC][2], pr_z[(PRE & 4) ? MI : 1][TMC][2];
-  constexpr bool CEL = CE && (PRE & (PRE - 1)) != 0;
+  constexpr bool ZPROD = (PRE & 16) != 0;
+  static_assert(!ZPROD || ((TMC == 4 || TMC == 2) && MI == 1 && (PRE & 14) == 0), "bitmap writer: a forward");
+  constexpr bool ZB = (PRE & 8) != 0;
+  static_assert(!ZB || ((PRE & 4) != 0 && TMC == 4), "bitmap operand: 16 bytes per 128-channel wave tile");
+  i32x4 pr_r[(PRE & 1) ? MI : 1][TMC][2], pr_b[(PRE & 2) ? MI : 1][TMC][2], pr_z[((PRE & 4) && !ZB) ? MI : 1][TMC][2];
+  i32x4 pr_zb[ZB ? MI : 1];
+  if constexpr (ZB) {
+#pragma unroll
+    for (int i = 0; i < MI; ++i) {
+      const int pix = p0 + (wave % NWP) * 32 * MI + 32 * i + r32;
+      const long long q = pix < npix ? pix : 0;
+      pr_zb[i] = *(const i32x4*)((const char*)p.zbits + q * p.zbits_ld + ((c0 + (wave / NWP) * 32 * TMC) >> 3));
+    }
+  }
+  constexpr int STREAMS = (PRE & 3) | (ZB ? 0 : (PRE & 4));
+  constexpr bool CEL = CE && (STREAMS & (STREAMS - 1)) != 0;
   if constexpr (CEL) {
     const int wp0 = wave % NWP, wc0 = wave / NWP;
     const int a8 = r32 >> 3, bl = lane & 7;
@@ -152,10 +166,10 @@
         pr_r[0][k >> 1][k & 1] = ok ? *(const i32x4*)((const bf16_t*)p.res + q * p.res_ld + co) : i32x4{0, 0, 0, 0};
       if constexpr ((PRE & 2) != 0)
         pr_b[0][k >> 1][k & 1] = ok ? *(const i32x4*)((const bf16_t*)p.y + q * p.y_ld + co) : i32x4{0, 0, 0, 0};
-      if constexpr ((PRE & 4) != 0)
+      if constexpr ((PRE & 4) != 0 && !ZB)
         pr_z[0][k >> 1][k & 1] = ok ? *(const i32x4*)((const bf16_t*)p.z + q * p.z_ld + co) : i32x4{0, 0, 0, 0};
     }
-  } else if constexpr (PRE != 0) {
+  } else if constexpr ((PRE & 7) != 0) {
     const int wp0 = wave % NWP, wc0 = wave / NWP;
 #pragma unroll
     for (int i = 0; i < MI; ++i)
@@ -171,7 +185,7 @@
             pr_r[i][j][P] = ok ? *(const i32x4*)((const bf16_t*)p.res + q * p.res_ld + co) : i32x4{0, 0, 0, 0};
           if constexpr ((PRE & 2) != 0)
             pr_b[i][j][P] = ok ? *(const i32x4*)((const bf16_t*)p.y + q * p.y_ld + co) : i32x4{0, 0, 0, 0};
-          if constexpr ((PRE & 4) != 0)
+          if constexpr ((PRE & 4) != 0 && !ZB)
             pr_z[i][j][P] = ok ? *(const i32x4*)((const bf16_t*)p.z + q * p.z_ld + co) : i32x4{0, 0, 0, 0};
         }
   }
@@ -228,11 +242,12 @@
     };
     if constexpr ((PRE & 1) != 0) tr(pr_r[0]);
     if constexpr ((PRE & 2) != 0) tr(pr_b[0]);
-    if constexpr ((PRE & 4) != 0) tr(pr_z[0]);
+    if constexpr ((PRE & 4) != 0 && !ZB) tr(pr_z[0]);
   }
   i32x4 ob[CE ? 8 : 1];
 #pragma unroll
   for (int i = 0; i < MI; ++i) {
+  unsigned zq[2] = {0u, 0u};
   const int pix0 = p0 + wp * 32 * MI + 32 * i + r32;
   const int pix = CE ? min(pix0, npix - 1) : pix0;
   float v[TMC][2][8];
@@ -272,18 +287,44 @@
         }
         act8(w, p.act, p.alpha);
         if (p.dact) {
-          if constexpr ((PRE & 4) != 0)
+          if constexpr (ZB)
+            dact_bits8(w, ((unsigned)pr_zb[i][j] >> (8 * (2 * P + hh))) & 0xffu, p.dact, p.alpha);
+          else if constexpr ((PRE & 4) != 0)
             dact_bf16x8(w, pr_z[i][j][P], p.dact, p.alpha);
           else
             dact_bf16x8(w, *(const i32x4*)((const bf16_t*)p.z + yp * p.z_ld + co), p.dact, p.alpha);
         }
         const i32x4 o = pack_bf16x8(w);
+        if constexpr (ZPROD && !CE) zq[(2 * j + P) / TMC] |= sign_bits8(o) << (8 * ((2 * j + P) % TMC));
         if constexpr (CE)
           ob[2 * j + P] = o;
         else if (!(dbg & 1) || w[0] == 12345.678f)
           *(i32x4*)dst = o;
       }
     }
+  if constexpr (ZPROD) {
+    if constexpr (CE) {
+#pragma unroll
+      for (int k = 0; k < 2 * TMC; ++k) zq[k / TMC] |= sign_bits8(ob[k]) << (8 * (k % TMC));
+    }
+    {
+      const auto sw = __builtin_amdgcn_permlane32_swap(zq[0], zq[1], false, false);
+      const unsigned ev = sw[0], od = sw[1];
+      const unsigned z0 = (ev & 0xffu) | ((od & 0xffu) << 8) | ((ev & 0xff00u) << 8) | ((od & 0xff00u) << 16);
+      const int cz = c0 + wc * 32 * TMC + 16 * TMC * hh;
+      char* zdst = (char*)p.zbits + yp * p.zbits_ld + (cz >> 3);
+      if (pix0 < npix && cz < p.cout) {
+        if constexpr (TMC == 4) {
+          i32x2 zo;
+          zo[0] = (int)z0;
+          zo[1] = (int)(((ev >> 16) & 0xffu) | ((od >> 8) & 0xff00u) | ((ev >> 8) & 0xff0000u) | (od & 0xff000000u));
+          *(i32x2*)zdst = zo;
+        } else {
+          *(unsigned*)zdst = z0;
+        }
+      }
+    }
+  }
   }
   if constexpr (CE) {
     transpose8x8(ob, lane);
@@ -445,7 +486,7 @@
   __builtin_amdgcn_s_waitcnt(0);
 }
 
-template <int TMC, int NWP, int MI, int NWC, int ACT, int AB = 0>
+template <int TMC, int NWP, int MI, int NWC, int ACT, int AB = 0, bool ZW = false>
 __global__ __launch_bounds__(64 * NWP * NWC) void conv1x1_ring_kernel(const dvie_conv_desc p, int n_ct, int n_tiles) {
   constexpr int dbg = AB;
   typedef G1Cfg<TMC, 2, 64, NWP, MI, NWC> C;
@@ -478,6 +519,10 @@
       ((unsigned long long)p.n * p.yh * p.yw - 1) * (unsigned long long)p.y_ld * 2ull + (unsigned long long)p.cout * 2ull;
   const __amdgpu_buffer_rsrc_t ry = __builtin_amdgcn_make_buffer_rsrc(p.y, 0, (int)ybytes, 0x00020000);
   const __amdgpu_buffer_rsrc_t rb = __builtin_amdgcn_make_buffer_rsrc((void*)p.bias, 0, p.bias ? p.cout * 4 : 0, 0x00020000);
+  static_assert(!ZW || (TMC == 4 && ACT == DVIE_ACT_LRELU), "bitmap writer: 16 bytes per 128-channel wave tile");
+  const __amdgpu_buffer_rsrc_t rzb = __builtin_amdgcn_make_buffer_rsrc(
+      ZW ? p.zbits : nullptr, 0,
+      ZW ? (int)(((unsigned long long)p.n * p.yh * p.yw - 1) * (unsigned long long)p.zbits_ld + p.cout / 8) : 0, 0x00020000);
 
   int prow[PPH];
   unsigned xoff[PPH], woff[PPH], chk[PPH];
@@ -547,7 +592,7 @@
   int jj = 0;
   auto job = [&](bool first, bool after_epi) {
     if (after_epi)
-      DVIE_VMCNT1(PPH + 2 * MI * TMC);
+      DVIE_VMCNT1(PPH + 2 * MI * TMC + (ZW ? MI : 0));
     else
       DVIE_VMCNT1(PPH);
     __builtin_amdgcn_s_waitcnt(0xC07F);
@@ -615,6 +660,7 @@
         const int oy = r / p.ow, ox = r - oy * p.ow;
         yp = ((long long)n * p.yh + oy * p.osy + p.ory) * p.yw + ox * p.osx + p.orx;
       }
+      unsigned zq[2] = {0u, 0u};
 #pragma unroll
       for (int j = 0; j < TMC; ++j)
 #pragma unroll
@@ -632,19 +678,69 @@
             for (int e = 0; e < 8; ++e) w[e] = fmaxf(w[e], w[e] * p.alpha);
           }
           const i32x4 o = pack_bf16x8(w);
+          if constexpr (ZW) zq[j >> 1] |= sign_bits8(o) << (8 * (2 * (j & 1) + P));
           const int co = c0 + wc * 32 * TMC + 32 * j + 16 * P + 8 * hh;
           const unsigned yo = (pix_ok && co < p.cout && !(dbg & 1)) ? (unsigned)((yp * p.y_ld + co) * 2) : OOB;
           __builtin_amdgcn_raw_buffer_store_b128(__builtin_bit_cast(i32x4, o), ry, yo, 0, 0);
         }
+      if constexpr (ZW) {
+        const auto sw = __builtin_amdgcn_permlane32_swap(zq[0], zq[1], false, false);
+        const unsigned ev = sw[0], od = sw[1];
+        i32x2 zo;
+        zo[0] = (int)((ev & 0xffu) | ((od & 0xffu) << 8) | ((ev & 0xff00u) << 8) | ((od & 0xff00u) << 16));
+        zo[1] = (int)(((ev >> 16) & 0xffu) | ((od >> 8) & 0xff00u) | ((ev >> 8) & 0xff0000u) | (od & 0xff000000u));
+        const int cz = c0 + wc * 32 * TMC + 64 * hh;
+        const unsigned zo_off = (pix_ok && cz < p.cout) ? (unsigned)(yp * p.zbits_ld + (cz >> 3)) : OOB;
+        __builtin_amdgcn_raw_buffer_store_b64(zo, rzb, zo_off, 0, 0);
+      }
     }
   }
   __builtin_amdgcn_s_waitcnt(0);
 }
 
-template <int V, int NS, int MT>
+template <int V, int NS, int MT, int TMC = 4>
 struct PreOk {
-  static constexpr int v = NS != 1 || MT > 4 ? 0 : V;
+  static constexpr int v = NS != 1 || MT > 4 ? 0 : (V & 7) | (TMC == 4 ? (V & 8) : 0) | (MT == TMC && TMC <= 4 ? (V & 16) : 0);
 };
+
+static bool sign_act(int a) { return a == DVIE_ACT_LRELU || a == DVIE_ACT_RELU; }
+static bool ident_out(const dvie_conv_desc& p) {
+  return p.osy == 1 && p.osx == 1 && p.ory == 0 && p.orx == 0 && p.yh == p.oh && p.yw == p.ow;
+}
+enum Tile1x1 { T_2_1, T_2_3, T_4_3, T_4_1, T_WIDE };
+static Tile1x1 tile_1x1(const dvie_conv_desc& p) {
+  const bool one = p.c <= 64;
+  if (p.cout <= 64 || (p.cout <= 128 && one)) return one ? T_2_1 : T_2_3;
+  if (p.cout <= 128) return T_4_3;
+  return one ? T_4_1 : T_WIDE;
+}
+static bool ring_takes(const dvie_conv_desc& p) {
+  if (tile_1x1(p) != T_WIDE || p.out_f32) return false;
+  const int npix = p.n * p.oh * p.ow;
+  const int n_tiles = ((p.cout + 255) / 256) * ((npix + 255) / 256);
+  const unsigned long long span = ((unsigned long long)p.n * p.yh * p.yw - 1) * (unsigned long long)p.y_ld * 2ull +
+                                  (unsigned long long)p.cout * 2ull;
+  const unsigned long long xspan = ((unsigned long long)npix - 1) * (unsigned long long)p.x_ld * 2ull + (unsigned long long)p.c * 2ull;
+  return p.c > 64 && n_tiles > 256 && !p.res && !p.beta && !p.dact && span < 0xFFFFFF00ull && xspan < 0xFFFFFF00ull &&
+         p.ih == p.oh && p.iw == p.ow &&
+         (p.act == DVIE_ACT_NONE || (p.act == DVIE_ACT_LRELU && p.alpha >= 0.f && p.alpha <= 1.f));
+}
+static bool zb_reads(const dvie_conv_desc& p) {
+  return p.zbits && sign_act(p.dact) && !p.out_f32 && ident_out(p) && tile_1x1(p) == T_4_1 &&
+         ((uintptr_t)p.zbits & 15) == 0 && p.zbits_ld % 16 == 0 && p.cout % 128 == 0;
+}
+static bool zb_writes(const dvie_conv_desc& p) {
+  if (!p.zbits || !sign_act(p.act) || p.dact || p.beta || p.out_f32 || !ident_out(p)) return false;
+  const Tile1x1 t = tile_1x1(p);
+  if (t == T_WIDE) {
+    const unsigned long long zspan = (unsigned long long)p.n * p.yh * p.yw * (unsigned long long)p.zbits_ld;
+    return ring_takes(p) && p.act == DVIE_ACT_LRELU && ((uintptr_t)p.zbits & 7) == 0 && p.zbits_ld % 8 == 0 &&
+           p.cout % 64 == 0 && zspan < 0x7FFFFF00ull;
+  }
+  if (t != T_4_1 && t != T_2_1) return false;
+  const int a = t == T_4_1 ? 8 : 4;
+  return ((uintptr_t)p.zbits & (a - 1)) == 0 && p.zbits_ld % a == 0 && p.cout % (8 * a) == 0;
+}
 
 static int dbg_env() {
 #ifdef DVIE_TIMING_DBG
@@ -661,9 +757,11 @@
 }
 
 template <int TMC, int NS, int KC = 64, int NWP = 8, int MI = 1, int NWC = 1>
-static void launch_1x1(const dvie_conv_desc& p, hipStream_t s) {
+static void launch_1x1(const dvie_conv_desc& p_in, hipStream_t s) {
   typedef G1Cfg<TMC, NS, KC, NWP, MI, NWC> C;
   constexpr int NW = C::NW;
+  dvie_conv_desc p = p_in;
+  if (p.zbits && p.act && !zb_writes(p)) p.zbits = nullptr;
   const int npix = p.n * p.oh * p.ow;
   const int n_ct = (p.cout + C::BC - 1) / C::BC;
   const int n_tiles = n_ct * ((npix + C::BP - 1) / C::BP);
@@ -672,12 +770,8 @@
     return;
   }
   if constexpr (NS == 2 && KC == 64 && TMC == 4 && NWP == 4 && MI == 2 && NWC == 2) {
-    const unsigned long long span = ((unsigned long long)p.n * p.yh * p.yw - 1) * (unsigned long long)p.y_ld * 2ull +
-                                    (unsigned long long)p.cout * 2ull;
-    const unsigned long long xspan = ((unsigned long long)npix - 1) * (unsigned long long)p.x_ld * 2ull + (unsigned long long)p.c * 2ull;
-    if (p.c > KC && n_tiles > 256 && !p.res && !p.beta && !p.dact && span < 0xFFFFFF00ull &&
-        xspan < 0xFFFFFF00ull && p.ih == p.oh && p.iw == p.ow &&
-        (p.act == DVIE_ACT_NONE || (p.act == DVIE_ACT_LRELU && p.alpha >= 0.f && p.alpha <= 1.f))) {
+    static_assert(C::BC == 256 && C::BP == 256, "ring_takes counts 256 x 256 tiles");
+    if (ring_takes(p)) {
 #ifdef DVIE_TIMING_DBG
       if (p.act == DVIE_ACT_LRELU) switch (dbg_env() & 7) {
 #define DVIE_RING_AB(V)                                                                                                \
@@ -690,7 +784,9 @@
           default: break;
         }
 #endif
-      if (p.act == DVIE_ACT_LRELU)
+      if (p.act == DVIE_ACT_LRELU && p.zbits)
+        DVIE_LAUNCH((conv1x1_ring_kernel<TMC, NWP, MI, NWC, DVIE_ACT_LRELU, 0, true>), dim3(256), dim3(64 * NW), 0, s, p, n_ct, n_tiles);
+      else if (p.act == DVIE_ACT_LRELU)
         DVIE_LAUNCH((conv1x1_ring_kernel<TMC, NWP, MI, NWC, DVIE_ACT_LRELU>), dim3(256), dim3(64 * NW), 0, s, p, n_ct, n_tiles);
       else
         DVIE_LAUNCH((conv1x1_ring_kernel<TMC, NWP, MI, NWC, DVIE_ACT_NONE>), dim3(256), dim3(64 * NW), 0, s, p, n_ct, n_tiles);
@@ -706,11 +802,13 @@
       return;
     }
   }
-  const bool ident = p.osy == 1 && p.osx == 1 && p.ory == 0 && p.orx == 0 && p.yh == p.oh && p.yw == p.ow;
+  const bool ident = ident_out(p);
   int pre = 0;
   if constexpr (NS == 1) {
     if (ident && p.c <= KC) {
       pre = MI * TMC > 4 ? 0 : (p.res ? 1 : 0) | (p.beta ? 2 : 0) | (p.dact ? 4 : 0);
+      if ((pre & 4) && zb_reads(p)) pre |= 8;
+      if (p.zbits && p.act) pre |= 16;
     }
   }
   if constexpr (NS == 1 && MI == 1 && 2 * TMC == 8) {
@@ -718,11 +816,12 @@
       switch (pre) {
 #define DVIE_CE_CASE(V)                                                                                              \
   case V:                                                                                                            \
-    DVIE_LAUNCH((conv1x1_kernel<TMC, NS, KC, NWP, MI, NWC, false, PreOk<V, NS, MI * TMC>::v, true>), dim3(n_tiles), \
+    DVIE_LAUNCH((conv1x1_kernel<TMC, NS, KC, NWP, MI, NWC, false, PreOk<V, NS, MI * TMC, TMC>::v, true>), dim3(n_tiles), \
                        dim3(64 * NW), 0, s, p, n_ct, n_tiles, 0);                                                     \
     return;
         DVIE_CE_CASE(0) DVIE_CE_CASE(1) DVIE_CE_CASE(2) DVIE_CE_CASE(3) DVIE_CE_CASE(4)
         DVIE_CE_CASE(5) DVIE_CE_CASE(6) DVIE_CE_CASE(7)
+        DVIE_CE_CASE(12) DVIE_CE_CASE(13) DVIE_CE_CASE(14) DVIE_CE_CASE(15) DVIE_CE_CASE(16) DVIE_CE_CASE(17)
 #undef DVIE_CE_CASE
       }
     }
@@ -730,34 +829,43 @@
   switch (pre) {
 #define DVIE_PRE_CASE(V)                                                                                          \
   case V:                                                                                                        \
-    DVIE_LAUNCH((conv1x1_kernel<TMC, NS, KC, NWP, MI, NWC, false, PreOk<V, NS, MI * TMC>::v>), dim3(n_tiles), \
+    DVIE_LAUNCH((conv1x1_kernel<TMC, NS, KC, NWP, MI, NWC, false, PreOk<V, NS, MI * TMC, TMC>::v>), dim3(n_tiles), \
                        dim3(64 * NW), 0, s, p, n_ct, n_tiles, dbg_env());                                                   \
     break;
     DVIE_PRE_CASE(1) DVIE_PRE_CASE(2) DVIE_PRE_CASE(3) DVIE_PRE_CASE(4) DVIE_PRE_CASE(5)
     DVIE_PRE_CASE(6) DVIE_PRE_CASE(7)
+    DVIE_PRE_CASE(12) DVIE_PRE_CASE(13) DVIE_PRE_CASE(14) DVIE_PRE_CASE(15) DVIE_PRE_CASE(16) DVIE_PRE_CASE(17)
 #undef DVIE_PRE_CASE
     default:
       DVIE_LAUNCH((conv1x1_kernel<TMC, NS, KC, NWP, MI, NWC, false>), dim3(n_tiles), dim3(64 * NW), 0, s, p, n_ct, n_tiles, dbg_env());
   }
 }
 
-bool conv1x1_launch(const dvie_conv_desc& p, hipStream_t s) {
+static bool takes_1x1(const dvie_conv_desc& p) {
   if (p.dtype != DVIE_BF16 || p.th != 1 || p.tw != 1) return false;
   if (p.sy != 1 || p.sx != 1 || p.dy0 != 0 || p.dx0 != 0 || p.ih != p.oh || p.iw != p.ow) return false;
   if (p.osy < 1 || p.osx < 1 || p.ory < 0 || p.orx < 0) return false;
   if (p.c % 64 != 0 && p.c > 64) return false;
   if ((long long)p.n * p.oh * p.ow >= (1LL << 31)) return false;
-  const int cout = p.cout;
-  const bool one = p.c <= 64;
-  if (cout <= 64 || (cout <= 128 && one))
-    one ? launch_1x1<2, 1>(p, s) : launch_1x1<2, 3>(p, s);
-  else if (cout <= 128)
-    launch_1x1<4, 3>(p, s);
-  else if (one)
-    launch_1x1<4, 1>(p, s);
-  else
-    launch_1x1<4, 2, 64, 4, 2, 2>(p, s);
   return true;
 }
 
-}
+int conv1x1_zbits(const dvie_conv_desc& p) {
+  if (!takes_1x1(p)) return -1;
+  if (zb_writes(p)) return tile_1x1(p) == T_WIDE ? 2 : 1;
+  return zb_reads(p);
+}
+
+bool conv1x1_launch(const dvie_conv_desc& p, hipStream_t s) {
+  if (!takes_1x1(p)) return false;
+  switch (tile_1x1(p)) {
+    case T_2_1: launch_1x1<2, 1>(p, s); break;
+    case T_2_3: launch_1x1<2, 3>(p, s); break;
+    case T_4_3: launch_1x1<4, 3>(p, s); break;
+    case T_4_1: launch_1x1<4, 1>(p, s); break;
+    case T_WIDE: launch_1x1<4, 2, 64, 4, 2, 2>(p, s); break;
+  }
+  return true;
+}
+
+}
diff --git a/deep_video_interpolation_extrapolation_amd/csrc/conv_epilogue.h b/deep_video_interpolation_extrapolation_amd/csrc/conv_epilogue.h
--- a/deep_video_interpolation_extrapolation_amd/csrc/conv_epilogue.h
+++ b/deep_video_interpolation_extrapolation_amd/csrc/conv_epilogue.h
@@ -65,6 +65,25 @@
   dact8(w, z, dact, alpha);
 }
 
+__device__ __forceinline__ void dact_bits8(float* w, unsigned bits, int dact, float alpha) {
+  if (dact == DVIE_ACT_LRELU) {
+#pragma unroll
+    for (int k = 0; k < 8; ++k) w[k] *= (bits >> k) & 1u ? 1.f : alpha;
+  } else if (dact == DVIE_ACT_RELU) {
+#pragma unroll
+    for (int k = 0; k < 8; ++k) w[k] = (bits >> k) & 1u ? w[k] : 0.f;
+  }
+}
+
+__device__ __forceinline__ unsigned sign_bits8(const i32x4 packed) {
+  float z[8];
+  unpack_bf16x8(packed, z);
+  unsigned bits = 0;
+#pragma unroll
+  for (int k = 0; k < 8; ++k) bits |= (z[k] > 0.f ? 1u : 0u) << k;
+  return bits;
+}
+
 template <bool R, bool B, bool Z>
 __device__ __forceinline__ i32x4 epi8_regs(float* w, const dvie_conv_desc& p, const i32x4* r, const i32x4* b,
                                            const i32x4* z) {
@@ -72,6 +91,16 @@
   if constexpr (B) add_bf16x8(w, *b);
   act8(w, p.act, p.alpha);
   if constexpr (Z) dact_bf16x8(w, *z, p.dact, p.alpha);
+  return pack_bf16x8(w);
+}
+
+template <bool R, bool B>
+__device__ __forceinline__ i32x4 epi8_regs_bits(float* w, const dvie_conv_desc& p, const i32x4* r, const i32x4* b,
+                                                unsigned bits) {
+  if constexpr (R) add_bf16x8(w, *r);
+  if constexpr (B) add_bf16x8(w, *b);
+  act8(w, p.act, p.alpha);
+  dact_bits8(w, bits, p.dact, p.alpha);
   return pack_bf16x8(w);
 }
 
diff --git a/deep_video_interpolation_extrapolation_amd/csrc/conv_fwd.hip b/deep_video_interpolation_extrapolation_amd/csrc/conv_fwd.hip
--- a/deep_video_interpolation_extrapolation_amd/csrc/conv_fwd.hip
+++ b/deep_video_interpolation_extrapolation_amd/csrc/conv_fwd.hip
@@ -330,10 +330,27 @@
 bool conv_halo_ph4_launch(const dvie_conv_desc& p, hipStream_t s);
 bool conv1x1_launch(const dvie_conv_desc& p, hipStream_t s);
 bool conv_s2_launch(const dvie_conv_desc& p, hipStream_t s);
+int conv1x1_zbits(const dvie_conv_desc& p);
+int conv_halo_zbits(const dvie_conv_desc& p);
 
 }
 
 using namespace dvie;
+
+static long long batch_chunk(const dvie_conv_desc* d, unsigned long long img_x) {
+  return (long long)(0xFFFFFF00ull / img_x) < d->n ? (long long)(0xFFFFFF00ull / img_x) : d->n;
+}
+
+extern "C" int dvie_conv_zbits(const dvie_conv_desc* d) {
+  if (!d || !d->zbits || d->dtype != DVIE_BF16 || d->out_f32 || d->phc) return 0;
+  if (d->zbits_ld <= 0 || d->ih <= 0 || d->iw <= 0) return 0;
+  if (d->x_ld <= 0 || d->n <= 0) return 0;
+  const unsigned long long img_x = (unsigned long long)d->ih * d->iw * d->x_ld * 2ull;
+  if (img_x >= 0xFFFFFF00ull || batch_chunk(d, img_x) < d->n) return 0;
+  int r = conv1x1_zbits(*d);
+  if (r < 0) r = conv_halo_zbits(*d);
+  return r > 0 ? r : 0;
+}
 
 extern "C" int dvie_conv2d_fwd(const dvie_conv_desc* d, void* stream) {
   DVIE_CHECK_ARG(d && d->x && d->w && d->y, "conv: null pointer");
@@ -357,7 +374,7 @@
   DVIE_CHECK_ARG(wb < 0xFFFFFF00ull, "conv: weights exceed the 4 GiB buffer range");
   DVIE_CHECK_ARG(img_x < 0xFFFFFF00ull, "conv: one input image exceeds the 4 GiB buffer range");
   hipStream_t s = (hipStream_t)stream;
-  const long long chunk = (long long)(0xFFFFFF00ull / img_x) < d->n ? (long long)(0xFFFFFF00ull / img_x) : d->n;
+  const long long chunk = batch_chunk(d, img_x);
   const int oes = (d->out_f32 || d->dtype == DVIE_F32) ? 4 : 2;
   const unsigned long long img_y = (unsigned long long)d->yh * d->yw;
   for (long long n0 = 0; n0 < d->n; n0 += chunk) {
@@ -367,6 +384,7 @@
     c.y = (char*)d->y + n0 * img_y * d->y_ld * oes;
     if (d->res) c.res = (const char*)d->res + n0 * img_y * d->res_ld * oes;
     if (d->z) c.z = (const char*)d->z + n0 * img_y * d->z_ld * es;
+    if (d->zbits) c.zbits = (char*)d->zbits + n0 * img_y * d->zbits_ld;
     if (c.phc) {
       DVIE_CHECK_ARG(conv_halo_ph4_launch(c, s), "conv: phase-split output (phc=%d) needs bf16, 2x2 taps at "
                      "(0,0), osy=osx=2, cout=4*phc, phc %% 32 == 0, no bias", c.phc);
diff --git a/deep_video_interpolation_extrapolation_amd/csrc/conv_halo.hip b/deep_video_interpolation_extrapolation_amd/csrc/conv_halo.hip
--- a/deep_video_interpolation_extrapolation_amd/csrc/conv_halo.hip
+++ b/deep_video_interpolation_extrapolation_amd/csrc/conv_halo.hip
@@ -837,7 +837,7 @@
   static constexpr int NS = (NG + 1) / 2;
 };
 
-template <int CP8, bool OUTF32, bool PRE = false>
+template <int CP8, bool OUTF32, bool PRE = false, bool ZB = false>
 __global__ __launch_bounds__(512, 2) void conv_nk_kernel(const dvie_conv_desc p, int n_cb, int n_tiles, int tiles_x,
                                                         int tiles_y) {
   typedef NkCfg<CP8> C;
@@ -920,20 +920,23 @@
         (void*)p.res, 0,
         p.res ? (int)(((unsigned long long)p.n * p.yh * p.yw - 1) * (unsigned long long)p.res_ld * 2ull + p.cout * 2ull) : 0,
         0x00020000);
+    static_assert(!ZB || PRE, "bitmap operand: the prefetch form");
     const __amdgpu_buffer_rsrc_t rz = __builtin_amdgcn_make_buffer_rsrc(
-        (void*)p.z, 0,
-        p.dact ? (int)(((unsigned long long)p.n * p.yh * p.yw - 1) * (unsigned long long)p.z_ld * 2ull + p.cout * 2ull) : 0,
+        ZB ? (void*)p.zbits : (void*)p.z, 0,
+        ZB ? (int)(((unsigned long long)p.n * p.yh * p.yw - 1) * (unsigned long long)p.zbits_ld + p.cout / 8)
+           : p.dact ? (int)(((unsigned long long)p.n * p.yh * p.yw - 1) * (unsigned long long)p.z_ld * 2ull + p.cout * 2ull) : 0,
         0x00020000);
-    const int nops = (p.res ? 1 : 0) + (p.beta ? 1 : 0) + (p.dact ? 1 : 0);
+    const int nloads = 4 * ((p.res ? 1 : 0) + (p.beta ? 1 : 0)) + (ZB ? 2 : p.dact ? 4 : 0);
     auto offs = [&](const TP& T, int b, int P, unsigned& oy_, unsigned& or_, unsigned& oz_) {
       const int oy = T.y0 + wp, ox = T.x0 + 32 * b + r32, co = co0 + 16 * P;
       const bool ok = oy < p.oh && ox < p.ow && co < p.cout;
       const long long pix = ((long long)T.n * p.yh + oy * p.osy + p.ory) * p.yw + ox * p.osx + p.orx;
       oy_ = ok ? (unsigned)((pix * p.y_ld + co) * 2) : OOB;
       or_ = ok ? (unsigned)((pix * p.res_ld + co) * 2) : OOB;
-      oz_ = ok ? (unsigned)((pix * p.z_ld + co) * 2) : OOB;
+      oz_ = !ok ? OOB : ZB ? (unsigned)(pix * p.zbits_ld + ((co0 - 8 * hh) >> 3)) : (unsigned)((pix * p.z_ld + co) * 2);
     };
     i32x4 er[2][2], eb[2][2], ez[2][2];
+    unsigned ezb[2] = {0u, 0u};
     auto prefetch = [&](const TP& T) {
 #pragma unroll
       for (int b = 0; b < 2; ++b)
@@ -943,7 +946,11 @@
           offs(T, b, P, o_y, o_r, o_z);
           if (p.res) er[b][P] = __builtin_bit_cast(i32x4, __builtin_amdgcn_raw_buffer_load_b128(rr, o_r, 0, 0));
           if (p.beta) eb[b][P] = __builtin_bit_cast(i32x4, __builtin_amdgcn_raw_buffer_load_b128(ry, o_y, 0, 0));
-          if (p.dact) ez[b][P] = __builtin_bit_cast(i32x4, __builtin_amdgcn_raw_buffer_load_b128(rz, o_z, 0, 0));
+          if constexpr (ZB) {
+            if (P == 0) ezb[b] = __builtin_amdgcn_raw_buffer_load_b32(rz, o_z, 0, 0);
+          } else {
+            if (p.dact) ez[b][P] = __builtin_bit_cast(i32x4, __builtin_amdgcn_raw_buffer_load_b128(rz, o_z, 0, 0));
+          }
         }
     };
     f32x4 bia[2][2];
@@ -995,7 +1002,10 @@
           if (p.res) add_bf16x8(w, er[b][P]);
           if (p.beta) add_bf16x8(w, eb[b][P]);
           act8(w, p.act, p.alpha);
-          if (p.dact) dact_bf16x8(w, ez[b][P], p.dact, p.alpha);
+          if constexpr (ZB)
+            dact_bits8(w, (ezb[b] >> (8 * (2 * P + hh))) & 0xffu, p.dact, p.alpha);
+          else if (p.dact)
+            dact_bf16x8(w, ez[b][P], p.dact, p.alpha);
           const i32x4 o = pack_bf16x8(w);
           unsigned o_y, o_r, o_z;
           offs(cur, b, P, o_y, o_r, o_z);
@@ -1003,7 +1013,7 @@
         }
       }
       prefetch(nxt);
-      wait_vmcnt(4 + 4 * nops);
+      wait_vmcnt(4 + nloads);
       __builtin_amdgcn_s_barrier();
       cur = nxt;
     }
@@ -1045,6 +1055,14 @@
 static bool nk_pre_on() {
   const char* e = getenv("DVIE_NK_PRE");
   return !(e && *e == '0');
+}
+
+static bool nk_zb_reads(const dvie_conv_desc& p) {
+  if (!p.zbits || !(p.dact == DVIE_ACT_LRELU || p.dact == DVIE_ACT_RELU) || p.out_f32 || !nk_pre_on()) return false;
+  if (((uintptr_t)p.zbits & 3) != 0 || p.zbits_ld % 4 != 0 || p.cout % 32 != 0) return false;
+  const unsigned long long opix = (unsigned long long)p.n * p.yh * p.yw - 1;
+  return (opix * p.y_ld + p.cout) * 2ull < 0xFFFFFF00ull && (!p.res || (opix * p.res_ld + p.cout) * 2ull < 0xFFFFFF00ull) &&
+         opix * (unsigned long long)p.zbits_ld + p.cout / 8 < 0x7FFFFF00ull;
 }
 
 template <int CP8>
@@ -1063,6 +1081,8 @@
                         (!p.dact || (opix * p.z_ld + p.cout) * 2ull < 0xFFFFFF00ull);
   if (p.out_f32)
     DVIE_LAUNCH((conv_nk_kernel<CP8, true>), dim3(grid), dim3(512), 0, s, p, n_cb, n_tiles, tiles_x, tiles_y);
+  else if (nk_zb_reads(p))
+    DVIE_LAUNCH((conv_nk_kernel<CP8, false, true, true>), dim3(grid), dim3(512), 0, s, p, n_cb, n_tiles, tiles_x, tiles_y);
   else if (nk_pre_on() && spans_ok && (p.res || p.beta || p.dact))
     DVIE_LAUNCH((conv_nk_kernel<CP8, false, true>), dim3(grid), dim3(512), 0, s, p, n_cb, n_tiles, tiles_x, tiles_y);
   else
@@ -1283,9 +1303,13 @@
           (void*)((const bf16_t*)p.res + ((EPI & 1) ? pix0 * p.res_ld : 0)), 0, 0x7FFFFFF0, 0x00020000);
       const __amdgpu_buffer_rsrc_t rb =
           __builtin_amdgcn_make_buffer_rsrc((void*)((const bf16_t*)p.y + pix0 * p.y_ld), 0, 0x7FFFFFF0, 0x00020000);
+      constexpr bool ZB = (EPI & 8) != 0;
+      static_assert(!ZB || (EPI & 4) != 0, "bitmap operand: with the activation derivative");
       const __amdgpu_buffer_rsrc_t rz = __builtin_amdgcn_make_buffer_rsrc(
-          (void*)((const bf16_t*)p.z + ((EPI & 4) ? pix0 * p.z_ld : 0)), 0, 0x7FFFFFF0, 0x00020000);
+          ZB ? (void*)((const char*)p.zbits + pix0 * p.zbits_ld)
+             : (void*)((const bf16_t*)p.z + ((EPI & 4) ? pix0 * p.z_ld : 0)), 0, 0x7FFFFFF0, 0x00020000);
       i32x4 o_r[2][2], o_b[2][2], o_z[2][2];
+      unsigned o_zb[2] = {0u, 0u};
       auto epi_load = [&](int gi) {
         const int i = gi & 1, r = gi >> 2, b = (gi >> 1) & 1, u = gi & 1;
 #pragma unroll
@@ -1296,7 +1320,9 @@
             const long long dp = (long long)(2 * wp + r) * p.osy * p.yw + (long long)(32 * b + r32) * p.osx;
             if (EPI & 1) o_r[u][P] = __builtin_amdgcn_raw_buffer_load_b128(rr, ok ? (unsigned)((dp * p.res_ld + co) * 2) : OOB, 0, 0);
             if (EPI & 2) o_b[u][P] = __builtin_amdgcn_raw_buffer_load_b128(rb, ok ? (unsigned)((dp * p.y_ld + co) * 2) : OOB, 0, 0);
-            if (EPI & 4) o_z[u][P] = __builtin_amdgcn_raw_buffer_load_b128(rz, ok ? (unsigned)((dp * p.z_ld + co) * 2) : OOB, 0, 0);
+            if ((EPI & 4) && !ZB) o_z[u][P] = __builtin_amdgcn_raw_buffer_load_b128(rz, ok ? (unsigned)((dp * p.z_ld + co) * 2) : OOB, 0, 0);
+            if (ZB && P == 0)
+              o_zb[u] = __builtin_amdgcn_raw_buffer_load_b32(rz, ok ? (unsigned)(dp * p.zbits_ld + ((J.c0 + wc * 64 + 32 * i) >> 3)) : OOB, 0, 0);
           }
       };
       if (EPI) epi_load(0);
@@ -1324,7 +1350,9 @@
             const int co = J.c0 + wc * 64 + 32 * i + 16 * P + 8 * hh;
             float* w = v8[P];
             if (p.bias) add_f32x8(w, p.bias + co);
-            const i32x4 o = epi8_regs<(EPI & 1) != 0, (EPI & 2) != 0, (EPI & 4) != 0>(w, p, &o_r[u][P], &o_b[u][P], &o_z[u][P]);
+            const i32x4 o = ZB ? epi8_regs_bits<(EPI & 1) != 0, (EPI & 2) != 0>(w, p, &o_r[u][P], &o_b[u][P],
+                                                                                (o_zb[u] >> (8 * (2 * P + hh))) & 0xffu)
+                               : epi8_regs<(EPI & 1) != 0, (EPI & 2) != 0, (EPI & 4) != 0>(w, p, &o_r[u][P], &o_b[u][P], &o_z[u][P]);
             if (ok) __builtin_amdgcn_raw_buffer_store_b128(o, rb, (unsigned)((dp * p.y_ld + co) * 2), 0, 0);
           }
         }
@@ -1348,16 +1376,27 @@
   DVIE_LAUNCH((conv_h8_kernel<EPI>), dim3(grid), dim3(H8::NTH), 0, s, p, n_ct, n_tiles, tiles_x, tiles_y);
 }
 
+static bool h8_takes(const dvie_conv_desc& p) {
+  if (!h8_on() || p.out_f32 || p.c % 32 != 0 || p.c < 64 || p.cout % 128 != 0) return false;
+  const long long nt = (long long)(p.cout / H8::BC) * ((p.ow + 63) / 64) * ((p.oh + H8::PR - 1) / H8::PR) * p.n;
+  return nt >= 224 && nt < (1LL << 30);
+}
+
+static bool h8_zb_reads(const dvie_conv_desc& p) {
+  if (!p.zbits || !(p.dact == DVIE_ACT_LRELU || p.dact == DVIE_ACT_RELU)) return false;
+  if (((uintptr_t)p.zbits & 3) != 0 || p.zbits_ld % 4 != 0) return false;
+  return (unsigned long long)p.n * p.yh * p.yw * (unsigned long long)p.zbits_ld < 0x7FFFFF00ull;
+}
+
 static bool conv_h8_launch(const dvie_conv_desc& p, hipStream_t s) {
-  if (!h8_on() || p.out_f32 || p.c % 32 != 0 || p.c < 64 || p.cout % 128 != 0) return false;
+  if (!h8_takes(p)) return false;
   const int n_ct = p.cout / H8::BC, tiles_x = (p.ow + 63) / 64, tiles_y = (p.oh + H8::PR - 1) / H8::PR;
-  const long long nt = (long long)n_ct * tiles_x * tiles_y * p.n;
-  if (nt < 224 || nt >= (1LL << 30)) return false;
-  const int n_tiles = (int)nt;
-  switch ((p.res ? 1 : 0) | (p.beta ? 2 : 0) | (p.dact ? 4 : 0)) {
+  const int n_tiles = n_ct * tiles_x * tiles_y * p.n;
+  switch ((p.res ? 1 : 0) | (p.beta ? 2 : 0) | (p.dact ? 4 : 0) | (h8_zb_reads(p) ? 8 : 0)) {
 #define DVIE_H8(EPI) \
   case EPI: launch_h8<EPI>(p, s, n_ct, n_tiles, tiles_x, tiles_y); break;
     DVIE_H8(0) DVIE_H8(1) DVIE_H8(2) DVIE_H8(3) DVIE_H8(4) DVIE_H8(5) DVIE_H8(6) DVIE_H8(7)
+    DVIE_H8(12) DVIE_H8(13) DVIE_H8(14) DVIE_H8(15)
 #undef DVIE_H8
   }
   return true;
@@ -1377,7 +1416,7 @@
   return p.cout % 128 != 0 ? try_halo<1, 2, 4, 2, 2, true>(p, s) : try_halo<2, 2, 4, 2, 2, true>(p, s);
 }
 
-bool conv_halo_launch(const dvie_conv_desc& p, hipStream_t s) {
+static bool halo_takes(const dvie_conv_desc& p) {
   if (p.dtype != DVIE_BF16) return false;
   if (p.sy != 1 || p.sx != 1 || p.ddy != 1 || p.ddx != 1) return false;
   if (p.osy < 1 || p.osx < 1 || p.ory < 0 || p.orx < 0) return false;
@@ -1388,7 +1427,25 @@
   const unsigned long long pix = (unsigned long long)p.n * p.ih * p.iw;
   if (pix >= (1ull << 31)) return false;
   if (((pix - 1) * (unsigned long long)p.x_ld + (unsigned long long)p.c) * 2ull >= 0xFFFFFF00ull) return false;
-  if (t3 && p.c % 8 == 0 && p.c <= 24 && p.kpad >= 9 * p.c) {
+  return true;
+}
+
+static bool nk_takes(const dvie_conv_desc& p) {
+  return p.c % 8 == 0 && p.c <= 24 && p.kpad >= 9 * p.c;
+}
+
+int conv_halo_zbits(const dvie_conv_desc& p) {
+  if (!halo_takes(p)) return -1;
+  if (p.th != 3 || p.tw != 3) return 0;
+  if (nk_takes(p)) return nk_zb_reads(p);
+  return h8_takes(p) && h8_zb_reads(p);
+}
+
+bool conv_halo_launch(const dvie_conv_desc& p, hipStream_t s) {
+  if (!halo_takes(p)) return false;
+  const bool t1 = p.th == 1 && p.tw == 1, t3 = p.th == 3 && p.tw == 3;
+  const bool t22 = p.th == 2 && p.tw == 2, t12 = p.th == 1 && p.tw == 2, t21 = p.th == 2 && p.tw == 1;
+  if (t3 && nk_takes(p)) {
     switch (p.c / 8) {
       case 1: launch_nk<1>(p, s); break;
       case 2: launch_nk<2>(p, s); break;
diff --git a/deep_video_interpolation_extrapolation_amd/engine.py b/deep_video_interpolation_extrapolation_amd/engine.py
--- a/deep_video_interpolation_extrapolation_amd/engine.py
+++ b/deep_video_interpolation_extrapolation_amd/engine.py
@@ -644,6 +644,11 @@
         self._i2c = None
         self.ws = None
         self.ws_floats = 1
+        self.zbits = {}
+        self._zbits_level = int(os.environ.get("DVIE_ZBITS", "1") or 0)
+        self._zbits_on = self._zbits_level > 0
+        self._fwd_conv = {}
+        self._zb = {}
         self._alloc()
         self._build_pack()
         self._build_forward()
@@ -916,6 +921,8 @@
                                              + lay.cout * lay.cin * lay.kh * lay.kw)))
         if ext:
             self.ext_out.setdefault(out.buf.name, []).append((len(self.fwd), out))
+        else:
+            self._fwd_conv[id(op)] = o
         self.fwd.append(o)
 
     def _convT_fwd(self, op):
@@ -1155,9 +1162,60 @@
             epi = Epilogue(beta=0 if i == 0 else 1, res=r[0] if r else None, res_ld=r[1] if r else 0)
             if i == len(seq) - 1:
                 epi = epi._replace(dact=dact, z=z, z_ld=b.C)
-            self.bwd.extend(em(epi))
+            n_placed = len(self.bwd)
+            ops = em(epi)
+            if fuse_dact and i == len(seq) - 1:
+                self._zbits_region(b, region, prod[0], ops, self.bwd[n_placed:])
+            self.bwd.extend(ops)
         b.n_flushed += 1
         b.done = b.n_flushed == len(b.expected)
+
+    def _zbits_region(self, b, region, prod, ops, placed):
+        if not self._zbits_on or self.dtype != torch.bfloat16 or prod.act not in (L.ACT_LRELU, L.ACT_RELU):
+            return
+        st = self._zb.setdefault(id(b), dict(buf=b, prod=prod, users=[], regions=set(), ok=True, t=None))
+        fo = self._fwd_conv.get(id(prod))
+        if not ops and any(o.kind == L.OP_HEAD3_BWD and o.u.head3.dact for o in placed):
+            st["regions"].add(region.key())
+            return
+        dact_of = {L.OP_CONV: lambda o: o.u.conv.dact, L.OP_EW: lambda o: o.u.ew.dact, L.OP_ATTN: lambda o: o.u.attn.dact}
+        carriers = [o for o in ops if dact_of.get(o.kind, lambda o: 1)(o)]
+        if (fo is None or b.C % 8 or region.c0 % 8 or prod.out.c0 % 8 or not carriers
+                or any(o.kind != L.OP_CONV for o in carriers)):
+            st["ok"] = False
+            return
+        if st["t"] is None:
+            st["t"] = torch.empty(self.nf * b.H * b.W * b.C // 8, dtype=torch.uint8, device=self.device)
+        for o in carriers:
+            d = o.u.conv
+            d.zbits, d.zbits_ld = st["t"].data_ptr() + region.c0 // 8, b.C // 8
+            st["users"].append((o, region))
+            st["regions"].add(region.key())
+            if not L.load().dvie_conv_zbits(ctypes.byref(d)):
+                st["ok"] = False
+
+    def _zbits_settle(self):
+        for st in self._zb.values():
+            b, prod = st["buf"], st["prod"]
+            ok = st["ok"] and st["t"] is not None and len(st["regions"]) == len(b.expected)
+            if ok:
+                d = self._fwd_conv[id(prod)].u.conv
+                d.zbits, d.zbits_ld = st["t"].data_ptr() + prod.out.c0 // 8, b.C // 8
+                ok = 0 < L.load().dvie_conv_zbits(ctypes.byref(d)) <= self._zbits_level
+                if not ok:
+                    d.zbits, d.zbits_ld = None, 0
+            if not ok:
+                for o, _ in st["users"]:
+                    o.u.conv.zbits, o.u.conv.zbits_ld = None, 0
+                continue
+            self.zbits[b.name] = st["t"]
+            self.keep.append(st["t"])
+            for o, r in st["users"]:
+                d = o.u.conv
+                o.meta["bytes"] -= float(d.n * d.oh * d.ow * d.cout) * (self.es - 0.125)
+            fo = self._fwd_conv[id(prod)]
+            fo.meta["bytes"] += float(self.nf * b.H * b.W * prod.out.c) / 8
+        self._zb = {}
 
     def _ensure_dact(self, op):
         b = op.out.buf
@@ -1257,6 +1315,7 @@
             if bf.needs_grad and bf.expected and not bf.done:
                 raise RuntimeError(f"incomplete gradient for {bf}: pending {({k: len(v) for k, v in bf.pending.items()})}"
                                    f" of {bf.expected}")
+        self._zbits_settle()
 
     def _out_nchw_backward(self, op, gout, gld):
         pass
diff --git a/include/dvie.h b/include/dvie.h
--- a/include/dvie.h
+++ b/include/dvie.h
@@ -38,9 +38,13 @@
   float alpha;
   int phc;
   int pad1;
+  void* zbits;
+  long long zbits_ld;
 } dvie_conv_desc;
 
 int dvie_conv2d_fwd(const dvie_conv_desc* d, void* stream);
+
+int dvie_conv_zbits(const dvie_conv_desc* d);
 
 typedef struct dvie_wgrad_desc {
   const void* g;
```

Measured after the change: 261.0 frames/s (median of 6 runs). 1.8% higher.
